# IvanBanny/para-ortho-pca-bo

Measured on AMD Instinct MI355X. Metric: BO iterations/sec (incl. GP refit + EI opt), BBOB f15 d=40, higher is better.
Workload: dtype f64; 1 GPU; configs[1]: PCA_BO on BBOB f15 d=40, budget=450, n_DoE=120, EI, var_threshold=0.95; one run per GPU (run list f15/d40/instances 0..N-1 partitioned by pcabo.sharding), timed steps spread evenly over the 330 BO iterations of the run; num_restarts=10, raw_samples=512, batch_limit=5, maxiter=200, parallelism=run-parallel x1

## Files before the change

### include/pcabo.h

```cpp
#ifndef PCABO_H
#define PCABO_H

#include <stddef.h>
#include <stdint.h>

#ifdef __cplusplus
extern "C" {
#endif

typedef struct pcabo_ctx pcabo_ctx;

typedef enum {
  PCABO_OK = 0,
  PCABO_ERR_ARG = -1,
  PCABO_ERR_NOT_PD = -2,
  PCABO_ERR_HIP = -3,
  PCABO_ERR_NAN = -4,
  PCABO_ERR_TIMEOUT = -5
} pcabo_status;

enum { PCABO_KERNEL_MATERN52 = 0, PCABO_KERNEL_RBF = 1 };
enum { PCABO_ACQ_LOG_EI = 0, PCABO_ACQ_PI = 1, PCABO_ACQ_UCB = 2 };
enum { PCABO_PTR_HOST = 0, PCABO_PTR_DEVICE = 1 };

int pcabo_abi_version(void);

int pcabo_device_count(void);

int pcabo_ctx_create(int device, int max_n, int max_d, int max_q, pcabo_ctx** out);
int pcabo_ctx_destroy(pcabo_ctx* ctx);
int pcabo_set_pointer_mode(pcabo_ctx* ctx, int mode);
int pcabo_last_error(pcabo_ctx* ctx, char* buf, int buflen);

enum { PCABO_OPT_RESIDENT = 0, PCABO_OPT_BESTF_F32 = 1, PCABO_OPT_GROUP_ACQ = 2,
       PCABO_OPT_DEVICE_LBFGSB = 3 ,
       PCABO_OPT_HIDDEN_TAIL = 5  };
int pcabo_set_option(pcabo_ctx* ctx, int option, int value);

int pcabo_wpca(pcabo_ctx* ctx, const double* X, const double* f, const int64_t* ranks, int n, int d,
               int maximize, double var_threshold, int n_components, const double* noise,
               double* data_mean, double* pca_mean, double* comps, double* evr, int* k, double* Z);

int pcabo_gp_condition(pcabo_ctx* ctx, const double* Z, const double* y, int n, int k,
                       const double* norm_bounds, double lengthscale, double noise, int kernel);

int pcabo_gp_condition_begin(pcabo_ctx* ctx, const double* Z, const double* y, int n, int k,
                             const double* norm_bounds, double lengthscale, double noise, int kernel);
int pcabo_gp_condition_end(pcabo_ctx* ctx);

int pcabo_gp_condition_end_eval(pcabo_ctx* ctx, const double* Xq, int q, double best_f, int maximize, int acq,
                                double* val);

int pcabo_gp_mll(pcabo_ctx* ctx, const double* Z , const double* y, int n, int k,
                 const double* norm_bounds, int kernel, const double* theta , double* loss, double* grad );
#define PCABO_FIT_TASK_NOT_PD (-2)
#define PCABO_FIT_TASK_DOMAIN (-3)
int pcabo_gp_fit(pcabo_ctx* ctx, const double* Z, const double* y, int n, int k, const double* norm_bounds, int kernel,
                 double* theta_inout , double* loss, int* info );
int pcabo_gp_mll_ard(pcabo_ctx* ctx, const double* Z, const double* y, int n, int k, const double* norm_bounds, int kernel,
                     const double* theta , double* loss, double* grad );
int pcabo_gp_fit_ard(pcabo_ctx* ctx, const double* Z, const double* y, int n, int k, const double* norm_bounds, int kernel,
                     double* theta_inout , double* loss, int* info );

int pcabo_wpca_gp_condition_begin(pcabo_ctx* ctx, const double* X, const double* f, const int64_t* ranks, int n,
                                  int d, int maximize, double var_threshold, int n_components, const double* noise,
                                  const double* y, double lengthscale, double gp_noise, int kernel,
                                  double* data_mean, double* pca_mean, double* comps, double* evr, int* k);

int pcabo_wpca_results(pcabo_ctx* ctx, double* data_mean, double* pca_mean, double* comps, double* evr, int* k);

int pcabo_acq_bounds(pcabo_ctx* ctx, double* bounds);

int pcabo_acq_eval(pcabo_ctx* ctx, const double* Xq, int q, double best_f, int maximize, int acq,
                   double* val, double* grad);
int pcabo_logei(pcabo_ctx* ctx, const double* Xq, int q, double best_f, int maximize,
                double* val, double* grad);

int pcabo_optimize_acqf(pcabo_ctx* ctx, const double* ics, int num_restarts, int batch_limit,
                        const double* bounds, int maxiter, double best_f, int maximize, int acq,
                        double* cand, double* vals, int* info, int* failed);

int pcabo_inverse_map(pcabo_ctx* ctx, const double* z, double* x);

int pcabo_get_gp_state(pcabo_ctx* ctx, double* K_chol , double* Rinv ,
                       double* alpha , double* y_mean_std , double* norm_bounds );
int pcabo_get_gram(pcabo_ctx* ctx, double* K );

typedef double (*pcabo_fg_callback)(const double* x, double* g, void* user);
int pcabo_lbfgsb_minimize(int nvar, double* x, const double* lower, const double* upper,
                          pcabo_fg_callback fg, void* user, int m, double factr, double pgtol,
                          int maxiter, int maxfun, int maxls, double* f_out, int* nit, int* nfev,
                          int* task_out);
int pcabo_lbfgsb_set_vector_kernels(int enabled);
int pcabo_lbfgsb_set_sum_order(int order);

int pcabo_sobol_scramble(int64_t* state, const int64_t* ltm, int k);
int pcabo_sobol_draw(const int64_t* state, const int64_t* shift, int k, int n, const double* lo, const double* rng, double* out);
int pcabo_sobol_draw_rows(const int64_t* const* states, const int64_t* const* shifts, const int* ks, int rows, int n,
                          const double* boxes, long long box_stride, double* const* outs);
int pcabo_torch_randint2(void* blob, int64_t count, int64_t* out);
int pcabo_torch_multinomial_rows(void* const* blobs, const double* weights, int rows, int n, int n_pick, int64_t* out);
int pcabo_boltzmann_pick_rows(void* const* blobs, const double* vals, int rows, int n, int n_pick, double eta, int64_t* out, int* flags);

int pcabo_set_profiling(pcabo_ctx* ctx, int enabled);
int pcabo_get_profile_calibration(pcabo_ctx* ctx, double* pair_ms, double* empty_kernel_ms);
int pcabo_get_profile(pcabo_ctx* ctx, int which, double* ms, int64_t* launches, double* bytes, double* flops);
int pcabo_reset_profile(pcabo_ctx* ctx);

typedef struct pcabo_batch pcabo_batch;
int pcabo_batch_create(int device, int B, int max_n, int max_d, int max_q, pcabo_batch** out);
int pcabo_batch_destroy(pcabo_batch* batch);
int pcabo_batch_set_workers(pcabo_batch* batch, int workers);
int pcabo_batch_set_option(pcabo_batch* batch, int option, int value);
int pcabo_device_lbfgsb_limits(int* max_n, int* max_k, int* max_group);
int pcabo_batch_last_error(pcabo_batch* batch, char* buf, int buflen);
pcabo_ctx* pcabo_batch_ctx(pcabo_batch* batch, int b);

int pcabo_batch_set_input_strides(pcabo_batch* batch, size_t x_stride, size_t noise_stride, size_t y_stride);
int pcabo_batch_wpca_gp_condition_begin(pcabo_batch* batch, const double* X, const int64_t* ranks, const double* noise,
// ... 49 lines not shown
```

### para-ortho-pca-bo_amd/csrc/kernels_acq.hip

```cpp
#include "pcabo_internal.h"
#include "acq_math.h"
#include <algorithm>
#include <cstdlib>
#include <mutex>

#define PSTRIDE (2 + 2 * PCABO_MAXD)

#ifdef PCABO_ACQ_TIMING
__device__ unsigned long long g_acq_stamps[16];
#define STAMP(i) do { if (blockIdx.x == gridDim.x / 2 && blockIdx.y == 0 && threadIdx.x == 0) g_acq_stamps[i] = wall_clock64(); } while (0)
#define STAMP_FIN(i) do { if (blockIdx.y == 0 && threadIdx.x == 0) g_acq_stamps[i] = wall_clock64(); } while (0)
extern "C" int pcabo_debug_acq_stamps(unsigned long long* out16) {
  return hipMemcpyFromSymbol(out16, HIP_SYMBOL(g_acq_stamps), sizeof(g_acq_stamps)) == hipSuccess ? 0 : -3;
}
#else
#define STAMP(i)
#define STAMP_FIN(i)
#endif

__device__ inline void st_wt(double* p, double v) {
  __hip_atomic_store(p, v, __ATOMIC_RELAXED, __HIP_MEMORY_SCOPE_AGENT);
}

template <int SLAB>
// ... 578 lines not shown
  __syncthreads();
  STAMP(5);
  {
    double gs[CU], gm[CU];
#pragma unroll
    for (int u = 0; u < CU; ++u) { gs[u] = 0.0; gm[u] = 0.0; }
#pragma unroll
    for (int b = 0; b < NB; ++b) {
      const double ts = s_ks[l + 64 * b], tm = s_tm[l + 64 * b];
#pragma unroll
      for (int u = 0; u < CU; ++u) {
        const double dlt = xc[u] - z[u][b];
        gs[u] += ts * dlt;
        gm[u] += tm * dlt;
      }
    }
    const int nu = k > w ? (k - w + 3) / 4 : 0;
    if (nu > 5) publish_grad<10>(gs, gm, w, k, l, pout, out, cur_seq);
    else if (nu > 2) publish_grad<5>(gs, gm, w, k, l, pout, out, cur_seq);
    else if (nu > 0) publish_grad<2>(gs, gm, w, k, l, pout, out, cur_seq);
  }
  }
  }
  q = (!SRV && ab.table) ? (int)(reinterpret_cast<const unsigned*>(qa.x)[blockIdx.y] & 0xffffu) : (int)blockIdx.y * qb;
  out = partial + ((size_t)q * S + s) * PSTRIDE;
  if (!server) {
    acq_tail<SLAB>(combine, s_v, partial, counters, q, S, k, bounds4, ystats, prm, val, grad, host_val, host_grad, hm, cur_seq, tid, w, l);
    break;
  }
  ++cur_seq;
  __syncthreads();
  }
}

__device__ void acq_scalar_core(double vv, double mus, int q, double ym, double ysd, const AcqParams& p, double* val,
                                double* host_val, double* coef, int l) {
  double value, c_mu, c_sg;
  acq_scalar_chain(vv, mus, ym, ysd, p.best_f, p.maximize, p.acq, &value, &c_mu, &c_sg);
  if (l == 0) {
    val[q] = value;
    if (host_val) host_val[q] = value;
    coef[0] = c_mu;
    coef[1] = c_sg;
  }
  STAMP_FIN(12);
}

__device__ void acq_finish_scalar(const double* base, int S, int q, const double* ystats, const AcqParams& p, double* val,
                                  double* host_val, double* coef, int l) {
  const double ym = ystats[0], ysd = ystats[1];
  double vv = 0.0, mus = 0.0;
  for (int s = l; s < S; s += 64) { vv += base[(size_t)s * PSTRIDE]; mus += base[(size_t)s * PSTRIDE + 1]; }
  vv = wave_sum(vv);
  mus = wave_sum(mus);
  STAMP_FIN(11);
  acq_scalar_core(vv, mus, q, ym, ysd, p, val, host_val, coef, l);
}

__device__ void acq_finish_query(const double* base, int S, int k, int q, const double* bounds4, const double* ystats,
                                 const AcqParams& p, double* val, double* grad, double* host_val, double* host_grad,
                                 int l) {
  __shared__ double s_cf2[4][2];
  double* coef = s_cf2[(threadIdx.x >> 6) & 3];
  acq_finish_scalar(base, S, q, ystats, p, val, host_val, coef, l);
  if (p.want_grad) {
    __builtin_amdgcn_wave_barrier();
    const double c_mu = coef[0], c_sg = coef[1];
    for (int c = l; c < k; c += 64) {
      double a0, b0, a1, b1, a2, b2;
      grad_partial_sum(base, S, c, 0, &a0, &b0);
      grad_partial_sum(base, S, c, 1, &a1, &b1);
      grad_partial_sum(base, S, c, 2, &a2, &b2);
      const double gs = (a0 + a1) + a2, gm = (b0 + b1) + b2;
      double g = __fma_rn(c_mu, gm, c_sg * gs) / (bounds4[PCABO_MAXD + c] - bounds4[c]);
      grad[(size_t)q * k + c] = g;
      if (host_grad) host_grad[(size_t)q * k + c] = g;
    }
  }
}

__global__ __launch_bounds__(256) void k_acq_combine(const double* __restrict__ partial, int q_total, int S, int k,
                                                     const double* __restrict__ bounds4,
                                                     const double* __restrict__ ystats, AcqParams p,
                                                     double* __restrict__ val, double* __restrict__ grad, AcqBatch ab) {
  if (ab.zs) {
    const unsigned run_ = blockIdx.z;
    partial = zrun(partial, ab.zs, run_); bounds4 = zrun(bounds4, ab.zs, run_); ystats = zrun(ystats, ab.zs, run_);
    val = zrun(val, ab.zs, run_); grad = zrun(grad, ab.zs, run_);
    if (ab.k_dev) k = *zrun(ab.k_dev, ab.zs, run_);
    if (ab.bestf) p.best_f = *zrun(ab.bestf, ab.zs, run_);
  }
  const int q = blockIdx.x * 4 + (threadIdx.x >> 6);
  if (q < q_total)
    acq_finish_query(partial + (size_t)q * S * PSTRIDE, S, k, q, bounds4, ystats, p, val, grad, nullptr, nullptr,
                     threadIdx.x & 63);
}

#ifdef PCABO_ACQ_TIMING
#define GSTAMP(i) do { if (blockIdx.x == gridDim.x - 1 && blockIdx.y == 0 && threadIdx.x == 0) g_acq_stamps[i] = wall_clock64(); } while (0)
#else
#define GSTAMP(i)
#endif
#define GQ 5
#define GT_LD 17
#define WAVE_LDS_SYNC() asm volatile("s_waitcnt lgkmcnt(0)" ::: "memory")
template <int NT>
__global__ __launch_bounds__(256) void k_acq_group(
    QueryArgs qa, const double* __restrict__ Xq, int n, int k, int NP, int ld,
    const double* __restrict__ ZnT, const double* __restrict__ R, const double* __restrict__ alpha,
    const double* __restrict__ bounds4, const double* __restrict__ ystats, AcqParams prm, double* partial,
    unsigned int* counters, double* __restrict__ val, double* __restrict__ grad, double* host_val, double* host_grad,
    HostMirror* hm, unsigned long long seq, AcqBatch ab) {
  const unsigned ent = reinterpret_cast<const unsigned*>(qa.x)[blockIdx.y];
  const unsigned run_ = ent >> 16;
  const int q0 = (int)((ent >> 8) & 0xffu), nq = (int)(ent & 0xffu);
  if (ab.zs) {
    ZnT = zrun(ZnT, ab.zs, run_); R = zrun(R, ab.zs, run_); alpha = zrun(alpha, ab.zs, run_);
    bounds4 = zrun(bounds4, ab.zs, run_); ystats = zrun(ystats, ab.zs, run_); partial = zrun(partial, ab.zs, run_);
    counters = zrun(counters, ab.zs, run_); val = zrun(val, ab.zs, run_); grad = zrun(grad, ab.zs, run_);
    Xq = zrun(Xq, ab.xq_host ? ab.hzs : ab.zs, run_);
    host_val = zrun(host_val, ab.hzs, run_); host_grad = zrun(host_grad, ab.hzs, run_); hm = zrun(hm, ab.hzs, run_);
    if (ab.k_dev) k = *zrun(ab.k_dev, ab.zs, run_);
    if (ab.bestf) prm.best_f = *zrun(ab.bestf, ab.zs, run_);
    if (ab.hyp) prm.inv_ls = zrun(ab.hyp, ab.zs, run_)[PCABO_HYP_INV_LS];
  }
  const int tid = threadIdx.x, l = tid & 63;
  const int w = __builtin_amdgcn_readfirstlane(tid >> 6);
  const int s = blockIdx.x, S = gridDim.x;
  const int r0 = 64 * s, ncol = 64 * (s + 1);
  const int KS = (k + 1) & ~1;
  extern __shared__ __attribute__((aligned(16))) double s_dyn[];
  double* s_ks = s_dyn;
  double* s_tile = s_ks + GQ * (NP > 2 * KS ? NP : 2 * KS);
  double* s_v = s_tile + 4 * 64 * GT_LD;
  double* s_tm = s_v + 64 * 8;
  double* s_coef = s_tm + GQ * 64;
  int* s_flag = reinterpret_cast<int*>(s_coef + 2 * GQ);
  double* s_vvmu = s_coef + 2 * GQ + 4;
  double* s_xn = s_vvmu + 2 * GQ;
  double* s_part = s_tile;
  double* s_gout = s_ks;
  const double inv_ls = prm.inv_ls;
  const int kernel = prm.kernel;

  GSTAMP(0);
  for (int idx = tid; idx < GQ * k; idx += 256) {
    const int q = idx / k, c = idx - q * k;
    const int qq = q < nq ? q : 0;
    const double lo = bounds4[c], hi = bounds4[PCABO_MAXD + c];
    s_xn[q * KS + c] = (Xq[(size_t)(q0 + qq) * k + c] - lo) / (hi - lo);
  }
  __syncthreads();
  GSTAMP(1);
  double cfr[NT][GQ];
  {
    const int jlim = n < ncol ? n : ncol;
    double sq[NT][GQ];
#pragma unroll
    for (int t = 0; t < NT; ++t)
#pragma unroll
      for (int q = 0; q < GQ; ++q) sq[t][q] = 0.0;
    constexpr int CB = NT == 1 ? 40 : (NT == 2 ? 20 : 8);
    for (int c0 = 0; c0 < k; c0 += CB) {
      double z[NT][CB];
#pragma unroll
      for (int t = 0; t < NT; ++t)
#pragma unroll
        for (int u = 0; u < CB; ++u) {
          const int cc = c0 + u < k ? c0 + u : k - 1, jj = tid + 256 * t < NP ? tid + 256 * t : NP - 1;
          z[t][u] = ZnT[(size_t)cc * ld + jj];
        }
#pragma unroll
      for (int u = 0; u < CB; ++u) {
        if (c0 + u < k) {
#pragma unroll
          for (int q = 0; q < GQ; ++q) {
            const double xq = s_xn[q * KS + c0 + u];
// ... 388 lines not shown
  const double* Rrow = R + (size_t)(I * 64) * ld;
  const double* Krow = KS + (size_t)(qb * 64) * ld;
  double pa[16], pb[16];
  auto fetch = [&](int J) {
#pragma unroll
    for (int u = 0; u < 16; ++u) {
      const int idx = tid + 256 * u, r = idx >> 6, c = idx & 63;
      pa[u] = Rrow[(size_t)r * ld + J * 64 + c];
      pb[u] = (qb * 64 + r < q_total) ? Krow[(size_t)r * ld + J * 64 + c] : 0.0;
    }
  };
  auto put = [&]() {
#pragma unroll
    for (int u = 0; u < 16; ++u) {
      const int idx = tid + 256 * u, r = idx >> 6, c = idx & 63;
      s_a[r * PCABO_TLD + c] = pa[u];
      s_b[r * PCABO_TLD + c] = pb[u];
    }
  };
  double4_t acc[4];
#pragma unroll
  for (int t = 0; t < 4; ++t) acc[t] = (double4_t){0.0, 0.0, 0.0, 0.0};
  fetch(0);
  for (int J = 0; J <= I; ++J) {
    __syncthreads();
    put();
    if (J < I) fetch(J + 1);
    __syncthreads();
    for (int kk = 0; kk < 64; kk += 4) {
      const double a = s_a[(16 * w + (l & 15)) * PCABO_TLD + kk + (l >> 4)];
#pragma unroll
      for (int t = 0; t < 4; ++t) {
        const double b = s_b[(16 * t + (l & 15)) * PCABO_TLD + kk + (l >> 4)];
        acc[t] = __builtin_amdgcn_mfma_f64_16x16x4f64(a, b, acc[t], 0, 0, 0);
      }
    }
  }
#pragma unroll
  for (int t = 0; t < 4; ++t) {
    double v = ((acc[t][0] * acc[t][0] + acc[t][1] * acc[t][1]) + acc[t][2] * acc[t][2]) + acc[t][3] * acc[t][3];
    v += __shfl_xor(v, 16, 64);
    v += __shfl_xor(v, 32, 64);
    if (l < 16) s_red[w][16 * t + l] = v;
  }
  __syncthreads();
  if (tid < 64 && qb * 64 + tid < q_total) {
    double* rec = partial + ((size_t)(qb * 64 + tid) * S + I) * PSTRIDE;
    rec[0] = ((s_red[0][tid] + s_red[1][tid]) + s_red[2][tid]) + s_red[3][tid];
    if (I >= njb) rec[1] = 0.0;
  }
}

bool score_gemm_possible(int q) { return q >= 64; }

__global__ __launch_bounds__(256) void k_score_ks_only(const double* __restrict__ Xq, int q_total, int n, int k, int NP, int ld,
                                                       const double* __restrict__ ZnT, const double* __restrict__ bounds4,
                                                       AcqParams prm, double* __restrict__ KS) {
  double ks[SC_QB];
  score_ks_block(Xq, q_total, n, k, NP, ld, ZnT, bounds4, prm, KS, ks);
}

__global__ __launch_bounds__(256) void k_score_mu(const double* __restrict__ KS, int q_total, int n, int ld,
                                                  const double* __restrict__ alpha, double* __restrict__ partial, int S) {
  __shared__ double s_mu[4][SC_QB];
  const int tid = threadIdx.x, l = tid & 63, w = tid >> 6;
  const int j = blockIdx.x * 256 + tid, q0 = blockIdx.y * SC_QB;
  const double aj = j < n ? alpha[j] : 0.0;
#pragma unroll
  for (int q = 0; q < SC_QB; ++q) {
    const double ks = (j < n && q0 + q < q_total) ? KS[(size_t)(q0 + q) * ld + j] : 0.0;
    const double m = wave_sum(aj * ks);
    if (l == 0) s_mu[w][q] = m;
  }
  __syncthreads();
  if (tid < SC_QB && q0 + tid < q_total)
    partial[((size_t)(q0 + tid) * S + blockIdx.x) * PSTRIDE + 1] = ((s_mu[0][tid] + s_mu[1][tid]) + s_mu[2][tid]) + s_mu[3][tid];
}

void launch_score_ks_only(hipStream_t st, const double* Xq, int q, const GpModel& m, AcqParams p, double* KS) {
  const int njb = (m.NP + 255) / 256;
  hipLaunchKernelGGL(k_score_ks_only, dim3(njb, (q + SC_QB - 1) / SC_QB, 1), dim3(256), 0, st, Xq, q, m.n, m.k, m.NP, m.ld, m.ZnT,
                     m.bounds4, p, KS);
}
void launch_score_tail(hipStream_t st, int q, const GpModel& m, AcqParams p, const double* KS, double* partial, double* val) {
  const int S = m.NP / 64, njb = (m.NP + 255) / 256;
  hipLaunchKernelGGL(k_score_mu, dim3(njb, (q + SC_QB - 1) / SC_QB, 1), dim3(256), 0, st, KS, q, m.n, m.ld, m.alpha, partial, S);
  hipLaunchKernelGGL(k_score_gemm, dim3(S, (q + 63) / 64, 1), dim3(256), 0, st, m.R, KS, q, m.NP, m.ld, njb, partial, (size_t)0);
  p.want_grad = 0;
  hipLaunchKernelGGL(k_acq_combine, dim3((q + 3) / 4, 1, 1), dim3(256), 0, st, partial, q, S, m.k, m.bounds4, m.ystats, p, val,
                     (double*)nullptr, AcqBatch());
}

void launch_score(hipStream_t st, const double* Xq, int q, const GpModel& m, AcqParams p, double* KS, double* partial, double* val,
                  AcqBatch ab, int B) {
  const int S = m.NP / 64, njb = (m.NP + 255) / 256;
  hipLaunchKernelGGL(k_score_ks, dim3(njb, (q + SC_QB - 1) / SC_QB, B), dim3(256), 0, st, Xq, q, m.n, m.k, m.NP, m.ld, m.ZnT, m.alpha,
                     m.bounds4, p, KS, partial, S, ab);
  hipLaunchKernelGGL(k_score_gemm, dim3(S, (q + 63) / 64, B), dim3(256), 0, st, m.R, KS, q, m.NP, m.ld, njb, partial, ab.zs);
  p.want_grad = 0;
  hipLaunchKernelGGL(k_acq_combine, dim3((q + 3) / 4, 1, B), dim3(256), 0, st, partial, q, S, m.k, m.bounds4, m.ystats, p, val,
                     (double*)nullptr, ab);
}

bool acq_server_possible(int q, int n, int k, int NP) {
  static int cus = -1;
  if (cus < 0) {
    int dev = 0;
    if (hipGetDevice(&dev) != hipSuccess || hipDeviceGetAttribute(&cus, hipDeviceAttributeMultiprocessorCount, dev) != hipSuccess) cus = 0;
  }
  if (k > 40 || NP > 512 || q < 1 || q > PCABO_INLAUNCH_MAXQ || (size_t)q * k > PCABO_QA_MAX) return false;
  const int S = acq_slabs(NP);
  return (S + 1) * q <= cus && S <= 32;
}

void launch_acq(hipStream_t st, const QueryArgs* qa, const double* Xq, int q, const GpModel& m, AcqParams p, double* partial,
                unsigned int* counters, double* val, double* grad, double* host_val, double* host_grad, HostMirror* hm,
                unsigned long long seq, MailPair* dev_mail, MailPair* part_pairs, AcqBatch ab, int B, int table_entries) {
  const int n = m.n, k = m.k, NP = m.NP, ld = m.ld;
  const double *ZnT = m.ZnT, *R = m.R, *alpha = m.alpha, *bounds4 = m.bounds4, *ystats = m.ystats;
  const int slab = NP >= ACQ_SLAB32_NP ? 32 : 16;
  const int S = NP / slab;
  static const QueryArgs empty = {};
  const int combine = hm != nullptr;
  const int nb = NP / 64;
  const bool fast = k <= 40 && nb <= 8;
  const int qb = (fast && !combine && q >= 64) ? 8 : 1;
  const int gy = ab.table ? table_entries : (q + qb - 1) / qb;
  const int gz = ab.table ? 1 : B;
#define ACQ_ARGS qa ? *qa : empty, Xq, q, n, k, NP, ld, ZnT, R, alpha, bounds4, ystats, p, partial, counters, val, grad, \
                 host_val, host_grad, hm, seq, combine, qb, dev_mail, part_pairs, ab
  const int FIN_LDS = 6 * PCABO_MAXD + 2;
#define ACQ_LDS(SL, NBV) (3 * NBV * 64 + PCABO_MAXD + SL + 2 + (4 * NBV * 64 > FIN_LDS ? 4 * NBV * 64 : FIN_LDS))
#define ACQ_FAST(SL, NBV)                                                                                      \
  case NBV:                                                                                                    \
    if (dev_mail)                                                                                              \
      hipLaunchKernelGGL((k_acq_fast<SL, NBV, true>), dim3(S + 1, gy), dim3(256),                              \
                         (size_t)std::max<int>(ACQ_LDS(SL, NBV), FIN_LDS_DOUBLES) * sizeof(double), st, ACQ_ARGS); \
    else                                                                                                       \
      hipLaunchKernelGGL((k_acq_fast<SL, NBV, false>), dim3(S, gy, gz), dim3(256),                             \
                         (size_t)ACQ_LDS(SL, NBV) * sizeof(double), st, ACQ_ARGS);                             \
    break;
  if (fast) {
    if (slab == 16) {
      switch (nb) { ACQ_FAST(16, 1) ACQ_FAST(16, 2) ACQ_FAST(16, 3) ACQ_FAST(16, 4) ACQ_FAST(16, 5) ACQ_FAST(16, 6)
                    ACQ_FAST(16, 7) ACQ_FAST(16, 8) }
    } else {
      switch (nb) { ACQ_FAST(32, 1) ACQ_FAST(32, 2) ACQ_FAST(32, 3) ACQ_FAST(32, 4) ACQ_FAST(32, 5) ACQ_FAST(32, 6)
                    ACQ_FAST(32, 7) ACQ_FAST(32, 8) }
    }
  } else {
    size_t lds = (size_t)(3 * NP + PCABO_MAXD + 32 + 2 + 6 * PCABO_MAXD + 2) * sizeof(double);
    if (slab == 16)
      hipLaunchKernelGGL(k_acq_fused<16>, dim3(S, ab.table ? gy : q, gz), dim3(256), lds, st, ACQ_ARGS);
    else
      hipLaunchKernelGGL(k_acq_fused<32>, dim3(S, ab.table ? gy : q, gz), dim3(256), lds, st, ACQ_ARGS);
  }
#undef ACQ_FAST
#undef ACQ_LDS
#undef ACQ_ARGS
  if (!combine)
    hipLaunchKernelGGL(k_acq_combine, dim3((q + 3) / 4, 1, gz), dim3(256), 0, st, partial, q, S, k, bounds4, ystats, p, val,
                       grad, ab);
}

template <int N>
__global__ __launch_bounds__(64) void k_debug_wave_sum_multi(const double* __restrict__ in, double* ref, double* multi,
                                                             double* uni, int* mism) {
  const int l = threadIdx.x;
  double v[N];
#pragma unroll
  for (int i = 0; i < N; ++i) v[i] = in[i * 64 + l];
#pragma unroll
  for (int i = 0; i < N; ++i) { const double r = wave_sum(v[i]); if (l == 0) ref[i] = r; }
  wave_sum_multi<N>(v, l);
  const int own = wave_multi_owner<N>(l), idx = wave_multi_index<N>(l);
  if (own >= 0) multi[own] = v[0];
  __syncthreads();
  if (__double_as_longlong(multi[idx]) != __double_as_longlong(v[0])) atomicAdd(&mism[idx], 1);
#pragma unroll
  for (int i = 0; i < N; ++i) { const double r = read_lane(v[0], __builtin_amdgcn_readfirstlane(wave_multi_lane(N, i))); if (l == 0) uni[i] = r; }
}

extern "C" int pcabo_debug_wave_sum_multi(const double* in, int N, double* ref, double* multi, double* uni, int* mism) {
  double* d = nullptr;
  if (hipMalloc(&d, (size_t)N * (64 + 3) * sizeof(double) + (size_t)N * sizeof(int)) != hipSuccess) return -3;
  double *dref = d + N * 64, *dmul = dref + N, *duni = dmul + N;
  int* dmis = reinterpret_cast<int*>(duni + N);
  int rc = hipMemcpy(d, in, (size_t)N * 64 * sizeof(double), hipMemcpyHostToDevice) == hipSuccess ? 0 : -3;
  if (rc == 0 && hipMemset(dref, 0, (size_t)N * 3 * sizeof(double) + (size_t)N * sizeof(int)) != hipSuccess) rc = -3;
#define DBG_WSM(NV) case NV: hipLaunchKernelGGL(k_debug_wave_sum_multi<NV>, dim3(1), dim3(64), 0, 0, d, dref, dmul, duni, dmis); break;
  if (rc == 0) {
    switch (N) { DBG_WSM(1) DBG_WSM(2) DBG_WSM(3) DBG_WSM(4) DBG_WSM(5) DBG_WSM(7) DBG_WSM(8) DBG_WSM(10) DBG_WSM(13)
                 DBG_WSM(20) DBG_WSM(33) DBG_WSM(64) default: rc = -1; }
  }
#undef DBG_WSM
  if (rc == 0 && hipGetLastError() != hipSuccess) rc = -3;
  if (rc == 0 && (hipMemcpy(ref, dref, N * sizeof(double), hipMemcpyDeviceToHost) != hipSuccess ||
                  hipMemcpy(multi, dmul, N * sizeof(double), hipMemcpyDeviceToHost) != hipSuccess ||
                  hipMemcpy(uni, duni, N * sizeof(double), hipMemcpyDeviceToHost) != hipSuccess ||
                  hipMemcpy(mism, dmis, N * sizeof(int), hipMemcpyDeviceToHost) != hipSuccess)) rc = -3;
  (void)hipFree(d);
  return rc;
}
```

### para-ortho-pca-bo_amd/csrc/kernels_gp.hip

```cpp
#include "pcabo_internal.h"
#include <mutex>
#include <cstdlib>

#define BS PCABO_BS
#define TLD PCABO_TLD

__global__ __launch_bounds__(256) void k_gram(const double* __restrict__ AT, const double* __restrict__ nrm, int n,
                                              int KP, int ld, double noise, int kernel, double* __restrict__ K,
                                              const int* __restrict__ k_dev, double* __restrict__ K2,
                                              int* __restrict__ info_reset, size_t zs, const double* __restrict__ hyp) {
  const XcdTile xt_ = xcd_tile();
  ZRUNX(AT); ZRUNX(nrm); ZRUNX(K); ZRUNX(k_dev); ZRUNX(K2); ZRUNX(info_reset); ZRUNX(hyp);
  if (hyp) noise = hyp[PCABO_HYP_NOISE];
  const int ti = (int)xt_.x, tj = (int)xt_.y;
  if (info_reset && ti == 0 && tj == 0 && threadIdx.x == 0) *info_reset = 0;
  if (tj > ti) return;
  if (k_dev) KP = (*k_dev + 3) & ~3;
  const int w = threadIdx.x >> 6, l = threadIdx.x & 63;
  const int i0 = ti * BS + 16 * w, j0 = tj * BS;
  double4_t acc[4];
  for (int t = 0; t < 4; ++t) acc[t] = (double4_t){0.0, 0.0, 0.0, 0.0};
  for (int kk = 0; kk < KP; kk += 4) {
    const double* row = AT + (size_t)(kk + (l >> 4)) * ld;
    double a = row[i0 + (l & 15)];
// ... 195 lines not shown
    for (int q = 0; q < 4; ++q)
#pragma unroll
      for (int r = 0; r < 4; ++r) dst[(size_t)(16 * w + (l >> 4) + 4 * r) * ld + 16 * q + (l & 15)] = cold[q][r];
  }
}
#define CHOL_LOOKN_NC 2
#define CHOL_LOOKN_LDS ((size_t)(1 + CHOL_LOOKN_NC) * BS * TLD * sizeof(double))

__global__ __launch_bounds__(256) void k_trinv_cols(const double* __restrict__ L, int nblk, int ld,
                                                    double* R, size_t zs) {
  const XcdTile xt_ = xcd_tile();
  ZRUNX(L); ZRUNX(R);
  __shared__ __attribute__((aligned(16))) double s_t[BS * TLD];
  __shared__ __attribute__((aligned(16))) double s_xk[BS * 16];
  const int tid = threadIdx.x;
  const int c0 = (int)xt_.x * 16;
  const int J = c0 / BS;
  const int w = tid >> 6, l = tid & 63;
  double pt[16], px[4];
  auto fetch_tile = [&](const double* src) {
#pragma unroll
    for (int u = 0; u < 16; ++u) { const int idx = tid + 256 * u; pt[u] = src[(size_t)(idx >> 6) * ld + (idx & 63)]; }
  };
  auto fetch_x = [&](int Kb) {
#pragma unroll
    for (int u = 0; u < 4; ++u) { const int idx = tid + 256 * u; px[u] = R[(size_t)(Kb * BS + (idx >> 4)) * ld + c0 + (idx & 15)]; }
  };
  auto put_tile = [&]() {
#pragma unroll
    for (int u = 0; u < 16; ++u) { const int idx = tid + 256 * u; s_t[(idx >> 6) * TLD + (idx & 63)] = pt[u]; }
  };
  auto put_x = [&]() {
#pragma unroll
    for (int u = 0; u < 4; ++u) s_xk[tid + 256 * u] = px[u];
  };
  if (J + 1 < nblk) { fetch_tile(L + (size_t)((J + 1) * BS) * ld + J * BS); fetch_x(J); }
  for (int I = J + 1; I < nblk; ++I) {
    double4_t acc = {0.0, 0.0, 0.0, 0.0};
    for (int Kb = J; Kb < I; ++Kb) {
      __syncthreads();
      put_tile(); put_x();
      if (Kb + 1 < I) { fetch_tile(L + (size_t)(I * BS) * ld + (Kb + 1) * BS); fetch_x(Kb + 1); }
      else fetch_tile(R + (size_t)(I * BS) * ld + I * BS);
      __syncthreads();
      for (int kk = 0; kk < BS; kk += 4) {
        double a = s_t[(16 * w + (l & 15)) * TLD + kk + (l >> 4)];
        double b = s_xk[(kk + (l >> 4)) * 16 + (l & 15)];
        acc = __builtin_amdgcn_mfma_f64_16x16x4f64(a, b, acc, 0, 0, 0);
      }
    }
    __syncthreads();
    for (int r = 0; r < 4; ++r) s_xk[(16 * w + (l >> 4) + 4 * r) * 16 + (l & 15)] = -acc[r];
    put_tile();
    if (I + 1 < nblk) { fetch_tile(L + (size_t)((I + 1) * BS) * ld + J * BS); fetch_x(J); }
    __syncthreads();
    double4_t x = {0.0, 0.0, 0.0, 0.0};
    for (int kk = 0; kk < BS; kk += 4) {
      double a = s_t[(16 * w + (l & 15)) * TLD + kk + (l >> 4)];
      double b = s_xk[(kk + (l >> 4)) * 16 + (l & 15)];
      x = __builtin_amdgcn_mfma_f64_16x16x4f64(a, b, x, 0, 0, 0);
    }
    for (int r = 0; r < 4; ++r)
      R[(size_t)(I * BS + 16 * w + (l >> 4) + 4 * r) * ld + c0 + (l & 15)] = x[r];
    __threadfence_block();
  }
}

__global__ __launch_bounds__(256) void k_rmatvec(const double* __restrict__ R, const double* __restrict__ y, int n,
                                                 int ld, double* __restrict__ t, size_t zs) {
  ZRUN(R); ZRUN(y); ZRUN(t);
  const int w = threadIdx.x >> 6, l = threadIdx.x & 63;
  for (int rr = 0; rr < 4; ++rr) {
    const int i = blockIdx.x * 16 + w * 4 + rr;
    double s = 0.0;
    if (i < n)
      for (int j = l; j <= i; j += 64) s += R[(size_t)i * ld + j] * y[j];
    s = wave_sum(s);
    if (l == 0) t[i] = (i < n) ? s : 0.0;
  }
}

#define RTM_WAVES 16
__global__ __launch_bounds__(64 * RTM_WAVES) void k_rtmatvec(const double* __restrict__ R, const double* __restrict__ t,
                                                             int n, int ld, double* __restrict__ out, size_t zs) {
  ZRUN(R); ZRUN(t); ZRUN(out);
  __shared__ double s_p[RTM_WAVES][64];
  const int w = threadIdx.x >> 6, l = threadIdx.x & 63;
  const int j0 = blockIdx.x * 64, j = j0 + l;
  double a0 = 0.0, a1 = 0.0, a2 = 0.0, a3 = 0.0;
  int i = j0 + w;
  for (; i + 3 * RTM_WAVES < n; i += 4 * RTM_WAVES) {
    a0 = fma(R[(size_t)i * ld + j], t[i], a0);
    a1 = fma(R[(size_t)(i + RTM_WAVES) * ld + j], t[i + RTM_WAVES], a1);
    a2 = fma(R[(size_t)(i + 2 * RTM_WAVES) * ld + j], t[i + 2 * RTM_WAVES], a2);
    a3 = fma(R[(size_t)(i + 3 * RTM_WAVES) * ld + j], t[i + 3 * RTM_WAVES], a3);
  }
  for (; i < n; i += RTM_WAVES) a0 = fma(R[(size_t)i * ld + j], t[i], a0);
  s_p[w][l] = (a0 + a1) + (a2 + a3);
  __syncthreads();
  if (w == 0) {
    double s = 0.0;
#pragma unroll
    for (int u = 0; u < RTM_WAVES; ++u) s += s_p[u][l];
    out[j] = (j < n) ? s : 0.0;
  }
}

void launch_gram(hipStream_t s, const double* AT, const double* nrm, int n, int NP, int KP, int ld, double noise,
                 int kernel, double* K, const int* k_dev, double* K2, int* info_reset, ZB zb) {
  int nb = NP / BS;
  hipLaunchKernelGGL(k_gram, dim3(nb, nb, zb.B), dim3(256), 0, s, AT, nrm, n, KP, ld, noise, kernel, K, k_dev, K2, info_reset,
                     zb.zs, zb.hyp);
}
void launch_add_jitter(hipStream_t s, double* K, int n, int ld, double jitter) {
  hipLaunchKernelGGL(k_add_jitter, dim3((n + 255) / 256), dim3(256), 0, s, K, n, ld, jitter);
}
bool chol_step_form(int NP, ZB zb) { return zb.B * (NP / BS) <= 256; }
int launch_cholesky(hipStream_t s, double* L, int NP, int ld, int* info, double* diag_scratch, ZB zb, double* R_folded) {
  const int nblk = NP / BS;
  if (chol_step_form(NP, zb)) return launch_chol_steps(s, L, NP, ld, info, diag_scratch, zb, R_folded);
  if (R_folded) return -1;
  if (zb.B * nblk > 1024) {
    for (int p = 0; p < nblk; ++p) {
      if (p > 0)
        hipLaunchKernelGGL(k_chol_lookback, dim3(nblk - p + 1, 1, zb.B), dim3(256), 0, s, L, p, nblk, ld, diag_scratch, zb.zs);
      launch_chol_panel(s, L, p, nblk - p, ld, info, diag_scratch, zb);
    }
    return 0;
  }
  constexpr int NC = CHOL_LOOKN_NC;
  {
    static std::mutex attr_mu;
    static bool attr_done[64] = {false};
    int dev = 0;
    if (hipGetDevice(&dev) != hipSuccess || dev < 0 || dev >= 64) return -1;
    std::lock_guard<std::mutex> lk(attr_mu);
    if (!attr_done[dev]) {
      if (hipFuncSetAttribute((const void*)k_chol_lookn<NC>, hipFuncAttributeMaxDynamicSharedMemorySize, (int)CHOL_LOOKN_LDS) != hipSuccess) return -1;
      attr_done[dev] = true;
    }
  }
  int last_panel = -1;
  for (int Jc = 0; Jc < nblk; Jc += NC) {
    const int ncols = nblk - Jc < NC ? nblk - Jc : NC;
    if (Jc > 0) {
      hipLaunchKernelGGL(k_chol_lookn<NC>, dim3(nblk - Jc + 1, 1, zb.B), dim3(256 * NC), CHOL_LOOKN_LDS, s, L, Jc, ncols, 0, Jc, ld,
                         diag_scratch, last_panel, zb.zs);
      last_panel = -1;
    }
    for (int c = 0; c < ncols; ++c) {
      const int p = Jc + c;
      launch_chol_panel(s, L, p, nblk - p, ld, info, diag_scratch, zb);
      last_panel = nblk - p > 1 ? p : -1;
      if (c + 1 < ncols) {
        hipLaunchKernelGGL(k_chol_lookn<NC>, dim3(nblk - (p + 1) + 1, 1, zb.B), dim3(256 * NC), CHOL_LOOKN_LDS, s, L, p + 1,
                           ncols - c - 1, p, p + 1, ld, diag_scratch, last_panel, zb.zs);
        last_panel = -1;
      }
    }
  }
  return 0;
}
void launch_trinv(hipStream_t s, const double* L, int NP, int ld, double* R, ZB zb) {
  const int nblk = NP / BS;
  launch_trinv_diag_w(s, L, nblk, ld, R, zb);
  hipLaunchKernelGGL(k_trinv_cols, dim3(NP / 16, 1, zb.B), dim3(256), 0, s, L, nblk, ld, R, zb.zs);
}
void launch_alpha(hipStream_t s, const double* R, const double* ys, int n, int NP, int ld, double* tmp, double* alpha,
                  ZB zb) {
  hipLaunchKernelGGL(k_rmatvec, dim3(NP / 16, 1, zb.B), dim3(256), 0, s, R, ys, n, ld, tmp, zb.zs);
  hipLaunchKernelGGL(k_rtmatvec, dim3(NP / 64, 1, zb.B), dim3(64 * RTM_WAVES), 0, s, R, tmp, n, ld, alpha, zb.zs);
}
```

### para-ortho-pca-bo_amd/csrc/kernels_wpca.hip

```cpp
#include "pcabo_internal.h"
#include <cstdlib>

#define WP_THREADS 1024

__device__ inline double block_sum_1024(double v, double* s_red) {
  const int tid = threadIdx.x, l = tid & 63;
  s_red[tid] = v;
  __syncthreads();
  if (tid < 64) {
    double a[8];
#pragma unroll
    for (int j = 0; j < 8; ++j) a[j] = s_red[64 * j + l] + s_red[64 * (j + 8) + l];
#pragma unroll
    for (int j = 0; j < 4; ++j) a[j] = a[j] + a[j + 4];
    a[0] = a[0] + a[2]; a[1] = a[1] + a[3];
    double x = a[0] + a[1];
#pragma unroll
    for (int off = 32; off > 0; off >>= 1) {
      const double y = __shfl_down(x, off, 64);
      if (l < off) x = x + y;
    }
    if (l == 0) s_red[0] = x;
  }
  __syncthreads();
  const double r = s_red[0];
  __syncthreads();
  return r;
}

__global__ void k_rank(const double* __restrict__ f, int n, int maximize, long long* __restrict__ ranks) {
  int i = blockIdx.x * blockDim.x + threadIdx.x;
  if (i >= n) return;
  double fi = maximize ? -f[i] : f[i];
  int r = 1;
  for (int j = 0; j < n; ++j) {
    double fj = maximize ? -f[j] : f[j];
    r += (fj < fi) || (fj == fi && j < i);
  }
  ranks[i] = r;
}

__global__ __launch_bounds__(WP_THREADS) void k_wpca_prep(
    const double* __restrict__ X, const long long* __restrict__ ranks, const double* __restrict__ noise,
    int n, int d, int DP, double* __restrict__ weights, double* __restrict__ data_mean,
    double* __restrict__ pca_mean, double* __restrict__ Wc, size_t zs) {
  ZRUN(X); ZRUN(ranks); ZRUN(noise); ZRUN(weights); ZRUN(data_mean); ZRUN(pca_mean); ZRUN(Wc);
  __shared__ double s_red[WP_THREADS];
  __shared__ double s_col[PCABO_MAXD];
  const int tid = threadIdx.x;
  const int CP = DP <= 64 ? 64 : 128;
  const int G = WP_THREADS / CP;
  const int c = tid % CP, g = tid / CP;
  const int n4 = (n + 3) & ~3;

  double loc = 0.0;
  const double logn = log((double)n);
  for (int i = tid; i < n; i += WP_THREADS) {
    double pw = logn - log((double)ranks[i]);
    weights[i] = pw;
    loc += pw;
  }
  const double tot = block_sum_1024(loc, s_red);
  for (int i = tid; i < n; i += WP_THREADS) weights[i] = weights[i] / tot;
  __syncthreads();

  constexpr int WP_ROWS = 32;
  const bool in_regs = (n4 + G - 1) / G <= WP_ROWS;
  double xr[WP_ROWS];
  double acc = 0.0;
  if (in_regs) {
#pragma unroll
    for (int u = 0; u < WP_ROWS; ++u) {
      const int i = g + u * G;
      xr[u] = (c < d && i < n) ? X[(size_t)i * d + c] : 0.0;
      if ((u & 7) == 7) __builtin_amdgcn_sched_barrier(0);
    }
    if (c < d) {
#pragma unroll
      for (int u = 0; u < WP_ROWS; ++u)
        if (g + u * G < n) acc += xr[u];
    }
  } else if (c < d) {
    for (int i = g; i < n; i += G) acc += X[(size_t)i * d + c];
  }
  s_red[tid] = acc;
  __syncthreads();
  if (tid < CP) {
    double s = 0.0;
    for (int gg = 0; gg < G; ++gg) s += s_red[gg * CP + tid];
    s_col[tid] = s / (double)n;
    if (tid < d) data_mean[tid] = s_col[tid];
  }
  __syncthreads();
  const double mu = (c < d) ? s_col[c] : 0.0;
  __syncthreads();

  acc = 0.0;
  if (in_regs) {
    if (c < DP) {
#pragma unroll
      for (int u = 0; u < WP_ROWS; ++u) {
        const int i = g + u * G;
        double w = 0.0;
        if (c < d && i < n) {
          w = (xr[u] - mu) * sqrt(weights[i]);
          if (noise) w += noise[(size_t)i * d + c];
        }
        xr[u] = w;
        if (i < n4) acc += w;
        if ((u & 7) == 7) __builtin_amdgcn_sched_barrier(0);
      }
    }
  } else if (c < DP) {
    for (int i = g; i < n4; i += G) {
      double w = 0.0;
      if (c < d && i < n) {
        w = (X[(size_t)i * d + c] - mu) * sqrt(weights[i]);
        if (noise) w += noise[(size_t)i * d + c];
      }
      Wc[(size_t)i * DP + c] = w;
      acc += w;
    }
  }
  s_red[tid] = acc;
  __syncthreads();
  if (tid < CP) {
    double s = 0.0;
    for (int gg = 0; gg < G; ++gg) s += s_red[gg * CP + tid];
    s_col[tid] = s / (double)n;
    if (tid < d) pca_mean[tid] = s_col[tid];
  }
  __syncthreads();
  const double mw = (c < d) ? s_col[c] : 0.0;
  if (in_regs) {
    if (c < DP) {
#pragma unroll
      for (int u = 0; u < WP_ROWS; ++u) {
        const int i = g + u * G;
        if (i < n4) Wc[(size_t)i * DP + c] = (c < d && i < n) ? xr[u] - mw : 0.0;
        if ((u & 7) == 7) __builtin_amdgcn_sched_barrier(0);
      }
    }
  } else if (c < d) {
    for (int i = g; i < n; i += G) Wc[(size_t)i * DP + c] -= mw;
  }
}

__global__ __launch_bounds__(256) void k_cov(const double* __restrict__ Wc, int n4, int DP, double inv_nm1,
                                             double* __restrict__ C, size_t zs) {
  ZRUN(Wc); ZRUN(C);
  __shared__ double s_acc[4][4][64];
  const int ti = blockIdx.x, tj = blockIdx.y;
  const int w = threadIdx.x >> 6, l = threadIdx.x & 63;
  double4_t acc = {0.0, 0.0, 0.0, 0.0};
  const int steps = n4 >> 2;
  for (int s = w; s < steps; s += 4) {
    const size_t row = (size_t)(4 * s + (l >> 4)) * DP;
    double a = Wc[row + ti * 16 + (l & 15)];
    double b = Wc[row + tj * 16 + (l & 15)];
    acc = __builtin_amdgcn_mfma_f64_16x16x4f64(a, b, acc, 0, 0, 0);
  }
  for (int r = 0; r < 4; ++r) s_acc[w][r][l] = acc[r];
  __syncthreads();
  if (w == 0) {
    for (int r = 0; r < 4; ++r) {
      double s = ((s_acc[0][r][l] + s_acc[1][r][l]) + s_acc[2][r][l]) + s_acc[3][r][l];
      C[(size_t)(ti * 16 + (l >> 4) + 4 * r) * DP + tj * 16 + (l & 15)] = s * inv_nm1;
    }
  }
}

#define JAC_THREADS 1024
#ifdef PCABO_ACQ_TIMING
__device__ unsigned long long g_jac_stamps[8];
extern "C" int pcabo_debug_jacobi_stamps(unsigned long long* out4) {
  return hipMemcpyFromSymbol(out4, HIP_SYMBOL(g_jac_stamps), sizeof(g_jac_stamps)) == hipSuccess ? 0 : -3;
}
#endif
struct PcaSelect {
  int n; double var_threshold; int n_components; double* comps; double* evr; int* k_dev; HostMirror* hm;
};
template <int NT>
__device__ inline void jac_chain(const double* x, const double* y, double& a, double& b, double& g) {
#pragma clang fp contract(off)
  a = NT > 1 ? x[NT > 1 ? 1 : 0] * x[NT > 1 ? 1 : 0] : 0.0;
  b = NT > 1 ? y[NT > 1 ? 1 : 0] * y[NT > 1 ? 1 : 0] : 0.0;
  a = __builtin_fma(x[0], x[0], a);
  b = __builtin_fma(y[0], y[0], b);
  g = __builtin_fma(x[0], y[0], 0.0);
  if (NT > 1) g = __builtin_fma(x[NT > 1 ? 1 : 0], y[NT > 1 ? 1 : 0], g);
#pragma unroll
  for (int t = 2; t < NT; ++t) {
    a = __builtin_fma(x[t], x[t], a);
    b = __builtin_fma(y[t], y[t], b);
    g = __builtin_fma(x[t], y[t], g);
  }
}
__device__ inline void jac_rotation(double a, double b, double g, double& cs, double& sn) {
#pragma clang fp contract(off)
  double r = __builtin_amdgcn_rcp(g);
  r = __builtin_fma(__builtin_fma(-g, r, 1.0), r, r);
  const double zeta = ((b - a) * 0.5) * r;
  const double hyp = __builtin_fma(zeta, zeta, 1.0);
  double y = __builtin_amdgcn_rsq(hyp);
  y = y * __builtin_fma((-0.5 * hyp) * y, y, 1.5);
  const double den = __builtin_fma(hyp, y, fabs(zeta));
  double q = __builtin_amdgcn_rcp(den);
  q = __builtin_fma(__builtin_fma(-den, q, 1.0), q, q);
  const double t = zeta >= 0.0 ? q : -q;
  const double w = __builtin_fma(t, t, 1.0), hw = -0.5 * w;
  double c = __builtin_amdgcn_rsq(w);
  c = c * __builtin_fma(hw * c, c, 1.5);
  c = c * __builtin_fma(hw * c, c, 1.5);
  cs = c;
  sn = c * t;
}
__device__ inline void jac_apply(double cs, double sn, double x, double y, double& xo, double& yo) {
#pragma clang fp contract(off)
  xo = __builtin_fma(cs, x, -(sn * y));
  yo = __builtin_fma(sn, x, cs * y);
}
template <int NT>
__global__ __launch_bounds__(JAC_THREADS) void k_jacobi(const double* __restrict__ C, int d, int DP,
                                                        const double* __restrict__ V0, double* __restrict__ Gout,
                                                        double* __restrict__ lam, int* __restrict__ sweeps_out,
                                                        PcaSelect sel, size_t zs, size_t hzs) {
  ZRUN(C); ZRUN(V0); ZRUN(Gout); ZRUN(lam); ZRUN(sweeps_out); ZRUN(sel.comps); ZRUN(sel.evr); ZRUN(sel.k_dev);
  sel.hm = zrun(sel.hm, hzs, blockIdx.z);
  constexpr int LP = 16;
  constexpr int RP = 16 * NT;
  constexpr int LD = RP | 1;
  extern __shared__ __attribute__((aligned(16))) double s_g[];
  __shared__ double s_lam[PCABO_MAXD], s_sgn[PCABO_MAXD], s_evr[PCABO_MAXD];
  __shared__ int s_order[PCABO_MAXD];
  __shared__ int s_rot;
  const int tid = threadIdx.x;
  if (tid == 0) s_rot = 0;
  __syncthreads();
  const bool staged = V0 && d <= 64;
  double* s_c = s_g + (size_t)d * LD;
  double* s_v = s_c + (size_t)d * LD;
  if (staged) {
    for (int idx = tid; idx < d * d; idx += (int)blockDim.x) {
      const int a = idx / d, b = idx % d;
      s_c[a * LD + b] = C[(size_t)a * DP + b];
      s_v[a * LD + b] = V0[(size_t)a * d + b];
    }
    __syncthreads();
  }
  if (V0) {
    if (staged) {
      for (int col = tid; col < d; col += (int)blockDim.x) {
        double a = 0.0;
        for (int r = 0; r < d; ++r) { double v = s_v[col * LD + r]; a += v * v; }
        if (!(fabs(a - 1.0) < 1e-8)) s_rot = 1;
      }
    } else {
      for (int col = tid >> 6; col < d; col += (int)blockDim.x >> 6) {
        double a = 0.0;
        for (int r = tid & 63; r < d; r += 64) { const double v = V0[(size_t)col * d + r]; a += v * v; }
        a = wave_sum(a);
        if ((tid & 63) == 0 && !(fabs(a - 1.0) < 1e-8)) s_rot = 1;
      }
// ... 72 lines not shown
        a += dpp_row<0xB1>(a); b += dpp_row<0xB1>(b); g += dpp_row<0xB1>(g);
        a += dpp_row<0x4E>(a); b += dpp_row<0x4E>(b); g += dpp_row<0x4E>(g);
        a += dpp_row<0x141>(a); b += dpp_row<0x141>(b); g += dpp_row<0x141>(g);
        a += dpp_row<0x140>(a); b += dpp_row<0x140>(b); g += dpp_row<0x140>(g);
        const double ab = a * b, gg = g * g;
        JSTAMP(ph_dot);
        if (gg > tol * tol * ab && fabs(g) > 1e-300) {
          double cs, sn;
          jac_rotation(a, b, g, cs, sn);
#ifdef PCABO_ACQ_TIMING
          if (cs == 123.456) s_rot = 2;
#endif
          JSTAMP(ph_rot);
#pragma unroll
          for (int t = 0; t < NT; ++t) {
            double xo, yo;
            jac_apply(cs, sn, xr[t], yr[t], xo, yo);
            gp[16 * t] = xo; gq[16 * t] = yo;
          }
          if (lane == 0 && gg > 1e-16 * ab) s_rot = 1;
          JSTAMP(ph_wr);
        }
      }
      __syncthreads();
      JSTAMP(ph_bar);
    }
    int rot = s_rot;
    __syncthreads();
    if (tid == 0) s_rot = 0;
    __syncthreads();
    if (!rot) { ++sweep; break; }
  }
#ifdef PCABO_ACQ_TIMING
  if (tid == 0) { g_jac_stamps[0] = clock64() - jc0; g_jac_stamps[1] = wall_clock64() - jw0; g_jac_stamps[2] = (unsigned long long)sweep; g_jac_stamps[3] = (unsigned long long)(de - 1);
    g_jac_stamps[4] = ph_dot; g_jac_stamps[5] = ph_rot; g_jac_stamps[6] = ph_wr; g_jac_stamps[7] = ph_bar; }
#endif
  {
    const int nw = (int)blockDim.x >> 6, w = tid >> 6, l = tid & 63;
    for (int c0 = w; c0 < d; c0 += 8 * nw) {
      double x0[8], x1[8], v[8];
#pragma unroll
      for (int i = 0; i < 8; ++i) {
        const int col = c0 + nw * i;
        x0[i] = col < d && l < d ? s_g[col * LD + l] : 0.0;
        x1[i] = col < d && l + 64 < d ? s_g[col * LD + l + 64] : 0.0;
        v[i] = __builtin_fma(x1[i], x1[i], __builtin_fma(x0[i], x0[i], 0.0));
      }
      wave_sum_multi<8>(v, l);
      const double nrm = sqrt(v[0]);
      const double inv = nrm > 0.0 ? 1.0 / nrm : 0.0;
#pragma unroll
      for (int i = 0; i < 8; ++i) {
        const int col = c0 + nw * i;
        const double inv_i = read_lane(inv, i);
        if (col < d && l < d) {
          const double u = x0[i] * inv_i;
          Gout[(size_t)col * d + l] = u;
          s_g[col * LD + l] = u;
        }
        if (col < d && l + 64 < d) {
          const double u = x1[i] * inv_i;
          Gout[(size_t)col * d + l + 64] = u;
          s_g[col * LD + l + 64] = u;
        }
      }
      if (l < 8 && c0 + nw * l < d) { lam[c0 + nw * l] = nrm / cscale; s_lam[c0 + nw * l] = nrm; }
    }
  }
  if (tid == 0) *sweeps_out = sweep;
  __syncthreads();
  if (tid < d) {
    const double me = s_lam[tid];
    int r = 0;
    for (int j = 0; j < d; ++j) r += (s_lam[j] > me) || (s_lam[j] == me && j < tid);
    s_order[r] = tid;
  }
  __syncthreads();
  const int rcount = sel.n < d ? sel.n : d;
  if (tid < rcount) {
    double tot = 0.0;
    for (int r = 0; r < rcount; ++r) tot += s_lam[s_order[r]];
    const double e = s_lam[s_order[tid]] / tot;
    sel.evr[tid] = e;
    s_evr[tid] = e;
    const double* v = s_g + s_order[tid] * LD;
    double best = -1.0, sgn = 1.0;
    for (int j = 0; j < d; ++j) {
      double a = fabs(v[j]);
      if (a > best) { best = a; sgn = v[j] < 0.0 ? -1.0 : 1.0; }
    }
    s_sgn[tid] = sgn;
  }
  __syncthreads();
  if (tid == 0) {
    int k;
    double cum = 0.0;
    int cnt = 0;
    for (int r = 0; r < rcount; ++r) {
      cum += s_evr[r];
      cnt += (cum <= sel.var_threshold);
    }
    if (sel.n_components > 0) k = sel.n_components < rcount ? sel.n_components : rcount;
    else {
      k = cnt + 1;
      if (k > rcount) k = rcount;
      if (k < 1) k = 1;
    }
    *sel.k_dev = k;
    sel.hm->k = k;
  }
  for (int idx = tid; idx < rcount * d; idx += (int)blockDim.x) {
    const int r = idx / d, j = idx % d;
    sel.comps[idx] = s_sgn[r] * s_g[s_order[r] * LD + j];
  }
}

__global__ __launch_bounds__(256) void k_project(const double* __restrict__ X, const double* __restrict__ data_mean,
                                                 const double* __restrict__ pca_mean, const double* __restrict__ comps,
                                                 const int* __restrict__ k_dev, int n, int d, double* __restrict__ Z,
                                                 size_t zs) {
  ZRUN(X); ZRUN(data_mean); ZRUN(pca_mean); ZRUN(comps); ZRUN(k_dev); ZRUN(Z);
  __shared__ double s_x[8][PCABO_MAXD];
  __shared__ double s_m[PCABO_MAXD];
  const int k = *k_dev;
  const int i0 = blockIdx.x * 8;
  for (int idx = threadIdx.x; idx < 8 * d; idx += 256) {
    int r = idx / d, j = idx % d;
    s_x[r][j] = (i0 + r < n) ? X[(size_t)(i0 + r) * d + j] - data_mean[j] : 0.0;
  }
  if (threadIdx.x < d) s_m[threadIdx.x] = pca_mean[threadIdx.x];
  __syncthreads();
  for (int idx = threadIdx.x; idx < 8 * k; idx += 256) {
    int r = idx / k, c = idx % k;
    if (i0 + r >= n) continue;
    const double* ck = comps + (size_t)c * d;
    double s = 0.0, sm = 0.0;
    for (int j = 0; j < d; ++j) { s += s_x[r][j] * ck[j]; sm += s_m[j] * ck[j]; }
    Z[(size_t)(i0 + r) * k + c] = s - sm;
  }
}

__global__ __launch_bounds__(WP_THREADS) void k_zstats(const double* __restrict__ Z, const double* __restrict__ y,
                                                       int n, int k, const double* __restrict__ user_nb,
                                                       double* __restrict__ bounds4, double* __restrict__ zn_mean,
                                                       double* __restrict__ ystats, double* __restrict__ ys,
                                                       HostMirror* hm, const int* __restrict__ k_dev, size_t zs,
                                                       size_t hzs, double mean_c, const double* __restrict__ hyp,
                                                       const double* __restrict__ ard_ls) {
  ZRUN(Z); ZRUN(y); ZRUN(user_nb); ZRUN(bounds4); ZRUN(zn_mean); ZRUN(ystats); ZRUN(ys); ZRUN(k_dev); ZRUN(hyp);
  if (hyp) mean_c = hyp[PCABO_HYP_MEAN_C];
  hm = zrun(hm, hzs, blockIdx.z);
  if (k_dev) k = *k_dev;
  __shared__ double s_red[WP_THREADS];
  __shared__ double s_min[WP_THREADS];
  __shared__ double s_max[WP_THREADS];
  const int tid = threadIdx.x;
  const int CP = k <= 64 ? 64 : 128;
  const int G = WP_THREADS / CP;
  const int c = tid % CP, g = tid / CP;
  double mn = INFINITY, mx = -INFINITY, sm = 0.0;
  if (c < k) {
    int i = g;
    for (; i + 7 * G < n; i += 8 * G) {
      double z[8];
#pragma unroll
      for (int u = 0; u < 8; ++u) z[u] = Z[(size_t)(i + u * G) * k + c];
#pragma unroll
      for (int u = 0; u < 8; ++u) { mn = fmin(mn, z[u]); mx = fmax(mx, z[u]); sm += z[u]; }
    }
    for (; i < n; i += G) {
      double z = Z[(size_t)i * k + c];
      mn = fmin(mn, z); mx = fmax(mx, z); sm += z;
    }
  }
  s_min[tid] = mn; s_max[tid] = mx; s_red[tid] = sm;
  __syncthreads();
  if (tid < k) {
    double a = INFINITY, b = -INFINITY, s = 0.0;
    for (int gg = 0; gg < G; ++gg) {
      a = fmin(a, s_min[gg * CP + tid]); b = fmax(b, s_max[gg * CP + tid]); s += s_red[gg * CP + tid];
    }
    double rng = b - a;
    double nlo = a - 0.1 * rng, nhi = b + 0.1 * rng;
    if (user_nb) { nlo = user_nb[tid]; nhi = user_nb[k + tid]; }
    if (ard_ls) nhi = nlo + fmax((nhi - nlo) * ard_ls[tid], fmax(fabs(nlo), nhi - nlo) * 0x1p-40);
    double alo = a - 0.5 * rng, ahi = b + 0.5 * rng;
    if (ahi - alo < 0.1) { double mid = (ahi + alo) / 2; alo = mid - 0.1 / 2; ahi = mid + 0.1 / 2; }
    bounds4[tid] = nlo; bounds4[PCABO_MAXD + tid] = nhi;
    bounds4[2 * PCABO_MAXD + tid] = alo; bounds4[3 * PCABO_MAXD + tid] = ahi;
    hm->norm_lo[tid] = nlo; hm->norm_hi[tid] = nhi; hm->acq_lo[tid] = alo; hm->acq_hi[tid] = ahi;
    zn_mean[tid] = (s / (double)n - nlo) / (nhi - nlo);
  }
  __syncthreads();
  double loc = 0.0;
  for (int i = tid; i < n; i += WP_THREADS) loc += y[i];
  const double ym = block_sum_1024(loc, s_red) / (double)n;
  loc = 0.0;
  for (int i = tid; i < n; i += WP_THREADS) { double t = y[i] - ym; loc += t * t; }
  double var = block_sum_1024(loc, s_red) / (double)(n > 1 ? n - 1 : 1);
  double sd = sqrt(var);
  if (!(sd >= 1e-8)) sd = 1.0;
  const double ym2 = (mean_c == 0.0) ? ym : ym + sd * mean_c;
  for (int i = tid; i < n; i += WP_THREADS) ys[i] = (y[i] - ym2) / sd;
  if (tid == 0) { ystats[0] = ym2; ystats[1] = sd; hm->y_mean = ym2; hm->y_std = sd; }
}

__global__ __launch_bounds__(256) void k_znorm(const double* __restrict__ Z, int n, int k, int NP, int KP, int ld,
                                               const double* __restrict__ bounds4, const double* __restrict__ zn_mean,
                                               double inv_ls, double* __restrict__ ZnT, double* __restrict__ AT,
                                               double* __restrict__ nrm, const int* __restrict__ k_dev, size_t zs,
                                               const double* __restrict__ hyp) {
  ZRUN(Z); ZRUN(bounds4); ZRUN(zn_mean); ZRUN(ZnT); ZRUN(AT); ZRUN(nrm); ZRUN(k_dev); ZRUN(hyp);
  if (hyp) inv_ls = hyp[PCABO_HYP_INV_LS];
  if (k_dev) { k = *k_dev; KP = (k + 3) & ~3; }
  const int i = blockIdx.x * 256 + threadIdx.x;
  if (i >= NP) return;
  double s = 0.0;
  const size_t row = (size_t)(i < n ? i : n - 1) * k;
  for (int c0 = 0; c0 < KP; c0 += 4) {
    double zr[4];
#pragma unroll
    for (int u = 0; u < 4; ++u) zr[u] = Z[row + (c0 + u < k ? c0 + u : k - 1)];
#pragma unroll
    for (int u = 0; u < 4; ++u) {
      const int c = c0 + u;
      double zn = 0.0, a = 0.0;
      if (i < n && c < k) {
        double lo = bounds4[c], hi = bounds4[PCABO_MAXD + c];
        zn = (zr[u] - lo) / (hi - lo);
        a = (zn - zn_mean[c]) * inv_ls;
      }
      ZnT[(size_t)c * ld + i] = zn;
      AT[(size_t)c * ld + i] = a;
      s += a * a;
    }
  }
  nrm[i] = s;
}

__global__ __launch_bounds__(128) void k_inverse_map(const double* __restrict__ z, const double* __restrict__ comps,
                                                     const double* __restrict__ data_mean,
                                                     const double* __restrict__ pca_mean, int k, int d,
                                                     double* __restrict__ x, const int* __restrict__ k_dev, size_t zs,
                                                     double* __restrict__ host_x, HostMirror* hm, unsigned long long seq) {
  ZRUN(z); ZRUN(comps); ZRUN(data_mean); ZRUN(pca_mean); ZRUN(x); ZRUN(k_dev);
  if (k_dev) k = *k_dev;
  const int j = threadIdx.x;
  if (j < d) {
    double s = 0.0;
    int c = 0;
    for (; c + 8 <= k; c += 8) {
      double cv[8];
#pragma unroll
      for (int u = 0; u < 8; ++u) cv[u] = comps[(size_t)(c + u) * d + j];
#pragma unroll
      for (int u = 0; u < 8; ++u) s += z[c + u] * cv[u];
    }
    for (; c < k; ++c) s += z[c] * comps[(size_t)c * d + j];
    const double xj = (s + pca_mean[j]) + data_mean[j];
    x[j] = xj;
    if (host_x) host_x[j] = xj;
  }
  if (hm) {
    __threadfence_system();
    __syncthreads();
    if (threadIdx.x == 0)
      __hip_atomic_store(const_cast<unsigned long long*>(&hm->qflag[0]), seq, __ATOMIC_RELEASE, __HIP_MEMORY_SCOPE_SYSTEM);
  }
}

void launch_rank(hipStream_t s, const double* f, int n, int maximize, long long* ranks) {
  hipLaunchKernelGGL(k_rank, dim3((n + 255) / 256), dim3(256), 0, s, f, n, maximize, ranks);
}
void launch_wpca_prep(hipStream_t s, const double* X, const long long* ranks, const double* noise, int n, int d,
                      int DP, double* weights, double* data_mean, double* pca_mean, double* Wc, ZB zb) {
  hipLaunchKernelGGL(k_wpca_prep, dim3(1, 1, zb.B), dim3(WP_THREADS), 0, s, X, ranks, noise, n, d, DP, weights, data_mean,
                     pca_mean, Wc, zb.zs);
}
void launch_cov(hipStream_t s, const double* Wc, int n, int DP, double* C, ZB zb) {
  int n4 = (n + 3) & ~3;
  hipLaunchKernelGGL(k_cov, dim3(DP / 16, DP / 16, zb.B), dim3(256), 0, s, Wc, n4, DP, 1.0 / (double)(n - 1), C, zb.zs);
}
template <int NT>
static void launch_jacobi_as(hipStream_t s, int threads, size_t lds, const double* C, int d, int DP, const double* V0, double* G,
                             double* lam, int* sweeps, const PcaSelect& sel, const ZB& zb) {
  static bool attr_set = false;
  if (!attr_set) {
    (void)hipFuncSetAttribute((const void*)k_jacobi<NT>, hipFuncAttributeMaxDynamicSharedMemorySize, 156 * 1024);
    attr_set = true;
  }
  hipLaunchKernelGGL(k_jacobi<NT>, dim3(1, 1, zb.B), dim3(threads), lds, s, C, d, DP, V0, G, lam, sweeps, sel, zb.zs, zb.hzs);
}
void launch_jacobi(hipStream_t s, const double* C, int d, int DP, const double* V0, double* G, double* lam, int* sweeps,
                   int n, double var_threshold, int n_components, double* comps, double* evr, int* k_dev, HostMirror* hm,
                   ZB zb) {
  const int nt = d <= 16 ? 1 : d <= 32 ? 2 : d <= 48 ? 3 : d <= 64 ? 4 : d <= 96 ? 6 : 8;
  const size_t col = (size_t)(16 * nt | 1);
  size_t lds = (size_t)d * col * sizeof(double);
  if (V0 && d <= 64) lds += (size_t)2 * d * col * sizeof(double);
  const int npairs = ((d + 1) & ~1) / 2;
  int threads = (npairs * 16 + 63) & ~63;
  if (threads < d) threads = (d + 63) & ~63;
  PcaSelect sel{n, var_threshold, n_components, comps, evr, k_dev, hm};
  switch (nt) {
    case 1: launch_jacobi_as<1>(s, threads, lds, C, d, DP, V0, G, lam, sweeps, sel, zb); break;
    case 2: launch_jacobi_as<2>(s, threads, lds, C, d, DP, V0, G, lam, sweeps, sel, zb); break;
    case 3: launch_jacobi_as<3>(s, threads, lds, C, d, DP, V0, G, lam, sweeps, sel, zb); break;
    case 4: launch_jacobi_as<4>(s, threads, lds, C, d, DP, V0, G, lam, sweeps, sel, zb); break;
    case 6: launch_jacobi_as<6>(s, threads, lds, C, d, DP, V0, G, lam, sweeps, sel, zb); break;
    default: launch_jacobi_as<8>(s, threads, lds, C, d, DP, V0, G, lam, sweeps, sel, zb); break;
  }
}
void launch_project(hipStream_t s, const double* X, const double* data_mean, const double* pca_mean,
                    const double* comps, const int* k_dev, int n, int d, double* Z, ZB zb) {
  hipLaunchKernelGGL(k_project, dim3((n + 7) / 8, 1, zb.B), dim3(256), 0, s, X, data_mean, pca_mean, comps, k_dev, n, d, Z,
                     zb.zs);
}
void launch_zstats(hipStream_t s, const double* Z, const double* y, int n, int k, const double* user_norm_bounds,
                   double* bounds4, double* zn_mean, double* ystats, double* ys, HostMirror* hm, const int* k_dev, ZB zb,
                   double mean_c, const double* ard_ls) {
  hipLaunchKernelGGL(k_zstats, dim3(1, 1, zb.B), dim3(WP_THREADS), 0, s, Z, y, n, k, user_norm_bounds, bounds4, zn_mean,
                     ystats, ys, hm, k_dev, zb.zs, zb.hzs, mean_c, zb.hyp, ard_ls);
}
void launch_znorm(hipStream_t s, const double* Z, int n, int k, int NP, int KP, int ld, const double* bounds4,
                  const double* zn_mean, double inv_ls, double* ZnT, double* AT, double* nrm, const int* k_dev, ZB zb) {
  hipLaunchKernelGGL(k_znorm, dim3((NP + 255) / 256, 1, zb.B), dim3(256), 0, s, Z, n, k, NP, KP, ld, bounds4, zn_mean, inv_ls,
                     ZnT, AT, nrm, k_dev, zb.zs, zb.hyp);
}
void launch_inverse_map(hipStream_t s, const double* z, const double* comps, const double* data_mean,
                        const double* pca_mean, int k, int d, double* x, const int* k_dev, ZB zb, double* host_x,
                        HostMirror* hm, unsigned long long seq) {
  hipLaunchKernelGGL(k_inverse_map, dim3(1, 1, zb.B), dim3(128), 0, s, z, comps, data_mean, pca_mean, k, d, x, k_dev, zb.zs,
                     host_x, hm, seq);
}
```

### para-ortho-pca-bo_amd/csrc/pcabo_api.hip

```cpp
#include "../../include/pcabo.h"
#include "pcabo_internal.h"
#include "lbfgsb.h"
#include "host_side.h"

#include <algorithm>
#include <atomic>
#include <chrono>
#include <thread>
#include <condition_variable>
#include <functional>
#include <mutex>
#include <cstdlib>
#include <cmath>
#include <cstdio>
#include <cstring>
#include <new>
#include <optional>
#include <vector>
#include <dirent.h>
#include <fcntl.h>
#include <signal.h>
#include <stdint.h>
#include <cerrno>
#include <unistd.h>
#include <emmintrin.h>

#define PCABO_ABI_VERSION 2
#define PROF_GROUPS 6
#define PROF_POOL 4096

struct ProfPair { hipEvent_t a, b; int group; double bytes, flops; };

struct OptHelper {
  std::thread th;
  std::mutex mu;
  std::condition_variable cv;
  std::atomic<unsigned> go{0}, done{0};
  std::atomic<bool> quit{false}, active{false};
  std::function<void()> fn;
  void run() {
    unsigned seen = 0;
    while (true) {
      {
        std::unique_lock<std::mutex> lk(mu);
        cv.wait(lk, [&] { return active.load(std::memory_order_acquire) || quit.load(std::memory_order_acquire); });
      }
      if (quit.load(std::memory_order_acquire)) return;
      while (active.load(std::memory_order_acquire)) {
        const unsigned cur = go.load(std::memory_order_acquire);
        if (cur == seen) { __builtin_ia32_pause(); continue; }
        seen = cur;
        fn();
        done.store(cur, std::memory_order_release);
      }
    }
  }
  void start() { if (!th.joinable()) th = std::thread([this] { run(); }); }
  void begin(std::function<void()> f) {
    start();
    fn = std::move(f);
    { std::lock_guard<std::mutex> lk(mu); active.store(true, std::memory_order_release); }
    cv.notify_one();
  }
  void end() { active.store(false, std::memory_order_release); }
  void shutdown() {
    if (!th.joinable()) return;
    { std::lock_guard<std::mutex> lk(mu); quit.store(true, std::memory_order_release); active.store(false, std::memory_order_release); }
    cv.notify_one();
    th.join();
  }
};

struct pcabo_ctx {
  int device = 0;
  hipStream_t stream = nullptr;
  hipEvent_t evBounds = nullptr;
  hipEvent_t evPca = nullptr;
  hipStream_t stream2 = nullptr;
  hipEvent_t evZn = nullptr, evKS = nullptr;
  bool zn_recorded = false;
  bool opt_hidden_tail = true;
  int max_n = 0, max_d = 0, max_q = 0;
  int NPcap = 0, ld = 0, DPcap = 0, KPcap = 0, Scap = 0;
  int ptr_mode = PCABO_PTR_HOST;
  int n = 0, d = 0, k = 0, NP = 0, KP = 0;
  bool have_wpca = false, have_gp = false, gp_pending = false;
  int wpca_n = 0, wpca_d = 0; bool wpca_uncollected = false;
  double lengthscale = 0.0, noise = 0.0;
  int kernel = 0;
  double *dX = nullptr, *dNoise = nullptr, *dF = nullptr, *dWeights = nullptr, *dWc = nullptr;
  long long* dRanks = nullptr;
  double *dDataMean = nullptr, *dPcaMean = nullptr, *dC = nullptr, *dG = nullptr, *dLam = nullptr;
  double* dGbuf[2] = {nullptr, nullptr};
  int gcur = 0, vprev_d = 0;
  double *dComps = nullptr, *dEvr = nullptr, *dZ = nullptr;
  double* dPcaOut = nullptr;
  double *dIn = nullptr, *hIn = nullptr;
  int *dK = nullptr, *dSweeps = nullptr, *dInfo = nullptr;
  double *dY = nullptr, *dYs = nullptr, *dYstats = nullptr, *dBounds4 = nullptr, *dZnMean = nullptr, *dUserNB = nullptr;
  double *dZnT = nullptr, *dAT = nullptr, *dNrm = nullptr, *dGram = nullptr, *dL = nullptr, *dR = nullptr;
  double *dTmp = nullptr, *dAlpha = nullptr, *dDiag = nullptr;
  double *dXq = nullptr, *dPartial = nullptr, *dVal = nullptr, *dGrad = nullptr, *dZq = nullptr, *dXout = nullptr;
  unsigned int* dCounters = nullptr;
  int cnt_S = 0; bool cnt_dirty = true;
  double* dKS = nullptr;
  double* dBestF = nullptr;
  double* dMll = nullptr;
  double* dArdLs = nullptr;
  double* dHyp = nullptr;
  char *dRegion = nullptr, *hRegion = nullptr;
  size_t region_bytes = 0, hregion_bytes = 0;
  bool in_batch = false; int batch_index = 0;
  bool rt_stale = false;
  HostMirror* hm = nullptr;
  double *hXq = nullptr, *hVal = nullptr, *hGrad = nullptr, *hSmall = nullptr, *hBestF = nullptr;
  double* hMll = nullptr;
  double* hArdLs = nullptr;
  double* hHyp = nullptr;
  MailPair* dMail = nullptr;
  bool mail_bar = false;
  MailPair* dPairs = nullptr;
  bool opt_resident = true;
  bool opt_group_acq = false;
  bool bestf_f32 = true;
  int srv_penalty = 0;
  unsigned long long seq = 0;
  OptHelper helper;
  std::vector<std::unique_ptr<OptHelper>> more_helpers;
  bool registered = false;
  bool alone = true; int alone_age = 0;
  char err[512] = {0};
  bool prof = false;
  std::vector<ProfPair> pairs;
  size_t pairs_used = 0;
  double prof_ms[PROF_GROUPS] = {0};
  double prof_pair_ms = 0.0;
  double prof_empty_ms = 0.0;
  int64_t prof_launches[PROF_GROUPS] = {0};
  double prof_bytes[PROF_GROUPS] = {0}, prof_flops[PROF_GROUPS] = {0};
};

static std::mutex g_presence_mu;
static int g_presence_refs[64] = {0};
static void presence_path(char* buf, size_t n, int device, long pid) { snprintf(buf, n, "/dev/shm/pcabo.%d.%ld", device, pid); }
static void presence_register(int device) {
  if (device < 0 || device >= 64) return;
  std::lock_guard<std::mutex> lk(g_presence_mu);
  if (g_presence_refs[device]++ == 0) {
    char path[128]; presence_path(path, sizeof(path), device, (long)getpid());
    int fd = open(path, O_CREAT | O_WRONLY, 0644);
    if (fd >= 0) close(fd);
  }
}
static void presence_unregister(int device) {
  if (device < 0 || device >= 64) return;
  std::lock_guard<std::mutex> lk(g_presence_mu);
  if (g_presence_refs[device] > 0 && --g_presence_refs[device] == 0) {
    char path[128]; presence_path(path, sizeof(path), device, (long)getpid());
    unlink(path);
  }
}
static int presence_local_contexts(int device) {
  if (device < 0 || device >= 64) return 1;
  std::lock_guard<std::mutex> lk(g_presence_mu);
// ... 234 lines not shown
  HIPCHK(hipEventCreateWithFlags(&ctx->evPca, hipEventDisableTiming));
  if (!stream) {
    HIPCHK(hipStreamCreateWithFlags(&ctx->stream2, hipStreamNonBlocking));
    HIPCHK(hipEventCreateWithFlags(&ctx->evZn, hipEventDisableTiming));
    HIPCHK(hipEventCreateWithFlags(&ctx->evKS, hipEventDisableTiming));
  }
  ctx->region_bytes = carve_device(ctx, nullptr);
  ctx->hregion_bytes = carve_host(ctx, nullptr);
  if (dreg) {
    ctx->dRegion = dreg; ctx->hRegion = hreg;
  } else {
    HIPCHK(hipMalloc((void**)&ctx->dRegion, ctx->region_bytes));
    HIPCHK(hipHostMalloc((void**)&ctx->hRegion, ctx->hregion_bytes, hipHostMallocDefault));
    memset(ctx->hRegion, 0, ctx->hregion_bytes);
  }
  carve_device(ctx, ctx->dRegion);
  carve_host(ctx, ctx->hRegion);
  if (!dreg) {
    HIPCHK(hipMemsetAsync(ctx->dRegion, 0, ctx->region_bytes, ctx->stream));
    if (hipExtMallocWithFlags((void**)&ctx->dMail, PCABO_MAIL_PAIRS * sizeof(MailPair), hipDeviceMallocFinegrained) != hipSuccess) {
      (void)hipGetLastError();
      HIPCHK(dalloc(&ctx->dMail, PCABO_MAIL_PAIRS));
    }
    HIPCHK(hipMemsetAsync(ctx->dMail, 0, PCABO_MAIL_PAIRS * sizeof(MailPair), ctx->stream));
    const size_t np = (size_t)PCABO_INLAUNCH_MAXQ * 32 * (2 + 2 * PCABO_MAXD);
    HIPCHK(dalloc(&ctx->dPairs, np));
    HIPCHK(hipMemsetAsync(ctx->dPairs, 0, np * sizeof(MailPair), ctx->stream));
    HIPCHK(hipStreamSynchronize(ctx->stream));
    ctx->mail_bar = mail_bar_usable(ctx);
  } else {
    ctx->opt_resident = false;
  }
  {
    static std::atomic<unsigned long long> ctx_counter{0};
    ctx->seq = ((unsigned long long)(getpid() & 0xffff) << 44) + ((ctx_counter.fetch_add(1) + 1) << 30);
  }
  return PCABO_OK;
}

static void ctx_teardown(pcabo_ctx* ctx) {
  (void)hipSetDevice(ctx->device);
  if (ctx->stream2) (void)hipStreamSynchronize(ctx->stream2);
  if (ctx->stream) (void)hipStreamSynchronize(ctx->stream);
  for (auto& p : ctx->pairs) { (void)hipEventDestroy(p.a); (void)hipEventDestroy(p.b); }
  if (!ctx->in_batch) {
    if (ctx->dRegion) (void)hipFree(ctx->dRegion);
    if (ctx->hRegion) (void)hipHostFree(ctx->hRegion);
    if (ctx->dMail) (void)hipFree(ctx->dMail);
    if (ctx->dPairs) (void)hipFree(ctx->dPairs);
  }
  if (ctx->evBounds) (void)hipEventDestroy(ctx->evBounds);
  if (ctx->evPca) (void)hipEventDestroy(ctx->evPca);
  if (ctx->evZn) (void)hipEventDestroy(ctx->evZn);
  if (ctx->evKS) (void)hipEventDestroy(ctx->evKS);
  if (ctx->stream2) (void)hipStreamDestroy(ctx->stream2);
  if (ctx->stream && !ctx->in_batch) (void)hipStreamDestroy(ctx->stream);
  ctx->helper.shutdown();
  for (auto& h : ctx->more_helpers) h->shutdown();
  ctx->more_helpers.clear();
  if (ctx->registered) presence_unregister(ctx->device);
}

static bool ctx_sizes_ok(int max_n, int max_d, int max_q) {
  return max_n >= 2 && max_d >= 1 && max_d <= PCABO_MAXD && max_q >= 1 && max_q < PCABO_CNT_DONE;
}

struct RowsDH {
  const double *Z, *y, *unb;
  int n, k, KP; const int* k_dev;
  double inv_ls, noise, mean_c; int kernel;
  ZB zb;
  hipEvent_t ev[2];
  int* cnt_S; bool* cnt_dirty;
  const double* ard_ls = nullptr;
  hipEvent_t ev_zn = nullptr;
};
template <class Phase>
static int enqueue_factor(pcabo_ctx* ctx, hipStream_t s, int n, int NP, ZB zb, Phase&& phase) {
  if (const int rc = phase(2)) return rc;
  const bool fold = !ctx->in_batch && ctx->opt_hidden_tail && zb.zs == 0 && zb.B == 1 && chol_step_form(NP, zb);
  if (launch_cholesky(s, ctx->dL, NP, ctx->ld, ctx->dInfo, ctx->dDiag, zb, fold ? ctx->dR : nullptr) != 0)
    return set_err(ctx, PCABO_ERR_HIP, "the Cholesky launches could not be set up (device or kernel attribute)%s", "");
  if (const int rc = phase(3)) return rc;
  if (fold) launch_trinv_drain(s, ctx->dL, NP, ctx->ld, ctx->dR);
  else launch_trinv(s, ctx->dL, NP, ctx->ld, ctx->dR, zb);
  launch_alpha(s, ctx->dR, ctx->dYs, n, NP, ctx->ld, ctx->dTmp, ctx->dAlpha, zb);
  if (const int rc = phase(4)) return rc;
  if (zb.zs) HIPCHK(hipMemcpy2DAsync((void*)&ctx->hm->chol_info, zb.hzs, ctx->dInfo, zb.zs, sizeof(int), zb.B, hipMemcpyDeviceToHost, s));
  else HIPCHK(hipMemcpyAsync((void*)&ctx->hm->chol_info, ctx->dInfo, sizeof(int), hipMemcpyDeviceToHost, s));
  return PCABO_OK;
}
template <class Phase>
static int enqueue_rows_dh(pcabo_ctx* ctx, hipStream_t s, const RowsDH& a, Phase&& phase) {
  const int NP = round_up(a.n, PCABO_BS);
  if (a.cnt_S && (acq_slabs(NP) != *a.cnt_S || *a.cnt_dirty)) {
    if (a.zb.zs) HIPCHK(hipMemset2DAsync(ctx->dCounters, a.zb.zs, 0, (PCABO_CNT_DONE + 1) * sizeof(unsigned int), a.zb.B, s));
    else HIPCHK(hipMemsetAsync(ctx->dCounters, 0, (PCABO_CNT_DONE + 1) * sizeof(unsigned int), s));
    *a.cnt_S = acq_slabs(NP); *a.cnt_dirty = false;
  }
  if (const int rc = phase(1)) return rc;
  launch_zstats(s, a.Z, a.y, a.n, a.k, a.unb, ctx->dBounds4, ctx->dZnMean, ctx->dYstats, ctx->dYs, ctx->hm, a.k_dev, a.zb, a.mean_c, a.ard_ls);
  for (hipEvent_t e : a.ev) if (e) HIPCHK(hipEventRecord(e, s));
  launch_znorm(s, a.Z, a.n, a.k, NP, a.KP, ctx->ld, ctx->dBounds4, ctx->dZnMean, a.inv_ls, ctx->dZnT, ctx->dAT, ctx->dNrm, a.k_dev, a.zb);
  if (a.ev_zn) HIPCHK(hipEventRecord(a.ev_zn, s));
  launch_gram(s, ctx->dAT, ctx->dNrm, a.n, NP, a.KP, ctx->ld, a.noise, a.kernel, nullptr, a.k_dev, ctx->dL, ctx->dInfo, a.zb);
  return enqueue_factor(ctx, s, a.n, NP, a.zb, phase);
}

struct CondProf {
  pcabo_ctx* c; int kk;
  std::optional<ProfScope> ps;
  int operator()(int phase) {
    const double n = c->n;
    ps.reset();
    if (phase == 1) ps.emplace(c, 1, 8.0 * n * kk + 4.0 * n * (n + 1.0), 2.0 * n * n * kk + 12.0 * n * n);
    if (phase == 2) ps.emplace(c, 2, 16.0 * n * n, n * n * n / 3.0);
    if (phase == 3) ps.emplace(c, 3, 16.0 * n * n, n * n * n / 3.0 + 2.0 * n * n);
    return PCABO_OK;
  }
};

static int launch_factorisation(pcabo_ctx* ctx, double jitter) {
  hipStream_t s = ctx->stream;
  if (jitter > 0.0) {
    launch_gram(s, ctx->dAT, ctx->dNrm, ctx->n, ctx->NP, round_up(ctx->k, 4), ctx->ld, ctx->noise, ctx->kernel, nullptr, nullptr,
                ctx->dL, ctx->dInfo);
    launch_add_jitter(s, ctx->dL, ctx->n, ctx->ld, jitter);
  }
  return enqueue_factor(ctx, s, ctx->n, ctx->NP, ZB(), CondProf{ctx, 0});
}

template <class Extra>
static int factor_attempts(pcabo_ctx* ctx, int attempt, Extra&& extra) {
  double jitter = 1e-8;
  for (int a = 2; a <= attempt; ++a) jitter *= 10.0;
  for (;; ++attempt) {
    if (attempt > 0) {
      const int rc = launch_factorisation(ctx, jitter);
      if (rc != PCABO_OK) return rc;
      jitter *= 10.0;
    }
    const int rc = extra();
    if (rc != PCABO_OK) return rc;
    HIPCHK(wait_stream(ctx->stream));
    HIPCHK(hipGetLastError());
    if (ctx->hm->chol_info == 0) return PCABO_OK;
    if (attempt == 3)
      return set_err(ctx, PCABO_ERR_NOT_PD, "K + s2 I not positive definite after jitter retries (pivot %s%d)", "", ctx->hm->chol_info);
  }
}
static int factor_attempts(pcabo_ctx* ctx, int attempt) { return factor_attempts(ctx, attempt, [] { return (int)PCABO_OK; }); }

extern "C" {

int pcabo_ctx_create(int device, int max_n, int max_d, int max_q, pcabo_ctx** out) {
  if (!out) return PCABO_ERR_ARG;
  *out = nullptr;
  if (!ctx_sizes_ok(max_n, max_d, max_q)) return PCABO_ERR_ARG;
  int ndev = 0;
  if (hipGetDeviceCount(&ndev) != hipSuccess || ndev <= 0 || device < 0 || device >= ndev) return PCABO_ERR_HIP;
  pcabo_ctx* ctx = new (std::nothrow) pcabo_ctx();
  if (!ctx) return PCABO_ERR_HIP;
  *out = ctx;
  return ctx_setup(ctx, device, max_n, max_d, max_q, nullptr, nullptr, nullptr);
}

int pcabo_ctx_destroy(pcabo_ctx* ctx) {
  if (!ctx) return PCABO_ERR_ARG;
  if (ctx->in_batch) return set_err(ctx, PCABO_ERR_ARG, "pcabo_ctx_destroy: the context belongs to a batch (pcabo_batch_destroy frees it)%s", "");
  ctx_teardown(ctx);
  delete ctx;
  return PCABO_OK;
}

int pcabo_set_pointer_mode(pcabo_ctx* ctx, int mode) {
  if (!ctx || (mode != PCABO_PTR_HOST && mode != PCABO_PTR_DEVICE)) return PCABO_ERR_ARG;
  ctx->ptr_mode = mode;
  return PCABO_OK;
}

int pcabo_set_option(pcabo_ctx* ctx, int option, int value) {
  if (!ctx) return PCABO_ERR_ARG;
  switch (option) {
    case PCABO_OPT_RESIDENT: ctx->opt_resident = value != 0 && !ctx->in_batch; return PCABO_OK;
    case PCABO_OPT_BESTF_F32: ctx->bestf_f32 = value != 0; return PCABO_OK;
    case PCABO_OPT_GROUP_ACQ: ctx->opt_group_acq = value != 0; return PCABO_OK;
    case PCABO_OPT_HIDDEN_TAIL: ctx->opt_hidden_tail = value != 0; return PCABO_OK;
    default: return set_err(ctx, PCABO_ERR_ARG, "pcabo_set_option: unknown option %s%d", "", option);
  }
}

int pcabo_last_error(pcabo_ctx* ctx, char* buf, int buflen) {
  if (!ctx || !buf || buflen <= 0) return PCABO_ERR_ARG;
  snprintf(buf, buflen, "%s", ctx->err);
  return PCABO_OK;
}

#define STAGE_IN(dst, src, count, T)                                                                        \
  do {                                                                                                      \
    if (ctx->ptr_mode == PCABO_PTR_HOST) {                                                                  \
      HIPCHK(hipMemcpyAsync((void*)(dst), (const void*)(src), (size_t)(count) * sizeof(T), hipMemcpyHostToDevice, ctx->stream)); \
    } else {                                                                                                \
      HIPCHK(hipMemcpyAsync((void*)(dst), (const void*)(src), (size_t)(count) * sizeof(T), hipMemcpyDeviceToDevice, ctx->stream)); \
    }                                                                                                       \
  } while (0)
#define STAGE_OUT(dst, src, count, T)                                                                       \
  do {                                                                                                      \
    HIPCHK(hipMemcpyAsync((void*)(dst), (const void*)(src), (size_t)(count) * sizeof(T),                    \
                          ctx->ptr_mode == PCABO_PTR_HOST ? hipMemcpyDeviceToHost : hipMemcpyDeviceToDevice, ctx->stream)); \
  } while (0)
#define HOST_OUT(dst, src, count, T) \
  HIPCHK(hipMemcpyAsync((void*)(dst), (const void*)(src), (size_t)(count) * sizeof(T), hipMemcpyDeviceToHost, ctx->stream))

struct WpcaInputs { const double *X, *noise, *y; const long long* ranks; };
static int stage_inputs(pcabo_ctx* ctx, const double* X, const double* f, const int64_t* ranks, const double* noise,
                        const double* y, int n, int d, int maximize, WpcaInputs* in) {
  hipStream_t s = ctx->stream;
  const size_t nd = (size_t)n * d;
  if (ctx->ptr_mode == PCABO_PTR_HOST) {
    double* h = ctx->hIn;
    size_t off = 0;
    memcpy(h, X, nd * sizeof(double));                               in->X = ctx->dIn; off += nd;
    if (noise) { memcpy(h + off, noise, nd * sizeof(double));        in->noise = ctx->dIn + off; off += nd; }
    const size_t off_r = off;
    memcpy(h + off, ranks ? (const void*)ranks : (const void*)f, (size_t)n * 8); off += n;
    if (y) { memcpy(h + off, y, (size_t)n * sizeof(double));         in->y = ctx->dIn + off; off += n; }
    HIPCHK(hipMemcpyAsync(ctx->dIn, h, off * sizeof(double), hipMemcpyHostToDevice, s));
    if (ranks) in->ranks = (const long long*)(ctx->dIn + off_r);
    else { launch_rank(s, ctx->dIn + off_r, n, maximize, ctx->dRanks); in->ranks = ctx->dRanks; }
    return PCABO_OK;
  }
  STAGE_IN(ctx->dX, X, nd, double);                                  in->X = ctx->dX;
  if (ranks) { STAGE_IN(ctx->dRanks, ranks, n, long long); }
  else { STAGE_IN(ctx->dF, f, n, double); launch_rank(s, ctx->dF, n, maximize, ctx->dRanks); }
  in->ranks = ctx->dRanks;
  if (noise) { STAGE_IN(ctx->dNoise, noise, nd, double);             in->noise = ctx->dNoise; }
  if (y) { STAGE_IN(ctx->dY, y, n, double);                          in->y = ctx->dY; }
  return PCABO_OK;
}

static int enqueue_wpca(pcabo_ctx* ctx, const WpcaInputs& in, int n, int d, double var_threshold, int n_components) {
  hipStream_t s = ctx->stream;
  const int DP = round_up(d, 16);
  {
    ProfScope ps(ctx, 0, 8.0 * n * d * 2 + 8.0 * n * d, 2.0 * n * d * d + 9.0 * d * d * d + 2.0 * n * d * d);
    launch_wpca_prep(s, in.X, in.ranks, in.noise, n, d, DP, ctx->dWeights, ctx->dDataMean, ctx->dPcaMean, ctx->dWc);
    launch_cov(s, ctx->dWc, n, DP, ctx->dC);
    const double* v0 = (ctx->vprev_d == d) ? ctx->dGbuf[ctx->gcur] : nullptr;
    ctx->gcur ^= 1;
    ctx->dG = ctx->dGbuf[ctx->gcur];
    launch_jacobi(s, ctx->dC, d, DP, v0, ctx->dG, ctx->dLam, ctx->dSweeps, n, var_threshold, n_components, ctx->dComps,
                  ctx->dEvr, ctx->dK, ctx->hm);
    ctx->vprev_d = d;
    launch_project(s, in.X, ctx->dDataMean, ctx->dPcaMean, ctx->dComps, ctx->dK, n, d, ctx->dZ);
  }
  const int rcount = n < d ? n : d;
  HIPCHK(hipMemcpyAsync(ctx->hSmall, ctx->dPcaOut, ((size_t)3 * ctx->max_d + (size_t)rcount * d) * sizeof(double),
                        hipMemcpyDeviceToHost, s));
  HIPCHK(hipEventRecord(ctx->evPca, s));
  return PCABO_OK;
}

static int collect_wpca(pcabo_ctx* ctx, int n, int d, double* data_mean, double* pca_mean, double* comps, double* evr,
                        int* k) {
  HIPCHK(wait_event(ctx->evPca));
  HIPCHK(hipGetLastError());
  const int rcount = n < d ? n : d;
  const double* h = ctx->hSmall;
  const size_t D = ctx->max_d;
  if (data_mean) memcpy(data_mean, h, (size_t)d * sizeof(double));
  if (pca_mean) memcpy(pca_mean, h + D, (size_t)d * sizeof(double));
  if (evr) memcpy(evr, h + 2 * D, (size_t)rcount * sizeof(double));
  if (comps) memcpy(comps, h + 3 * D, (size_t)rcount * d * sizeof(double));
  ctx->d = d; ctx->k = ctx->hm->k;
  ctx->have_wpca = true;
  if (k) *k = ctx->k;
  return PCABO_OK;
}

int pcabo_wpca(pcabo_ctx* ctx, const double* X, const double* f, const int64_t* ranks, int n, int d, int maximize,
               double var_threshold, int n_components, const double* noise, double* data_mean, double* pca_mean,
               double* comps, double* evr, int* k, double* Z) {
  if (!ctx) return PCABO_ERR_ARG;
  if (!X || (!f && !ranks) || n < 2 || n > ctx->max_n || d < 1 || d > ctx->max_d)
    return set_err(ctx, PCABO_ERR_ARG, "pcabo_wpca: bad argument or size beyond context capacity%s", "");
  if (ctx->gp_pending) return set_err(ctx, PCABO_ERR_ARG, "pcabo_wpca: a conditioning is in flight, call pcabo_gp_condition_end first%s", "");
  HIPCHK(hipSetDevice(ctx->device));
  hipStream_t s = ctx->stream;
  WpcaInputs in{nullptr, nullptr, nullptr, nullptr};
  int rc = stage_inputs(ctx, X, f, ranks, noise, nullptr, n, d, maximize, &in);
  if (rc != PCABO_OK) return rc;
  rc = enqueue_wpca(ctx, in, n, d, var_threshold, n_components);
  if (rc != PCABO_OK) return rc;
  ctx->have_gp = false;
  rc = collect_wpca(ctx, n, d, data_mean, pca_mean, comps, evr, k);
  if (rc != PCABO_OK) return rc;
  ctx->n = n;
  if (Z) {
    STAGE_OUT(Z, ctx->dZ, (size_t)n * ctx->k, double);
    HIPCHK(hipStreamSynchronize(s));
  }
  return PCABO_OK;
}

static int enqueue_condition(pcabo_ctx* ctx, const double* y_dev, int n, int k, const double* unb, double lengthscale,
                             double noise, int kernel, double mean_c = 0.0, const double* ard_ls = nullptr) {
  ctx->n = n;
  ctx->NP = round_up(n, PCABO_BS);
  if (k >= 0) { ctx->k = k; ctx->KP = round_up(k, 4); }
  ctx->lengthscale = lengthscale; ctx->noise = noise; ctx->kernel = kernel;
  ctx->have_gp = false;
  ctx->gp_pending = true;
  ctx->zn_recorded = ctx->stream2 && ctx->opt_hidden_tail && !ctx->prof;
  const RowsDH a{ctx->dZ, y_dev, unb, n, k, ctx->KP, k < 0 ? ctx->dK : nullptr, 1.0 / lengthscale, noise, mean_c, kernel, ZB(),
                 {ctx->evBounds, nullptr}, &ctx->cnt_S, &ctx->cnt_dirty, ard_ls, ctx->zn_recorded ? ctx->evZn : nullptr};
  return enqueue_rows_dh(ctx, ctx->stream, a, CondProf{ctx, k < 0 ? ctx->max_d : k});
}

static int stage_gp_inputs(pcabo_ctx* ctx, const double* Z, const double* y, int n, int k, const double* norm_bounds, const double** unb) {
  HIPCHK(hipSetDevice(ctx->device));
  if (Z) STAGE_IN(ctx->dZ, Z, (size_t)n * k, double);
  STAGE_IN(ctx->dY, y, n, double);
  *unb = nullptr;
  if (norm_bounds) {
    HIPCHK(hipMemcpyAsync(ctx->dUserNB, norm_bounds, (size_t)2 * k * sizeof(double), hipMemcpyHostToDevice, ctx->stream));
    *unb = ctx->dUserNB;
  }
  return PCABO_OK;
}

static bool gp_args_ok(const pcabo_ctx* ctx, int n, double lengthscale, double noise, int kernel) {
  return n >= 2 && n <= ctx->max_n && lengthscale > 0.0 && noise >= 0.0 &&
         (kernel == PCABO_KERNEL_MATERN52 || kernel == PCABO_KERNEL_RBF);
}

int pcabo_gp_condition_begin(pcabo_ctx* ctx, const double* Z, const double* y, int n, int k, const double* norm_bounds,
                             double lengthscale, double noise, int kernel) {
  if (!ctx) return PCABO_ERR_ARG;
// ... 196 lines not shown
  return PCABO_OK;
}

int pcabo_acq_bounds(pcabo_ctx* ctx, double* bounds) {
  if (!ctx || !bounds) return PCABO_ERR_ARG;
  if (ctx->wpca_uncollected) { int rc0 = pcabo_wpca_results(ctx, nullptr, nullptr, nullptr, nullptr, nullptr); if (rc0 != PCABO_OK) return rc0; }
  if (ctx->gp_pending) {
    HIPCHK(hipSetDevice(ctx->device));
    HIPCHK(wait_event(ctx->evBounds));
  } else if (!ctx->have_gp) {
    return set_err(ctx, PCABO_ERR_ARG, "pcabo_acq_bounds: call pcabo_gp_condition first%s", "");
  }
  for (int c = 0; c < ctx->k; ++c) { bounds[c] = ctx->hm->acq_lo[c]; bounds[ctx->k + c] = ctx->hm->acq_hi[c]; }
  return PCABO_OK;
}

static const char* acq_arg_error(int acq, double scalar) {
  if (acq != PCABO_ACQ_LOG_EI && acq != PCABO_ACQ_PI && acq != PCABO_ACQ_UCB) return "unknown acquisition code";
  if (acq == PCABO_ACQ_UCB && !(std::isfinite(scalar) && scalar >= 0.0))
    return "PCABO_ACQ_UCB takes kappa = sqrt(beta) in the best_f slot: it must be finite and >= 0";
  return nullptr;
}

static AcqParams make_params(pcabo_ctx* ctx, double best_f, int maximize, int acq, int want_grad) {
  AcqParams p;
  p.best_f = ctx->bestf_f32 ? (double)(float)best_f : best_f;
  p.y_mean = 0.0; p.y_std = 1.0;
  p.inv_ls = 1.0 / ctx->lengthscale;
  p.maximize = maximize ? 1 : 0;
  p.acq = acq;
  p.kernel = ctx->kernel;
  p.want_grad = want_grad;
  return p;
}

static GpModel gp_model(const pcabo_ctx* c) { return {c->n, c->k, c->NP, c->ld, c->dZnT, c->dR, c->dAlpha, c->dBounds4, c->dYstats}; }

static int acq_published(pcabo_ctx* ctx, FlagWait w) {
  if (w == FLAGS_UNPUBLISHED) {
    HIPCHK(hipGetLastError());
    return set_err(ctx, PCABO_ERR_TIMEOUT, "acquisition kernel finished without publishing its results%s", "");
  }
  if (w == FLAGS_LATE) return set_err(ctx, PCABO_ERR_TIMEOUT, "device did not publish acquisition results%s", "");
  return PCABO_OK;
}

static int eval_staged(pcabo_ctx* ctx, int nq, AcqParams& p, bool allow_gemm = true) {
  hipStream_t s = ctx->stream;
  const int k = ctx->k;
  const unsigned long long seq = ++ctx->seq;
  const QueryArgs* qa = nullptr;
  const double* xdev = nullptr;
  if ((size_t)nq * k <= PCABO_QA_MAX) {
    qa = reinterpret_cast<const QueryArgs*>(ctx->hXq);
  } else {
    HIPCHK(hipMemcpyAsync(ctx->dXq, ctx->hXq, (size_t)nq * k * sizeof(double), hipMemcpyHostToDevice, s));
    xdev = ctx->dXq;
  }
  const bool small = nq <= PCABO_INLAUNCH_MAXQ;
  if (!small && !p.want_grad && allow_gemm && score_gemm_possible(nq)) {
    if (!xdev) {
      HIPCHK(hipMemcpyAsync(ctx->dXq, ctx->hXq, (size_t)nq * k * sizeof(double), hipMemcpyHostToDevice, s));
      xdev = ctx->dXq;
    }
    ProfScope ps(ctx, 5, acq_bytes(ctx->n, k, nq, 0), acq_flops(ctx->n, k, nq, 0));
    launch_score(s, xdev, nq, gp_model(ctx), p, ctx->dKS, ctx->dPartial, ctx->dVal);
  } else {
    ProfScope ps(ctx, small ? 4 : 5, acq_bytes(ctx->n, k, nq, p.want_grad), acq_flops(ctx->n, k, nq, p.want_grad));
    launch_acq(s, qa, xdev, nq, gp_model(ctx), p, ctx->dPartial, ctx->dCounters, ctx->dVal, ctx->dGrad, small ? ctx->hVal : nullptr,
               small ? ctx->hGrad : nullptr, small ? ctx->hm : nullptr, seq);
  }
  if (!small) {
    HIPCHK(hipMemcpyAsync(ctx->hVal, ctx->dVal, (size_t)nq * sizeof(double), hipMemcpyDeviceToHost, s));
    if (p.want_grad) HIPCHK(hipMemcpyAsync(ctx->hGrad, ctx->dGrad, (size_t)nq * k * sizeof(double), hipMemcpyDeviceToHost, s));
    HIPCHK(wait_stream(s));
    HIPCHK(hipGetLastError());
    return PCABO_OK;
  }
  return acq_published(ctx, wait_flags(ctx->hm, 0, nq, seq, deadline_in(20), &s));
}

static int score_tail(pcabo_ctx* ctx, int nq, AcqParams& p) {
  hipStream_t s = ctx->stream;
  launch_score_tail(s, nq, gp_model(ctx), p, ctx->dKS, ctx->dPartial, ctx->dVal);
  HIPCHK(hipMemcpyAsync(ctx->hVal, ctx->dVal, (size_t)nq * sizeof(double), hipMemcpyDeviceToHost, s));
  HIPCHK(wait_stream(s));
  HIPCHK(hipGetLastError());
  return PCABO_OK;
}

static int eval_staged_groups(pcabo_ctx* ctx, const int* g0, const int* gn, int ng, AcqParams& p) {
  hipStream_t s = ctx->stream;
  const unsigned long long seq = ++ctx->seq;
  QueryArgs tab;
  unsigned* ent = reinterpret_cast<unsigned*>(tab.x);
  for (int g = 0; g < ng; ++g) ent[g] = ((unsigned)g0[g] << 8) | (unsigned)gn[g];
  {
    int nq = 0;
    for (int g = 0; g < ng; ++g) nq += gn[g];
    ProfScope ps(ctx, 4, acq_bytes(ctx->n, ctx->k, nq, p.want_grad), acq_flops(ctx->n, ctx->k, nq, p.want_grad));
    if (launch_acq_group(s, &tab, ng, ctx->hXq, gp_model(ctx), p, ctx->dPartial, ctx->dCounters + PCABO_GROUP_CNT_OFFSET, ctx->dVal,
                         ctx->dGrad, ctx->hVal, ctx->hGrad, ctx->hm, seq, AcqBatch()) != 0)
      return set_err(ctx, PCABO_ERR_HIP, "the restart-group acquisition kernel could not be launched%s", "");
  }
  HIPCHK(hipGetLastError());
  const auto deadline = deadline_in(20);
  FlagWait w = FLAGS_SET;
  for (int g = 0; g < ng && w == FLAGS_SET; ++g) w = wait_flags(ctx->hm, g0[g], gn[g], seq, deadline, &s);
  return acq_published(ctx, w);
}
static bool group_mode(const pcabo_ctx* ctx, int q, int want_grad) {
  return ctx->opt_group_acq && want_grad && q <= PCABO_INLAUNCH_MAXQ && acq_group_possible(ctx->NP, ctx->k);
}

int pcabo_acq_eval(pcabo_ctx* ctx, const double* Xq, int q, double best_f, int maximize, int acq, double* val,
                   double* grad) {
  if (!ctx) return PCABO_ERR_ARG;
  if (!Xq || !val || q < 1 || q > ctx->max_q)
    return set_err(ctx, PCABO_ERR_ARG, "pcabo_acq_eval: bad argument or q beyond context capacity%s", "");
  if (const char* why = acq_arg_error(acq, best_f)) return set_err(ctx, PCABO_ERR_ARG, "pcabo_acq_eval: %s", why);
  if (!ctx->have_gp) return set_err(ctx, PCABO_ERR_ARG, "pcabo_acq_eval: call pcabo_gp_condition first%s", "");
  HIPCHK(hipSetDevice(ctx->device));
  hipStream_t s = ctx->stream;
  const int k = ctx->k;
  const size_t nx = (size_t)q * k;
  if (ctx->ptr_mode == PCABO_PTR_HOST) memcpy(ctx->hXq, Xq, nx * sizeof(double));
  else {
    HIPCHK(hipMemcpyAsync(ctx->hXq, Xq, nx * sizeof(double), hipMemcpyDeviceToHost, s));
    HIPCHK(hipStreamSynchronize(s));
  }
  AcqParams p = make_params(ctx, best_f, maximize, acq, grad ? 1 : 0);
  int rc;
  if (group_mode(ctx, q, grad != nullptr) && ctx->ptr_mode == PCABO_PTR_HOST) {
    int g0[(PCABO_INLAUNCH_MAXQ + PCABO_GROUP_Q - 1) / PCABO_GROUP_Q], gn[(PCABO_INLAUNCH_MAXQ + PCABO_GROUP_Q - 1) / PCABO_GROUP_Q], ng = 0;
    for (int a = 0; a < q; a += PCABO_GROUP_Q) { g0[ng] = a; gn[ng] = std::min(PCABO_GROUP_Q, q - a); ++ng; }
    rc = eval_staged_groups(ctx, g0, gn, ng, p);
  } else {
    rc = eval_staged(ctx, q, p);
  }
  if (rc != PCABO_OK) return rc;
  if (ctx->ptr_mode == PCABO_PTR_HOST) {
    memcpy(val, ctx->hVal, (size_t)q * sizeof(double));
    if (grad) memcpy(grad, ctx->hGrad, nx * sizeof(double));
  } else {
    HIPCHK(hipMemcpyAsync(val, ctx->dVal, (size_t)q * sizeof(double), hipMemcpyDeviceToDevice, s));
    if (grad) HIPCHK(hipMemcpyAsync(grad, ctx->dGrad, nx * sizeof(double), hipMemcpyDeviceToDevice, s));
    HIPCHK(hipStreamSynchronize(s));
  }
  return PCABO_OK;
}

int pcabo_gp_condition_end_eval(pcabo_ctx* ctx, const double* Xq, int q, double best_f, int maximize, int acq,
                                double* val) {
  if (!ctx) return PCABO_ERR_ARG;
  if (!Xq || !val || q < 1 || q > ctx->max_q)
    return set_err(ctx, PCABO_ERR_ARG, "pcabo_gp_condition_end_eval: bad argument or q beyond context capacity%s", "");
  if (const char* why = acq_arg_error(acq, best_f)) return set_err(ctx, PCABO_ERR_ARG, "pcabo_gp_condition_end_eval: %s", why);
  if (!ctx->gp_pending) return set_err(ctx, PCABO_ERR_ARG, "pcabo_gp_condition_end_eval: no conditioning in flight%s", "");
  if (ctx->wpca_uncollected) { int rc0 = pcabo_wpca_results(ctx, nullptr, nullptr, nullptr, nullptr, nullptr); if (rc0 != PCABO_OK) return rc0; }
  if (q <= PCABO_INLAUNCH_MAXQ || ctx->ptr_mode != PCABO_PTR_HOST) {
    int rc = pcabo_gp_condition_end(ctx);
    if (rc != PCABO_OK) return rc;
    return pcabo_acq_eval(ctx, Xq, q, best_f, maximize, acq, val, nullptr);
  }
  HIPCHK(hipSetDevice(ctx->device));
  memcpy(ctx->hXq, Xq, (size_t)q * ctx->k * sizeof(double));
  AcqParams p = make_params(ctx, best_f, maximize, acq, 0);
  const bool hidden = ctx->zn_recorded && ctx->opt_hidden_tail && !ctx->prof && score_gemm_possible(q);
  ctx->zn_recorded = false;
  int rc;
  if (hidden) {
    HIPCHK(hipStreamWaitEvent(ctx->stream2, ctx->evZn, 0));
    HIPCHK(hipMemcpyAsync(ctx->dXq, ctx->hXq, (size_t)q * ctx->k * sizeof(double), hipMemcpyHostToDevice, ctx->stream2));
    launch_score_ks_only(ctx->stream2, ctx->dXq, q, gp_model(ctx), p, ctx->dKS);
    HIPCHK(hipEventRecord(ctx->evKS, ctx->stream2));
    HIPCHK(hipStreamWaitEvent(ctx->stream, ctx->evKS, 0));
    rc = score_tail(ctx, q, p);
  } else {
    rc = eval_staged(ctx, q, p);
  }
  if (rc != PCABO_OK) { ctx->gp_pending = false; return rc; }
  if (ctx->hm->chol_info != 0) {
    rc = pcabo_gp_condition_end(ctx);
    if (rc != PCABO_OK) return rc;
    rc = hidden ? score_tail(ctx, q, p) : eval_staged(ctx, q, p);
    if (rc != PCABO_OK) return rc;
  } else {
    ctx->gp_pending = false;
    ctx->have_gp = true;
  }
  memcpy(val, ctx->hVal, (size_t)q * sizeof(double));
  return PCABO_OK;
}

int pcabo_logei(pcabo_ctx* ctx, const double* Xq, int q, double best_f, int maximize, double* val, double* grad) {
  return pcabo_acq_eval(ctx, Xq, q, best_f, maximize, PCABO_ACQ_LOG_EI, val, grad);
}

static void server_post(pcabo_ctx* ctx, int cap, int nq, int k, unsigned long long tag) {
  MailPair* m = ctx->dMail;
  const int np = cap * k;
  for (int i = 0; i < np; ++i) put_mail_pair(m + 1 + i, ctx->hXq[i], tag);
  for (int q = 0; q < cap; ++q) put_mail_pair(m + 1 + np + q, q < nq ? 1.0 : 0.0, tag);
  _mm_sfence();
}
static int server_wait(pcabo_ctx* ctx, int nq, unsigned long long tag) {
  if (wait_flags(ctx->hm, 0, nq, tag, deadline_in(3)) != FLAGS_SET)
    return set_err(ctx, PCABO_ERR_TIMEOUT, "resident acquisition kernel did not answer%s", "");
  return PCABO_OK;
}

int pcabo_optimize_acqf(pcabo_ctx* ctx, const double* ics, int num_restarts, int batch_limit, const double* bounds,
                        int maxiter, double best_f, int maximize, int acq, double* cand, double* vals, int* info,
                        int* failed) {
  if (!ctx) return PCABO_ERR_ARG;
  if (!ics || !bounds || !cand || !vals || num_restarts < 1 || batch_limit < 1 || num_restarts > ctx->max_q)
    return set_err(ctx, PCABO_ERR_ARG, "pcabo_optimize_acqf: bad argument%s", "");
  if (const char* why = acq_arg_error(acq, best_f)) return set_err(ctx, PCABO_ERR_ARG, "pcabo_optimize_acqf: %s", why);
  if (!ctx->have_gp) return set_err(ctx, PCABO_ERR_ARG, "pcabo_optimize_acqf: call pcabo_gp_condition first%s", "");
  HIPCHK(hipSetDevice(ctx->device));
  const int k = ctx->k;
  RunRestarts run;
  run.init(ics, bounds, num_restarts, batch_limit, k, maxiter);
  std::vector<RestartGroup>& grp = run.grp;
  const int ngroups = (int)grp.size();
  AcqParams p = make_params(ctx, best_f, maximize, acq, 1);
  auto now = [] { return std::chrono::duration<double>(std::chrono::steady_clock::now().time_since_epoch()).count(); };
  std::vector<char> pending(ngroups, 0);
  auto advance = [&](int gi) {
    if (pending[gi]) pending[gi] = 0;
    else grp[gi].advance();
  };
  OptHelper& hp = ctx->helper;
  const int T = ngroups >= 12 ? std::min(7, 1 + ngroups / 8) : 2;
  if (T > 2) while ((int)ctx->more_helpers.size() < T - 2) ctx->more_helpers.emplace_back(new OptHelper());
  std::vector<OptHelper*> hs;
  if (ngroups > 1) hs.push_back(&hp);
  for (int i = 0; i < T - 2; ++i) hs.push_back(ctx->more_helpers[i].get());
  for (size_t i = 0; i < hs.size(); ++i) {
    const int first = (int)i + 1;
    hs[i]->begin([&, first] { for (int gi = first; gi < ngroups; gi += T) advance(gi); });
  }
  struct Ender { std::vector<OptHelper*>& h; ~Ender() { for (OptHelper* x : h) x->end(); } } ender{hs};
  unsigned round_no = 0;
  std::vector<int> qoff(ngroups, -1);
  int srv_cap = 0;
  struct ServerStop {
    pcabo_ctx* c; int& cap; int k;
    void stop() {
      if (cap <= 0) return;
      server_post(c, cap, 0, k, ++c->seq);
      (void)hipStreamSynchronize(c->stream);
      cap = 0;
    }
    ~ServerStop() { stop(); }
  } server_stop{ctx, srv_cap, k};
  while (true) {
    ++round_no;
    unsigned tickets[8] = {0};
    for (size_t i = 0; i < hs.size(); ++i) {
      tickets[i] = hs[i]->go.load(std::memory_order_relaxed) + 1;
      hs[i]->go.store(tickets[i], std::memory_order_release);
    }
    for (int gi = 0; gi < ngroups; gi += T) advance(gi);
    for (size_t i = 0; i < hs.size(); ++i)
      while (hs[i]->done.load(std::memory_order_acquire) != tickets[i]) __builtin_ia32_pause();
    int nq = 0;
    for (int gi = 0; gi < ngroups; ++gi) {
      qoff[gi] = -1;
      if (!grp[gi].active) continue;
      qoff[gi] = nq;
      memcpy(ctx->hXq + (size_t)nq * k, grp[gi].x.data(), grp[gi].x.size() * sizeof(double));
      nq += grp[gi].nq;
    }
    if (nq == 0) break;
    int rc;
// ... 161 lines not shown


int pcabo_set_profiling(pcabo_ctx* ctx, int enabled) {
  if (!ctx) return PCABO_ERR_ARG;
  HIPCHK(hipSetDevice(ctx->device));
  if (enabled && ctx->pairs.empty()) {
    ctx->pairs.resize(PROF_POOL);
    for (auto& p : ctx->pairs) { HIPCHK(hipEventCreate(&p.a)); HIPCHK(hipEventCreate(&p.b)); p.group = 0; }
  }
  if (!enabled) prof_resolve(ctx);
  if (enabled && !ctx->prof) {
    prof_resolve(ctx);
    double med[2] = {0.0, 0.0};
    for (int mode = 0; mode < 2; ++mode) {
      std::vector<float> r;
      for (int i = 0; i < 64; ++i) {
        HIPCHK(hipEventRecord(ctx->pairs[i].a, ctx->stream));
        if (mode == 1) hipLaunchKernelGGL(k_nop, dim3(1), dim3(64), 0, ctx->stream);
        HIPCHK(hipEventRecord(ctx->pairs[i].b, ctx->stream));
      }
      HIPCHK(hipStreamSynchronize(ctx->stream));
      for (int i = 0; i < 64; ++i) { float ms = 0.f; if (hipEventElapsedTime(&ms, ctx->pairs[i].a, ctx->pairs[i].b) == hipSuccess) r.push_back(ms); }
      if (!r.empty()) { std::sort(r.begin(), r.end()); med[mode] = r[r.size() / 2]; }
    }
    ctx->prof_pair_ms = med[0];
    ctx->prof_empty_ms = med[1];
  }
  ctx->prof = enabled != 0;
  return PCABO_OK;
}

int pcabo_get_profile_calibration(pcabo_ctx* ctx, double* pair_ms, double* empty_kernel_ms) {
  if (!ctx) return PCABO_ERR_ARG;
  if (pair_ms) *pair_ms = ctx->prof_pair_ms;
  if (empty_kernel_ms) *empty_kernel_ms = ctx->prof_empty_ms;
  return PCABO_OK;
}

int pcabo_get_profile(pcabo_ctx* ctx, int which, double* ms, int64_t* launches, double* bytes, double* flops) {
  if (!ctx || which < 0 || which >= PROF_GROUPS) return PCABO_ERR_ARG;
  HIPCHK(hipSetDevice(ctx->device));
  prof_resolve(ctx);
  if (ms) *ms = ctx->prof_ms[which];
  if (launches) *launches = ctx->prof_launches[which];
  if (bytes) *bytes = ctx->prof_bytes[which];
  if (flops) *flops = ctx->prof_flops[which];
  return PCABO_OK;
}

int pcabo_reset_profile(pcabo_ctx* ctx) {
  if (!ctx) return PCABO_ERR_ARG;
  prof_resolve(ctx);
  for (int i = 0; i < PROF_GROUPS; ++i) { ctx->prof_ms[i] = 0.0; ctx->prof_launches[i] = 0; ctx->prof_bytes[i] = 0.0; ctx->prof_flops[i] = 0.0; }
  return PCABO_OK;
}


}


struct pcabo_batch {
  int device = 0, B = 0, max_n = 0, max_d = 0, max_q = 0;
  hipStream_t stream = nullptr;
  hipEvent_t evPca = nullptr, evBounds = nullptr;
  char *dSlab = nullptr, *hSlab = nullptr;
  size_t zs = 0, hzs = 0;
  std::vector<pcabo_ctx*> ctx;
  std::vector<char> active;
  int n = 0, d = 0, NP = 0;
  bool wpca_uncollected = false, gp_pending = false, have_gp = false;
  double lengthscale = 0.0, noise = 0.0;
  int kernel = 0;
  const double *fitZ = nullptr, *fitY = nullptr, *fitUnb = nullptr;
  bool fitted = false;
  int fit_rounds = 0;
  int gcur = 0, vprev_d = 0;
  int cnt_S = 0; bool cnt_dirty = true;
  bool prof = false; hipEvent_t pev[6] = {nullptr, nullptr, nullptr, nullptr, nullptr, nullptr};
  bool group_acq = true;
  size_t in_stride_x = 0, in_stride_noise = 0, in_stride_y = 0;
  bool score_enqueued = false;
  bool imap_enqueued = false;
  bool opt_enqueued = false; int opt_restarts = 0, opt_limit = 0; std::vector<int> opt_act;
  int dev_lbfgsb = 0;
  std::vector<unsigned> dbg_branches; std::vector<double> dbg_group_out; int dbg_groups = 0;
  unsigned *dOptTab = nullptr, *hOptTab = nullptr;
  int G = 0;
  std::vector<hipStream_t> gstream;
  GangPool pool;
  std::atomic<unsigned long long> seq{0};
  char err[512] = {0};
};

static int bset_err(pcabo_batch* b, int code, const char* fmt, const char* a = "", int v = 0) {
  if (b) snprintf(b->err, sizeof(b->err), fmt, a, v);
  return code;
}
#define BHIPCHK(call)                                                                        \
  do {                                                                                       \
    hipError_t e_ = (call);                                                                  \
    if (e_ != hipSuccess) return bset_err(batch, PCABO_ERR_HIP, "HIP error: %s (line %d)", hipGetErrorString(e_), __LINE__); \
  } while (0)

static ZB batch_zb(const pcabo_batch* b) { ZB z; z.B = b->B; z.zs = b->zs; z.hzs = b->hzs; return z; }
static const double* batch_hyp(const pcabo_batch* b) { return b->fitted ? b->ctx[0]->dHyp : nullptr; }

static void batch_free(pcabo_batch* batch) {
  (void)hipSetDevice(batch->device);
  batch->pool.shutdown();
  if (batch->stream) (void)hipStreamSynchronize(batch->stream);
  for (pcabo_ctx* c : batch->ctx) if (c) { ctx_teardown(c); delete c; }
  for (hipStream_t s : batch->gstream) if (s) (void)hipStreamDestroy(s);
  if (batch->evPca) (void)hipEventDestroy(batch->evPca);
  if (batch->evBounds) (void)hipEventDestroy(batch->evBounds);
  for (hipEvent_t e : batch->pev) if (e) (void)hipEventDestroy(e);
  if (batch->dSlab) (void)hipFree(batch->dSlab);
  if (batch->hSlab) (void)hipHostFree(batch->hSlab);
  if (batch->dOptTab) (void)hipFree(batch->dOptTab);
  if (batch->hOptTab) (void)hipHostFree(batch->hOptTab);
  if (batch->stream) (void)hipStreamDestroy(batch->stream);
  delete batch;
}

static int batch_enqueue_condition(pcabo_batch* batch, const double* Z, const double* y, const double* unb, int n, int d, int k,
                                   double lengthscale, double gp_noise, int kernel) {
  pcabo_ctx* c0 = batch->ctx[0];
  hipStream_t s = batch->stream;
  const ZB zb = batch_zb(batch);
  const int NP = round_up(n, PCABO_BS);
  const RowsDH a{Z, y, unb, n, -1, 0, c0->dK, 1.0 / lengthscale, gp_noise, 0.0, kernel, zb,
                 {batch->evBounds, k < 0 ? nullptr : batch->evPca}, &batch->cnt_S, &batch->cnt_dirty};
  const int rc = enqueue_rows_dh(c0, s, a, [&](int phase) {
    if (batch->prof) (void)hipEventRecord(batch->pev[phase], s);
    if (phase == 4 && batch->dev_lbfgsb) launch_rt_build(s, c0->dR, n, NP, c0->ld, c0->dGram, zb);
    return (int)PCABO_OK;
  });
  if (rc != PCABO_OK) return bset_err(batch, rc, "%s", c0->err);
  BHIPCHK(hipGetLastError());
  batch->n = n; batch->d = d; batch->NP = NP;
  batch->lengthscale = lengthscale; batch->noise = gp_noise; batch->kernel = kernel;
  batch->wpca_uncollected = k < 0; batch->gp_pending = true; batch->have_gp = false;
  batch->fitZ = Z; batch->fitY = y; batch->fitUnb = unb; batch->fitted = false;
  for (pcabo_ctx* c : batch->ctx) {
    c->n = n; c->d = d; c->NP = NP; c->lengthscale = lengthscale; c->noise = gp_noise; c->kernel = kernel;
    c->have_gp = false; c->have_wpca = false; c->gp_pending = false; c->wpca_uncollected = false;
    if (k >= 0) { c->k = k; c->KP = round_up(k, 4); }
    else { c->gcur = batch->gcur; c->dG = c->dGbuf[c->gcur]; c->vprev_d = d; }
    c->cnt_S = batch->cnt_S; c->cnt_dirty = false;
  }
  return PCABO_OK;
}

extern "C" {

int pcabo_batch_create(int device, int B, int max_n, int max_d, int max_q, pcabo_batch** out) {
  if (!out) return PCABO_ERR_ARG;
  *out = nullptr;
  if (B < 1 || B > 4096 || !ctx_sizes_ok(max_n, max_d, max_q)) return PCABO_ERR_ARG;
  int ndev = 0;
  if (hipGetDeviceCount(&ndev) != hipSuccess || ndev <= 0 || device < 0 || device >= ndev) return PCABO_ERR_HIP;
  pcabo_batch* batch = new (std::nothrow) pcabo_batch();
  if (!batch) return PCABO_ERR_HIP;
  *out = batch;
  batch->device = device; batch->B = B; batch->max_n = max_n; batch->max_d = max_d; batch->max_q = max_q;
  BHIPCHK(hipSetDevice(device));
  BHIPCHK(hipStreamCreateWithFlags(&batch->stream, hipStreamNonBlocking));
  BHIPCHK(hipEventCreateWithFlags(&batch->evPca, hipEventDisableTiming));
  BHIPCHK(hipEventCreateWithFlags(&batch->evBounds, hipEventDisableTiming));
  {
    pcabo_ctx probe;
    probe.max_n = max_n; probe.max_d = max_d; probe.max_q = max_q;
    probe.NPcap = round_up(max_n, PCABO_BS); probe.DPcap = round_up(max_d, 16); probe.KPcap = round_up(max_d, 4);
    probe.Scap = probe.NPcap / PCABO_SLAB;
    batch->zs = carve_device(&probe, nullptr);
    batch->hzs = carve_host(&probe, nullptr);
  }
  BHIPCHK(hipMalloc((void**)&batch->dSlab, batch->zs * (size_t)B));
  BHIPCHK(hipHostMalloc((void**)&batch->hSlab, batch->hzs * (size_t)B, hipHostMallocDefault));
  memset(batch->hSlab, 0, batch->hzs * (size_t)B);
  BHIPCHK(hipMalloc((void**)&batch->dOptTab, (size_t)B * PCABO_INLAUNCH_MAXQ * sizeof(unsigned)));
  BHIPCHK(hipHostMalloc((void**)&batch->hOptTab, (size_t)B * PCABO_INLAUNCH_MAXQ * sizeof(unsigned), hipHostMallocDefault));
  BHIPCHK(hipMemsetAsync(batch->dSlab, 0, batch->zs * (size_t)B, batch->stream));
  BHIPCHK(hipStreamSynchronize(batch->stream));
  batch->ctx.assign(B, nullptr);
  batch->active.assign(B, 1);
  for (int b = 0; b < B; ++b) {
    pcabo_ctx* c = new (std::nothrow) pcabo_ctx();
    if (!c) return bset_err(batch, PCABO_ERR_HIP, "out of memory%s", "");
    batch->ctx[b] = c;
    int rc = ctx_setup(c, device, max_n, max_d, max_q, batch->dSlab + batch->zs * (size_t)b,
                       batch->hSlab + batch->hzs * (size_t)b, batch->stream);
    c->batch_index = b;
    if (rc != PCABO_OK) return bset_err(batch, rc, "context %s%d of the batch could not be set up", "", b);
    if (c->region_bytes != batch->zs || c->hregion_bytes != batch->hzs)
      return bset_err(batch, PCABO_ERR_ARG, "internal: layout mismatch%s", "");
  }
  int T = std::min(8, (int)std::thread::hardware_concurrency() - 2);
  T = std::max(1, std::min(T, std::min(B, 32)));
  batch->G = T;
  batch->gstream.assign((size_t)T, nullptr);
  for (size_t g = 0; g < batch->gstream.size(); ++g) BHIPCHK(hipStreamCreateWithFlags(&batch->gstream[g], hipStreamNonBlocking));
  batch->pool.start(T);
  for (pcabo_ctx* c : batch->ctx) c->opt_group_acq = batch->group_acq;
  batch->seq.store(((unsigned long long)(getpid() & 0xffff) << 44) + (1ull << 43));
  return PCABO_OK;
}

int pcabo_batch_destroy(pcabo_batch* batch) {
  if (!batch) return PCABO_ERR_ARG;
  batch_free(batch);
  return PCABO_OK;
}

int pcabo_batch_set_workers(pcabo_batch* batch, int workers) {
  if (!batch || workers < 1) return PCABO_ERR_ARG;
  BHIPCHK(hipSetDevice(batch->device));
  const int T = std::max(1, std::min(workers, std::min(batch->B, 32)));
  if (T == batch->G) return PCABO_OK;
  batch->pool.shutdown();
  BHIPCHK(hipStreamSynchronize(batch->stream));
  for (hipStream_t& s : batch->gstream) if (s) { (void)hipStreamSynchronize(s); (void)hipStreamDestroy(s); s = nullptr; }
  batch->gstream.assign((size_t)T, nullptr);
  for (size_t g = 0; g < batch->gstream.size(); ++g) BHIPCHK(hipStreamCreateWithFlags(&batch->gstream[g], hipStreamNonBlocking));
  batch->G = T;
  batch->pool.start(T);
  return PCABO_OK;
}

int pcabo_batch_set_option(pcabo_batch* batch, int option, int value) {
  if (!batch) return PCABO_ERR_ARG;
  if (option == PCABO_OPT_DEVICE_LBFGSB) {
    if (value < 0 || value > 2) return bset_err(batch, PCABO_ERR_ARG, "pcabo_batch_set_option: PCABO_OPT_DEVICE_LBFGSB takes 0, 1 or 2 (%s%d)", "", value);
    if (value != 0 && batch->dev_lbfgsb == 0) for (pcabo_ctx* c : batch->ctx) if (c->have_gp) c->rt_stale = true;
    batch->dev_lbfgsb = value;
    return PCABO_OK;
  }
  if (option != PCABO_OPT_GROUP_ACQ) return bset_err(batch, PCABO_ERR_ARG, "pcabo_batch_set_option: unknown option %s%d", "", option);
  batch->group_acq = value != 0;
  for (pcabo_ctx* c : batch->ctx) c->opt_group_acq = batch->group_acq;
  return PCABO_OK;
}

int pcabo_batch_set_profiling(pcabo_batch* batch, int enabled) {
  if (!batch) return PCABO_ERR_ARG;
  BHIPCHK(hipSetDevice(batch->device));
  if (enabled && !batch->pev[0]) for (auto& e : batch->pev) BHIPCHK(hipEventCreate(&e));
  batch->prof = enabled != 0;
  return PCABO_OK;
}
int pcabo_batch_get_profile(pcabo_batch* batch, double* ms) {
  if (!batch || !ms || !batch->prof) return PCABO_ERR_ARG;
  BHIPCHK(hipSetDevice(batch->device));
  BHIPCHK(hipEventSynchronize(batch->pev[4]));
  for (int i = 0; i < 4; ++i) { float t = 0.f; BHIPCHK(hipEventElapsedTime(&t, batch->pev[i], batch->pev[i + 1])); ms[i] = t; }
  return PCABO_OK;
}

int pcabo_batch_set_active(pcabo_batch* batch, const int* active) {
  if (!batch || !active) return PCABO_ERR_ARG;
  for (int b = 0; b < batch->B; ++b) batch->active[b] = active[b] != 0;
  return PCABO_OK;
}

int pcabo_batch_last_error(pcabo_batch* batch, char* buf, int buflen) {
  if (!batch || !buf || buflen <= 0) return PCABO_ERR_ARG;
  snprintf(buf, buflen, "%s", batch->err);
  return PCABO_OK;
}

pcabo_ctx* pcabo_batch_ctx(pcabo_batch* batch, int b) {
  if (!batch || b < 0 || b >= batch->B) return nullptr;
  return batch->ctx[b];
}

int pcabo_batch_set_input_strides(pcabo_batch* batch, size_t x_stride, size_t noise_stride, size_t y_stride) {
  if (!batch) return PCABO_ERR_ARG;
  batch->in_stride_x = x_stride; batch->in_stride_noise = noise_stride; batch->in_stride_y = y_stride;
  return PCABO_OK;
}

int pcabo_batch_wpca_gp_condition_begin(pcabo_batch* batch, const double* X, const int64_t* ranks, const double* noise,
                                        const double* y, int n, int d, int maximize, double var_threshold,
                                        int n_components, double lengthscale, double gp_noise, int kernel) {
  (void)maximize;
  if (!batch) return PCABO_ERR_ARG;
  pcabo_ctx* c0 = batch->ctx[0];
  if (!X || !ranks || !y || n < 2 || n > batch->max_n || d < 1 || d > batch->max_d || !gp_args_ok(c0, n, lengthscale, gp_noise, kernel))
    return bset_err(batch, PCABO_ERR_ARG, "pcabo_batch_wpca_gp_condition_begin: bad argument or size beyond the batch's capacity%s", "");
  if (batch->gp_pending) return bset_err(batch, PCABO_ERR_ARG, "pcabo_batch_wpca_gp_condition_begin: a conditioning is in flight%s", "");
  BHIPCHK(hipSetDevice(batch->device));
  hipStream_t s = batch->stream;
  const int B = batch->B;
  const size_t nd = (size_t)n * d;
  const size_t off_noise = nd, off_r = noise ? 2 * nd : nd, off_y = off_r + n, total = off_y + n;
  const size_t sx = batch->in_stride_x ? batch->in_stride_x : nd, sn = batch->in_stride_noise ? batch->in_stride_noise : nd;
  const size_t sy = batch->in_stride_y ? batch->in_stride_y : (size_t)n;
  if (sx < nd || sn < nd || sy < (size_t)n)
    return bset_err(batch, PCABO_ERR_ARG, "pcabo_batch_wpca_gp_condition_begin: an input stride is smaller than a run's block%s", "");
  for (int b = 0; b < B; ++b) {
    double* h = batch->ctx[b]->hIn;
    memcpy(h, X + (size_t)b * sx, nd * sizeof(double));
    if (noise) memcpy(h + off_noise, noise + (size_t)b * sn, nd * sizeof(double));
    memcpy(h + off_r, ranks + (size_t)b * n, (size_t)n * 8);
    memcpy(h + off_y, y + (size_t)b * sy, (size_t)n * sizeof(double));
  }
  BHIPCHK(hipMemcpy2DAsync(c0->dIn, batch->zs, c0->hIn, batch->hzs, total * sizeof(double), B, hipMemcpyHostToDevice, s));
  const double* inX = c0->dIn;
  const double* inNoise = noise ? c0->dIn + off_noise : nullptr;
  const long long* inRanks = reinterpret_cast<const long long*>(c0->dIn + off_r);
  const double* inY = c0->dIn + off_y;
  const ZB zb = batch_zb(batch);
  const int DP = round_up(d, 16);
  if (batch->prof) (void)hipEventRecord(batch->pev[0], s);
  launch_wpca_prep(s, inX, inRanks, inNoise, n, d, DP, c0->dWeights, c0->dDataMean, c0->dPcaMean, c0->dWc, zb);
  launch_cov(s, c0->dWc, n, DP, c0->dC, zb);
  const double* v0 = (batch->vprev_d == d) ? c0->dGbuf[batch->gcur] : nullptr;
  batch->gcur ^= 1;
  launch_jacobi(s, c0->dC, d, DP, v0, c0->dGbuf[batch->gcur], c0->dLam, c0->dSweeps, n, var_threshold, n_components,
                c0->dComps, c0->dEvr, c0->dK, c0->hm, zb);
  batch->vprev_d = d;
  launch_project(s, inX, c0->dDataMean, c0->dPcaMean, c0->dComps, c0->dK, n, d, c0->dZ, zb);
  const int rcount = n < d ? n : d;
  BHIPCHK(hipMemcpy2DAsync(c0->hSmall, batch->hzs, c0->dPcaOut, batch->zs,
                           ((size_t)3 * batch->max_d + (size_t)rcount * d) * sizeof(double), B, hipMemcpyDeviceToHost, s));
  BHIPCHK(hipEventRecord(batch->evPca, s));
  return batch_enqueue_condition(batch, c0->dZ, inY, nullptr, n, d, -1, lengthscale, gp_noise, kernel);
}

int pcabo_batch_gp_condition_begin(pcabo_batch* batch, const double* Z, const double* y, int n, int k, const double* norm_bounds,
                                   double lengthscale, double gp_noise, int kernel) {
  if (!batch) return PCABO_ERR_ARG;
  pcabo_ctx* c0 = batch->ctx[0];
  if (!Z || !y || n < 2 || n > batch->max_n || k < 1 || k > batch->max_d || !gp_args_ok(c0, n, lengthscale, gp_noise, kernel))
    return bset_err(batch, PCABO_ERR_ARG, "pcabo_batch_gp_condition_begin: bad argument or size beyond the batch's capacity%s", "");
  if (batch->gp_pending) return bset_err(batch, PCABO_ERR_ARG, "pcabo_batch_gp_condition_begin: a conditioning is in flight%s", "");
  BHIPCHK(hipSetDevice(batch->device));
  hipStream_t s = batch->stream;
  const int B = batch->B;
  const size_t nk = (size_t)n * k, off_y = nk, total = nk + n;
  const size_t sx = batch->in_stride_x ? batch->in_stride_x : nk, sy = batch->in_stride_y ? batch->in_stride_y : (size_t)n;
  if (sx < nk || sy < (size_t)n)
    return bset_err(batch, PCABO_ERR_ARG, "pcabo_batch_gp_condition_begin: an input stride is smaller than a run's block%s", "");
  for (int b = 0; b < B; ++b) {
    pcabo_ctx* c = batch->ctx[b];
    memcpy(c->hIn, Z + (size_t)b * sx, nk * sizeof(double));
    memcpy(c->hIn + off_y, y + (size_t)b * sy, (size_t)n * sizeof(double));
    c->hm->k = k;
    if (norm_bounds) memcpy(c->hSmall, norm_bounds, (size_t)2 * k * sizeof(double));
  }
  BHIPCHK(hipMemcpy2DAsync(c0->dIn, batch->zs, c0->hIn, batch->hzs, total * sizeof(double), B, hipMemcpyHostToDevice, s));
  BHIPCHK(hipMemcpy2DAsync(c0->dK, batch->zs, &c0->hm->k, batch->hzs, sizeof(int), B, hipMemcpyHostToDevice, s));
  if (norm_bounds)
    BHIPCHK(hipMemcpy2DAsync(c0->dUserNB, batch->zs, c0->hSmall, batch->hzs, (size_t)2 * k * sizeof(double), B, hipMemcpyHostToDevice, s));
  if (batch->prof) (void)hipEventRecord(batch->pev[0], s);
  return batch_enqueue_condition(batch, c0->dIn, c0->dIn + off_y, norm_bounds ? c0->dUserNB : nullptr, n, k, k, lengthscale, gp_noise, kernel);
}

int pcabo_batch_wpca_results(pcabo_batch* batch, double* data_mean, double* pca_mean, double* comps, double* evr, int* k) {
  if (!batch) return PCABO_ERR_ARG;
  if (!batch->wpca_uncollected && batch->n == 0) return bset_err(batch, PCABO_ERR_ARG, "pcabo_batch_wpca_results: nothing enqueued%s", "");
  BHIPCHK(hipSetDevice(batch->device));
  BHIPCHK(wait_event(batch->evPca));
  BHIPCHK(hipGetLastError());
  const int n = batch->n, d = batch->d, rcount = n < d ? n : d;
  const size_t D = batch->max_d;
  for (int b = 0; b < batch->B; ++b) {
    pcabo_ctx* c = batch->ctx[b];
    const double* h = c->hSmall;
    if (data_mean) memcpy(data_mean + (size_t)b * d, h, (size_t)d * sizeof(double));
    if (pca_mean) memcpy(pca_mean + (size_t)b * d, h + D, (size_t)d * sizeof(double));
    if (evr) memcpy(evr + (size_t)b * d, h + 2 * D, (size_t)rcount * sizeof(double));
    if (comps) memcpy(comps + (size_t)b * d * d, h + 3 * D, (size_t)rcount * d * sizeof(double));
    c->k = c->hm->k; c->KP = round_up(c->k, 4); c->have_wpca = true;
    if (k) k[b] = c->k;
  }
  batch->wpca_uncollected = false;
  return PCABO_OK;
}

int pcabo_batch_acq_bounds(pcabo_batch* batch, double* bounds) {
  if (!batch || !bounds) return PCABO_ERR_ARG;
  if (batch->wpca_uncollected) { int rc = pcabo_batch_wpca_results(batch, nullptr, nullptr, nullptr, nullptr, nullptr); if (rc != PCABO_OK) return rc; }
  if (batch->gp_pending) {
    BHIPCHK(hipSetDevice(batch->device));
    BHIPCHK(wait_event(batch->evBounds));
  } else if (!batch->have_gp) {
    return bset_err(batch, PCABO_ERR_ARG, "pcabo_batch_acq_bounds: no conditioning enqueued%s", "");
  }
  for (int b = 0; b < batch->B; ++b) {
    const pcabo_ctx* c = batch->ctx[b];
    double* o = bounds + (size_t)b * 2 * batch->max_d;
    for (int j = 0; j < c->k; ++j) { o[j] = c->hm->acq_lo[j]; o[c->k + j] = c->hm->acq_hi[j]; }
  }
  return PCABO_OK;
}

static int batch_max_k(const pcabo_batch* batch) {
  int km = 1;
// ... 754 lines not shown
```

### para-ortho-pca-bo_amd/csrc/pcabo_internal.h

```cpp
#pragma once
#include <hip/hip_runtime.h>
#include <stdint.h>
#include <type_traits>

#define PCABO_BS 64
#define PCABO_SLAB 16
#define PCABO_MAXD 128
#define PCABO_TLD 66

#define PCABO_QA_MAX 416
#define PCABO_CNT_DONE 0x3fff
#define PCABO_INLAUNCH_MAXQ 32

typedef double double4_t __attribute__((ext_vector_type(4)));
struct QueryArgs { double x[PCABO_QA_MAX]; };
struct alignas(16) MailPair { double v; unsigned long long tag; };
static inline __host__ __device__ unsigned long long mail_mix(unsigned long long vbits) {
  const unsigned int lo = (unsigned int)vbits, hi = (unsigned int)(vbits >> 32);
  return (unsigned long long)((lo ^ hi ^ (hi >> 11)) & 0xFFFFFFu);
}
#define PCABO_MAIL_PAIRS (1 + PCABO_QA_MAX + PCABO_INLAUNCH_MAXQ + 1)
#define PCABO_SERVER_TIMEOUT_TICKS 200000000ull

#ifdef __HIPCC__
// ... 132 lines not shown
  if (T == 1) return dpp_get<0x4E, 0xf>(v);
  if (T == 2) return dpp_get<0x141, 0xf>(dpp_get<0x1B, 0xf>(v));
  return dpp_get<0x128, 0xf>(v);
}
template <int T>
__device__ inline double swap_add(double a, double b) {
  unsigned alo = (unsigned)__double2loint(a), ahi = (unsigned)__double2hiint(a);
  unsigned blo = (unsigned)__double2loint(b), bhi = (unsigned)__double2hiint(b);
  if (T == 4) {
    const auto lo = __builtin_amdgcn_permlane16_swap(alo, blo, false, false);
    const auto hi = __builtin_amdgcn_permlane16_swap(ahi, bhi, false, false);
    alo = lo[0]; blo = lo[1]; ahi = hi[0]; bhi = hi[1];
  } else {
    const auto lo = __builtin_amdgcn_permlane32_swap(alo, blo, false, false);
    const auto hi = __builtin_amdgcn_permlane32_swap(ahi, bhi, false, false);
    alo = lo[0]; blo = lo[1]; ahi = hi[0]; bhi = hi[1];
  }
  return __hiloint2double((int)ahi, (int)alo) + __hiloint2double((int)bhi, (int)blo);
}
template <int T>
__device__ inline double pair_level(double a, double b, int lane) {
  if (T >= 4) return swap_add<T>(a, b);
  const bool hi = (lane >> T) & 1;
  return (hi ? b : a) + lane_xor<T>(hi ? a : b);
}
template <int T>
__device__ inline double single_level(double v) {
  if (T >= 4) return swap_add<T>(v, v);
  return v + lane_xor<T>(v);
}
__host__ __device__ constexpr int wave_multi_live(int n, int t) { return (n + (1 << t) - 1) >> t; }
template <int T, int N>
__device__ inline void wave_multi_level(double* v, int lane) {
  constexpr int M = wave_multi_live(N, T);
#pragma unroll
  for (int i = 0; i < M / 2; ++i) v[i] = pair_level<T>(v[2 * i], v[2 * i + 1], lane);
  if (M & 1) v[M / 2] = single_level<T>(v[M - 1]);
}
template <int N>
__device__ inline void wave_sum_multi(double* v, int lane) {
  static_assert(N >= 1 && N <= 64, "one value per lane at the end");
  wave_multi_level<0, N>(v, lane); wave_multi_level<1, N>(v, lane); wave_multi_level<2, N>(v, lane);
  wave_multi_level<3, N>(v, lane); wave_multi_level<4, N>(v, lane); wave_multi_level<5, N>(v, lane);
}
template <int N>
__device__ inline int wave_multi_index(int lane) {
  int slot = 0;
#pragma unroll
  for (int t = 5; t >= 0; --t) {
    const int m = wave_multi_live(N, t);
    slot = slot < m / 2 ? 2 * slot + ((lane >> t) & 1) : m - 1;
  }
  return slot;
}
template <int N>
__device__ inline int wave_multi_owner(int lane) {
  int slot = 0;
  bool first = true;
#pragma unroll
  for (int t = 5; t >= 0; --t) {
    const int m = wave_multi_live(N, t);
    if (slot < m / 2) slot = 2 * slot + ((lane >> t) & 1);
    else { slot = m - 1; first = first && !((lane >> t) & 1); }
  }
  return first ? slot : -1;
}
__host__ __device__ constexpr int wave_multi_lane(int n, int i, int t = 0) {
  return t == 6 ? 0
       : (i < wave_multi_live(n, t) / 2 * 2 ? ((i & 1) << t) + wave_multi_lane(n, i / 2, t + 1)
                                            : wave_multi_lane(n, wave_multi_live(n, t) / 2, t + 1));
}
__device__ inline double read_lane(double v, int lane) {
  return __hiloint2double(__builtin_amdgcn_readlane(__double2hiint(v), lane),
                          __builtin_amdgcn_readlane(__double2loint(v), lane));
}
#endif

void launch_rank(hipStream_t s, const double* f, int n, int maximize, long long* ranks);
#define PCABO_HYP_INV_LS 0
#define PCABO_HYP_NOISE 1
#define PCABO_HYP_MEAN_C 2
#define PCABO_HYP_WORDS 4
struct ZB { int B = 1; size_t zs = 0, hzs = 0; const double* hyp = nullptr; };
void launch_wpca_prep(hipStream_t s, const double* X, const long long* ranks, const double* noise, int n, int d,
                      int DP, double* weights, double* data_mean, double* pca_mean, double* Wc, ZB zb = ZB());
void launch_cov(hipStream_t s, const double* Wc, int n, int DP, double* C, ZB zb = ZB());
void launch_jacobi(hipStream_t s, const double* C, int d, int DP, const double* V0, double* G, double* lam, int* sweeps,
                   int n, double var_threshold, int n_components, double* comps, double* evr, int* k_dev, HostMirror* hm,
                   ZB zb = ZB());
void launch_project(hipStream_t s, const double* X, const double* data_mean, const double* pca_mean,
                    const double* comps, const int* k_dev, int n, int d, double* Z, ZB zb = ZB());
void launch_zstats(hipStream_t s, const double* Z, const double* y, int n, int k, const double* user_norm_bounds,
                   double* bounds4 , double* zn_mean, double* ystats,
                   double* ys, HostMirror* hm, const int* k_dev = nullptr, ZB zb = ZB(),
                   double mean_c = 0.0,
                   const double* ard_ls = nullptr);
void launch_znorm(hipStream_t s, const double* Z, int n, int k, int NP, int KP, int ld, const double* bounds4,
                  const double* zn_mean, double inv_ls, double* ZnT, double* AT, double* nrm,
                  const int* k_dev = nullptr, ZB zb = ZB());
void launch_gram(hipStream_t s, const double* AT, const double* nrm, int n, int NP, int KP, int ld, double noise,
                 int kernel, double* K, const int* k_dev = nullptr, double* K2 = nullptr, int* info_reset = nullptr,
                 ZB zb = ZB());
void launch_add_jitter(hipStream_t s, double* K, int n, int ld, double jitter);
int launch_cholesky(hipStream_t s, double* L, int NP, int ld, int* info, double* diag_scratch, ZB zb = ZB(), double* R_folded = nullptr);
bool chol_step_form(int NP, ZB zb);
void launch_trinv_drain(hipStream_t s, const double* L, int NP, int ld, double* R);
void launch_trinv(hipStream_t s, const double* L, int NP, int ld, double* R, ZB zb = ZB());
void launch_chol_panel(hipStream_t s, double* L, int p, int nblocks, int ld, int* info, double* diag_scratch, ZB zb = ZB());
int launch_chol_steps(hipStream_t s, double* L, int NP, int ld, int* info, double* diag_scratch , ZB zb = ZB(),
                      double* R = nullptr);
void launch_trinv_diag_w(hipStream_t s, const double* L, int nblk, int ld, double* R, ZB zb = ZB());
void launch_alpha(hipStream_t s, const double* R, const double* ys, int n, int NP, int ld, double* tmp, double* alpha,
                  ZB zb = ZB());
void launch_mll_grad(hipStream_t s, const double* R, const double* AT, const double* nrm, const double* alpha, const double* L,
                     const double* ys, int n, int NP, int KP, int ld, double* partial, double* out,
                     const int* k_dev = nullptr, ZB zb = ZB());
void launch_mll_grad_ard(hipStream_t s, const double* R, const double* AT, const double* nrm, const double* alpha, const double* L,
                         const double* ys, int n, int NP, int KP, int ld, double* partial, double* out);
void launch_acq(hipStream_t s, const QueryArgs* qa, const double* Xq, int q, const GpModel& m, AcqParams p, double* partial,
                unsigned int* counters, double* val, double* grad, double* host_val, double* host_grad, HostMirror* hm,
                unsigned long long seq,
                MailPair* dev_mail = nullptr, MailPair* part_pairs = nullptr,
                AcqBatch ab = AcqBatch(), int B = 1, int table_entries = 0);
#define PCABO_GROUP_Q 5
#define PCABO_GROUP_CNT_OFFSET 8192
bool acq_group_possible(int NP, int k);
int launch_acq_group(hipStream_t st, const QueryArgs* tab, int entries, const double* Xq, const GpModel& m, AcqParams p,
                     double* partial, unsigned int* counters, double* val, double* grad, double* host_val, double* host_grad,
                     HostMirror* hm, unsigned long long seq, AcqBatch ab);
bool score_gemm_possible(int q);
void launch_score(hipStream_t st, const double* Xq, int q, const GpModel& m, AcqParams p, double* KS, double* partial, double* val,
                  AcqBatch ab = AcqBatch(), int B = 1);
void launch_score_ks_only(hipStream_t st, const double* Xq, int q, const GpModel& m, AcqParams p, double* KS);
void launch_score_tail(hipStream_t st, int q, const GpModel& m, AcqParams p, const double* KS, double* partial, double* val);
bool acq_server_possible(int q, int n, int k, int NP);
int acq_slabs(int NP);
void launch_inverse_map(hipStream_t s, const double* z, const double* comps, const double* data_mean,
                        const double* pca_mean, int k, int d, double* x, const int* k_dev = nullptr, ZB zb = ZB(),
                        double* host_x = nullptr, HostMirror* hm = nullptr, unsigned long long seq = 0);
void launch_rt_build(hipStream_t s, const double* R, int n, int NP, int ld, double* RT, ZB zb = ZB());
bool lbfgsb_device_possible(int NP, int kmax, int batch_limit);
int launch_lbfgsb_group(hipStream_t st, const unsigned* table, int entries, int mode, int num_restarts, int maxiter, const GpModel& m,
                        const double* Xq, const double* RT, const double* bestf, const int* k_dev, double inv_ls,
                        int maximize, int acq, int kernel, double* out_x, double* out_v, size_t zs,
                        const double* hyp = nullptr,
                        int batch_limit = PCABO_GROUP_Q);
```

### para-ortho-pca-bo_amd/pcabo/_native.py

```python
from __future__ import annotations

import ctypes as C
import math
import os
from typing import Optional

import numpy as np

ABI_VERSION = 2
KERNEL_MATERN52, KERNEL_RBF = 0, 1
ACQ_LOG_EI, ACQ_PI, ACQ_UCB = 0, 1, 2
PTR_HOST, PTR_DEVICE = 0, 1
OPT_RESIDENT, OPT_BESTF_F32, OPT_GROUP_ACQ, OPT_DEVICE_LBFGSB = 0, 1, 2, 3
OPT_HIDDEN_TAIL = 5
FIT_THETA0 = (0.006737946999085467, 0.0, 0.0)
FIT_TASK_NOT_PD = -2
PROFILE_GROUPS = ("wpca", "gram", "cholesky", "root_inverse_alpha", "acq_partial", "acq_large_batches")

HW_QUEUES_ENV, HW_QUEUES_WANTED = "GPU_MAX_HW_QUEUES", 16


def hw_queues_advice(streams: int) -> Optional[str]:
    try:
        have = int(os.environ.get(HW_QUEUES_ENV, "4"))
    except ValueError:
        have = 4
    if have >= streams:
        return None
    return (f"{HW_QUEUES_ENV}={os.environ.get(HW_QUEUES_ENV, 'unset (default 4)')}: {streams} streams of this batch will share "
            f"hardware queues and their kernels serialise; set {HW_QUEUES_ENV}={max(HW_QUEUES_WANTED, streams)} in the environment "
            "before the process makes its first GPU call")


_LIB_PATH = os.path.join(os.path.dirname(os.path.abspath(__file__)), "..", "lib", "libpcabo.so")

EXPORTS = [
    "pcabo_abi_version", "pcabo_device_count", "pcabo_ctx_create", "pcabo_ctx_destroy",
    "pcabo_set_pointer_mode", "pcabo_set_option", "pcabo_last_error", "pcabo_wpca", "pcabo_gp_condition", "pcabo_gp_condition_begin",
    "pcabo_gp_condition_end", "pcabo_gp_condition_end_eval", "pcabo_wpca_gp_condition_begin", "pcabo_wpca_results",
    "pcabo_gp_mll", "pcabo_gp_fit", "pcabo_gp_mll_ard", "pcabo_gp_fit_ard",
    "pcabo_acq_bounds",
    "pcabo_acq_eval", "pcabo_logei", "pcabo_optimize_acqf", "pcabo_inverse_map", "pcabo_get_gp_state",
    "pcabo_get_gram", "pcabo_lbfgsb_minimize", "pcabo_lbfgsb_set_vector_kernels", "pcabo_lbfgsb_set_sum_order", "pcabo_sobol_scramble", "pcabo_sobol_draw", "pcabo_sobol_draw_rows", "pcabo_torch_randint2", "pcabo_torch_multinomial_rows", "pcabo_boltzmann_pick_rows", "pcabo_set_profiling",
    "pcabo_get_profile", "pcabo_get_profile_calibration", "pcabo_reset_profile",
    "pcabo_batch_create", "pcabo_batch_destroy", "pcabo_batch_last_error", "pcabo_batch_ctx",
    "pcabo_batch_wpca_gp_condition_begin", "pcabo_batch_wpca_results", "pcabo_batch_acq_bounds",
    "pcabo_batch_gp_condition_end_eval", "pcabo_batch_optimize_acqf", "pcabo_batch_inverse_map", "pcabo_batch_device_acq_eval",
    "pcabo_batch_busy", "pcabo_batch_gp_condition_end_eval_begin", "pcabo_batch_gp_condition_end_eval_end",
    "pcabo_batch_optimize_acqf_begin", "pcabo_batch_optimize_acqf_end", "pcabo_batch_inverse_map_begin", "pcabo_batch_inverse_map_end",
    "pcabo_batch_set_input_strides", "pcabo_batch_gp_condition_begin",
    "pcabo_batch_gp_mll", "pcabo_batch_gp_fit", "pcabo_batch_gp_fit_rounds",
    "pcabo_batch_set_profiling", "pcabo_batch_get_profile", "pcabo_batch_set_active", "pcabo_batch_set_workers", "pcabo_batch_set_option",
    "pcabo_device_lbfgsb_limits",
    "pcabo_bbob_table_doubles", "pcabo_bbob_create", "pcabo_bbob_destroy", "pcabo_bbob_eval",
    "pcabo_comm_unique_id", "pcabo_comm_create", "pcabo_gather_best", "pcabo_comm_last_error", "pcabo_comm_destroy",
]


class PcaboError(RuntimeError):
    def __init__(self, code: int, msg: str):
        super().__init__(f"libpcabo error {code}: {msg}")
        self.code = code


def lib_path() -> str:
    return os.path.normpath(os.environ.get("PCABO_LIB") or _LIB_PATH)


def _load() -> C.CDLL:
    path = lib_path()
    if not os.path.exists(path):
        raise ImportError(
            f"{path} not found: build it with `python -c 'import __graft_entry__ as g; g.build()'` "
            "(or `make -C para-ortho-pca-bo_amd/csrc`).  There is no CPU fallback for the HIP path.")
    lib = C.CDLL(path)
    lib.pcabo_abi_version.restype = C.c_int
    if lib.pcabo_abi_version() != ABI_VERSION:
        raise ImportError(f"{path}: ABI version mismatch")
    dp, ip, vp = C.POINTER(C.c_double), C.POINTER(C.c_int), C.c_void_p
    lib.pcabo_device_count.restype = C.c_int
    lib.pcabo_ctx_create.argtypes = [C.c_int, C.c_int, C.c_int, C.c_int, C.POINTER(vp)]
    lib.pcabo_ctx_destroy.argtypes = [vp]
    lib.pcabo_set_pointer_mode.argtypes = [vp, C.c_int]
    lib.pcabo_set_option.argtypes = [vp, C.c_int, C.c_int]
    lib.pcabo_last_error.argtypes = [vp, C.c_char_p, C.c_int]
    lib.pcabo_wpca.argtypes = [vp, vp, vp, vp, C.c_int, C.c_int, C.c_int, C.c_double, C.c_int, vp,
                               vp, vp, vp, vp, ip, vp]
    lib.pcabo_gp_condition.argtypes = [vp, vp, vp, C.c_int, C.c_int, vp, C.c_double, C.c_double, C.c_int]
    lib.pcabo_gp_condition_begin.argtypes = lib.pcabo_gp_condition.argtypes
    lib.pcabo_gp_condition_end.argtypes = [vp]
    lib.pcabo_gp_mll.argtypes = [vp, vp, vp, C.c_int, C.c_int, vp, C.c_int, vp, dp, vp]
    lib.pcabo_gp_fit.argtypes = [vp, vp, vp, C.c_int, C.c_int, vp, C.c_int, vp, dp, vp]
    lib.pcabo_gp_mll_ard.argtypes = lib.pcabo_gp_mll.argtypes
    lib.pcabo_gp_fit_ard.argtypes = lib.pcabo_gp_fit.argtypes
    lib.pcabo_wpca_results.argtypes = [vp, vp, vp, vp, vp, ip]
    lib.pcabo_gp_condition_end_eval.argtypes = [vp, vp, C.c_int, C.c_double, C.c_int, C.c_int, vp]
    lib.pcabo_wpca_gp_condition_begin.argtypes = [vp, vp, vp, vp, C.c_int, C.c_int, C.c_int, C.c_double, C.c_int, vp,
                                                  vp, C.c_double, C.c_double, C.c_int, vp, vp, vp, vp, ip]
    lib.pcabo_acq_bounds.argtypes = [vp, vp]
    lib.pcabo_acq_eval.argtypes = [vp, vp, C.c_int, C.c_double, C.c_int, C.c_int, vp, vp]
    lib.pcabo_logei.argtypes = [vp, vp, C.c_int, C.c_double, C.c_int, vp, vp]
    lib.pcabo_optimize_acqf.argtypes = [vp, vp, C.c_int, C.c_int, vp, C.c_int, C.c_double, C.c_int, C.c_int,
                                        vp, vp, vp, ip]
    lib.pcabo_inverse_map.argtypes = [vp, vp, vp]
    lib.pcabo_get_gp_state.argtypes = [vp, vp, vp, vp, vp, vp]
    lib.pcabo_get_gram.argtypes = [vp, vp]
    lib.pcabo_sobol_scramble.argtypes = [vp, vp, C.c_int]
    lib.pcabo_sobol_draw.argtypes = [vp, vp, C.c_int, C.c_int, vp, vp, vp]
    lib.pcabo_sobol_draw_rows.argtypes = [vp, vp, vp, C.c_int, C.c_int, vp, C.c_longlong, vp]
    lib.pcabo_set_profiling.argtypes = [vp, C.c_int]
    lib.pcabo_get_profile.argtypes = [vp, C.c_int, dp, C.POINTER(C.c_int64), dp, dp]
    lib.pcabo_reset_profile.argtypes = [vp]
    lib.pcabo_get_profile_calibration.argtypes = [vp, dp, dp]
    lib.pcabo_lbfgsb_set_vector_kernels.argtypes = [C.c_int]
    lib.pcabo_batch_create.argtypes = [C.c_int, C.c_int, C.c_int, C.c_int, C.c_int, C.POINTER(vp)]
    lib.pcabo_comm_unique_id.argtypes = [C.c_char_p]
    lib.pcabo_comm_create.argtypes = [C.c_char_p, C.c_int, C.c_int, C.c_int, C.POINTER(vp)]
    lib.pcabo_gather_best.argtypes = [vp, vp, C.c_int, vp]
    lib.pcabo_comm_last_error.argtypes = [vp, C.c_char_p, C.c_int]
    lib.pcabo_comm_destroy.argtypes = [vp]
    lib.pcabo_batch_destroy.argtypes = [vp]
    lib.pcabo_batch_set_workers.argtypes = [vp, C.c_int]
    lib.pcabo_batch_set_option.argtypes = [vp, C.c_int, C.c_int]
    lib.pcabo_batch_last_error.argtypes = [vp, C.c_char_p, C.c_int]
    lib.pcabo_batch_ctx.argtypes = [vp, C.c_int]
    lib.pcabo_batch_wpca_gp_condition_begin.argtypes = [vp, vp, vp, vp, vp, C.c_int, C.c_int, C.c_int, C.c_double, C.c_int,
                                                        C.c_double, C.c_double, C.c_int]
    lib.pcabo_batch_wpca_results.argtypes = [vp, vp, vp, vp, vp, vp]
    lib.pcabo_batch_acq_bounds.argtypes = [vp, vp]
    lib.pcabo_batch_gp_condition_end_eval.argtypes = [vp, vp, C.c_int, vp, C.c_int, C.c_int, vp, vp]
    lib.pcabo_batch_optimize_acqf.argtypes = [vp, vp, C.c_int, C.c_int, vp, C.c_int, vp, C.c_int, C.c_int, vp, vp, vp, vp, vp]
    lib.pcabo_batch_inverse_map.argtypes = [vp, vp, vp]
    lib.pcabo_batch_device_acq_eval.argtypes = [vp, vp, C.c_int, vp, C.c_int, C.c_int, vp, vp]
    lib.pcabo_batch_busy.argtypes = [vp]
    lib.pcabo_batch_gp_condition_end_eval_begin.argtypes = [vp, vp, C.c_int, vp, C.c_int, C.c_int]
    lib.pcabo_batch_gp_condition_end_eval_end.argtypes = [vp, vp, C.c_int, vp, C.c_int, C.c_int, vp, vp]
    lib.pcabo_batch_optimize_acqf_begin.argtypes = [vp, vp, C.c_int, C.c_int, vp, C.c_int, vp, C.c_int, C.c_int]
    lib.pcabo_batch_optimize_acqf_end.argtypes = [vp, C.c_int, C.c_int, vp, vp, vp, vp, vp]
    lib.pcabo_batch_inverse_map_begin.argtypes = [vp, vp]
    lib.pcabo_batch_set_input_strides.argtypes = [vp, C.c_size_t, C.c_size_t, C.c_size_t]
    lib.pcabo_batch_gp_condition_begin.argtypes = [vp, vp, vp, C.c_int, C.c_int, vp, C.c_double, C.c_double, C.c_int]
    lib.pcabo_batch_inverse_map_end.argtypes = [vp, vp]
    lib.pcabo_batch_set_profiling.argtypes = [vp, C.c_int]
    lib.pcabo_batch_set_active.argtypes = [vp, vp]
    lib.pcabo_batch_get_profile.argtypes = [vp, vp]
    lib.pcabo_batch_gp_mll.argtypes = [vp, vp, vp, vp, vp]
    lib.pcabo_batch_gp_fit.argtypes = [vp, vp, vp, vp, vp]
    lib.pcabo_batch_gp_fit_rounds.argtypes = [vp]
    for name in EXPORTS:
        getattr(lib, name).restype = C.c_int
    lib.pcabo_batch_ctx.restype = vp
    return lib


LIB = _load()
FG_CALLBACK = C.CFUNCTYPE(C.c_double, C.POINTER(C.c_double), C.POINTER(C.c_double), C.c_void_p)
LIB.pcabo_lbfgsb_minimize.argtypes = [
    C.c_int, C.c_void_p, C.c_void_p, C.c_void_p, FG_CALLBACK, C.c_void_p, C.c_int, C.c_double, C.c_double,
    C.c_int, C.c_int, C.c_int, C.POINTER(C.c_double), C.POINTER(C.c_int), C.POINTER(C.c_int), C.POINTER(C.c_int)]


LIB.pcabo_debug_lbfgsb_branch_names.argtypes = [C.c_char_p, C.c_int]
LIB.pcabo_debug_lbfgsb_branches.argtypes = [C.c_void_p, C.c_int]


def _branch_names():
    buf = C.create_string_buffer(2048)
    count = LIB.pcabo_debug_lbfgsb_branch_names(buf, 2048)
    names = tuple(buf.value.decode().split(","))
    assert len(names) == count
    return names


LBFGSB_BRANCHES = _branch_names()
DEVICE_GROUP_FIELDS = ("niter", "nfev", "warnflag", "task", "status", "evaluations", "ties", "evaluation_cap")
if hasattr(LIB, "pcabo_debug_batch_lbfgsb_branches"):
    LIB.pcabo_debug_batch_lbfgsb_branches.argtypes = [C.c_void_p, C.c_void_p, C.c_int]
    LIB.pcabo_debug_batch_lbfgsb_device_out.argtypes = [C.c_void_p, C.c_void_p, C.c_int]


def device_count() -> int:
    return int(LIB.pcabo_device_count())


def device_lbfgsb_limits():
    a, b, c = C.c_int(0), C.c_int(0), C.c_int(0)
    LIB.pcabo_device_lbfgsb_limits(C.byref(a), C.byref(b), C.byref(c))
    return a.value, b.value, c.value


def _ptr(a: Optional[np.ndarray]):
    return None if a is None else a.ctypes.data


def _f64(a, shape=None) -> np.ndarray:
    a = np.ascontiguousarray(a, dtype=np.float64)
    if shape is not None:
        a = a.reshape(shape)
    return a


class Context:

    def __init__(self, max_n: int, max_d: int, max_q: int = 512, device: int = 0):
        self._h = C.c_void_p()
        rc = LIB.pcabo_ctx_create(int(device), int(max_n), int(max_d), int(max_q), C.byref(self._h))
        if rc != 0:
            msg = self._err() if self._h else "no usable HIP device (the HIP path has no CPU fallback)"
            if self._h:
                LIB.pcabo_ctx_destroy(self._h)
                self._h = C.c_void_p()
            raise PcaboError(rc, msg)
        self.max_n, self.max_d, self.max_q, self.device = max_n, max_d, max_q, device
        self.n = self.d = self.k = 0

    def _err(self) -> str:
        buf = C.create_string_buffer(512)
        LIB.pcabo_last_error(self._h, buf, 512)
        return buf.value.decode(errors="replace")

    def _chk(self, rc: int) -> None:
        if rc != 0:
            raise PcaboError(rc, self._err())

    def set_option(self, option: int, value: int) -> None:
        self._chk(LIB.pcabo_set_option(self._h, int(option), int(value)))

    def match_best_f_dtype(self, best_f) -> None:
        f32 = 0 if isinstance(best_f, np.floating) and best_f.dtype == np.float64 else 1
        if getattr(self, "_bestf_f32", 1) != f32:
            self.set_option(OPT_BESTF_F32, f32)
            self._bestf_f32 = f32

    def close(self) -> None:
        if getattr(self, "_h", None):
            LIB.pcabo_ctx_destroy(self._h)
            self._h = C.c_void_p()

    def __del__(self):
        try:
            self.close()
        except Exception:
            pass

    def wpca(self, X, f=None, ranks=None, maximize=False, var_threshold=0.95, n_components=0, noise=None,
             want_Z=True, want_full=True):
        X = _f64(X)
        n, d = X.shape
        f_a = None if f is None else _f64(f, (n,))
        r_a = None if ranks is None else np.ascontiguousarray(ranks, dtype=np.int64).reshape(n)
        nz = None if noise is None else _f64(noise, (n, d))
        rc_ = min(n, d)
        data_mean, pca_mean = np.empty(d), np.empty(d)
        comps = np.empty((rc_, d)) if want_full else None
        evr = np.empty(rc_) if want_full else None
        k = C.c_int(0)
        Z = np.empty((n, d)) if want_Z else None
        self._chk(LIB.pcabo_wpca(self._h, _ptr(X), _ptr(f_a), _ptr(r_a), n, d, int(bool(maximize)),
                                 float(var_threshold), int(n_components), _ptr(nz), _ptr(data_mean), _ptr(pca_mean),
                                 _ptr(comps), _ptr(evr), C.byref(k), _ptr(Z)))
        self.n, self.d, self.k = n, d, k.value
        if want_Z:
            Z = Z.reshape(-1)[: n * k.value].reshape(n, k.value).copy()
# ... 80 lines not shown

    @staticmethod
    def _theta_ard(theta, k):
        if theta is None:
            return np.array(FIT_THETA0[:2] + (0.0,) * k, dtype=np.float64)
        return _f64(theta, (2 + k,)).copy()

    def gp_mll_ard(self, y, theta, Z=None, norm_bounds=None, kernel=KERNEL_MATERN52):
        y, Z, k, nb = self._fit_args(y, Z, norm_bounds)
        th = self._theta_ard(theta, k)
        loss, g = C.c_double(0.0), np.empty(2 + k)
        self._chk(LIB.pcabo_gp_mll_ard(self._h, _ptr(Z), _ptr(y), y.shape[0], k, _ptr(nb), int(kernel), _ptr(th),
                                       C.byref(loss), _ptr(g)))
        self.n, self.k = y.shape[0], k
        return {**self._fit_result_ard(th, loss.value), "grad": g}

    def gp_fit_ard(self, y, theta0=None, Z=None, norm_bounds=None, kernel=KERNEL_MATERN52):
        y, Z, k, nb = self._fit_args(y, Z, norm_bounds)
        th = self._theta_ard(theta0, k)
        loss, info = C.c_double(0.0), np.zeros(4, dtype=np.int32)
        self._chk(LIB.pcabo_gp_fit_ard(self._h, _ptr(Z), _ptr(y), y.shape[0], k, _ptr(nb), int(kernel), _ptr(th),
                                       C.byref(loss), _ptr(info)))
        self.n, self.k = y.shape[0], k
        return {**self._fit_result_ard(th, loss.value), "iterations": int(info[0]), "evaluations": int(info[1]),
                "warnflag": int(info[2]), "task": int(info[3])}

    def gp_wait(self) -> None:
        self._chk(LIB.pcabo_gp_condition_end(self._h))
        self._keep = None

    def gp_wait_eval(self, Xq, best_f, maximize=False, acq=ACQ_LOG_EI) -> np.ndarray:
        Xq = _f64(Xq).reshape(-1, self.k)
        q = Xq.shape[0]
        val = np.empty(q)
        self._chk(LIB.pcabo_gp_condition_end_eval(self._h, _ptr(Xq), q, float(best_f), int(bool(maximize)), int(acq),
                                                  _ptr(val)))
        self._keep = None
        return val

    def acq_bounds(self) -> np.ndarray:
        b = np.empty((2, self.k))
        self._chk(LIB.pcabo_acq_bounds(self._h, _ptr(b)))
        return b

    def acq_eval(self, Xq, best_f, maximize=False, acq=ACQ_LOG_EI, grad=True):
        Xq = _f64(Xq).reshape(-1, self.k)
        q = Xq.shape[0]
        val = np.empty(q)
        g = np.empty((q, self.k)) if grad else None
        self._chk(LIB.pcabo_acq_eval(self._h, _ptr(Xq), q, float(best_f), int(bool(maximize)), int(acq), _ptr(val),
                                     _ptr(g)))
        return (val, g) if grad else val

    def optimize_acqf(self, ics, bounds, best_f, maximize=False, acq=ACQ_LOG_EI, batch_limit=5, maxiter=200):
        ics = _f64(ics).reshape(-1, self.k)
        nr = ics.shape[0]
        bounds = _f64(bounds, (2, self.k))
        cand = np.empty((nr, self.k))
        vals = np.empty(nr)
        ng = (nr + batch_limit - 1) // batch_limit
        info = np.zeros((ng, 4), dtype=np.int32)
        failed = C.c_int(0)
        self._chk(LIB.pcabo_optimize_acqf(self._h, _ptr(ics), nr, int(batch_limit), _ptr(bounds), int(maxiter),
                                          float(best_f), int(bool(maximize)), int(acq), _ptr(cand), _ptr(vals),
                                          _ptr(info), C.byref(failed)))
        return cand, vals, info, bool(failed.value)

    def inverse_map(self, z) -> np.ndarray:
        z = _f64(z).reshape(-1)
        x = np.empty(self.d)
        self._chk(LIB.pcabo_inverse_map(self._h, _ptr(z), _ptr(x)))
        return x

    def gp_state(self):
        n, k = self.n, self.k
        L, R, alpha, ys, nb = np.empty((n, n)), np.empty((n, n)), np.empty(n), np.empty(2), np.empty((2, k))
        self._chk(LIB.pcabo_get_gp_state(self._h, _ptr(L), _ptr(R), _ptr(alpha), _ptr(ys), _ptr(nb)))
        return {"L": np.tril(L), "R": np.tril(R), "alpha": alpha, "y_mean": ys[0], "y_std": ys[1], "norm_bounds": nb}

    def gram(self) -> np.ndarray:
        K = np.empty((self.n, self.n))
        self._chk(LIB.pcabo_get_gram(self._h, _ptr(K)))
        return K

    def set_profiling(self, on: bool) -> None:
        self._chk(LIB.pcabo_set_profiling(self._h, int(bool(on))))

    def reset_profile(self) -> None:
        self._chk(LIB.pcabo_reset_profile(self._h))

    def profile(self) -> dict:
        out = {}
        for i, name in enumerate(PROFILE_GROUPS):
            ms, cnt, by, fl = C.c_double(0), C.c_int64(0), C.c_double(0), C.c_double(0)
            self._chk(LIB.pcabo_get_profile(self._h, i, C.byref(ms), C.byref(cnt), C.byref(by), C.byref(fl)))
            out[name] = {"ms": ms.value, "launches": cnt.value, "bytes": by.value, "flops": fl.value}
        return out

    def profile_calibration(self) -> dict:
        a, b = C.c_double(0), C.c_double(0)
        self._chk(LIB.pcabo_get_profile_calibration(self._h, C.byref(a), C.byref(b)))
        return {"pair_ms": a.value, "empty_kernel_ms": b.value}


class _BorrowedContext(Context):

    def __init__(self, handle, max_n, max_d, max_q, device):
        self._h = C.c_void_p(handle)
        self.max_n, self.max_d, self.max_q, self.device = max_n, max_d, max_q, device
        self.n = self.d = self.k = 0

    def close(self) -> None:
        self._h = C.c_void_p()


class Batch:

    def __init__(self, B: int, max_n: int, max_d: int, max_q: int = 512, device: int = 0, workers: int = 0,
                 group_acq: bool = True, device_lbfgsb: int = 0):
        self._h = C.c_void_p()
        rc = LIB.pcabo_batch_create(int(device), int(B), int(max_n), int(max_d), int(max_q), C.byref(self._h))
        if rc != 0:
            msg = self._err() if self._h else "no usable HIP device (the HIP path has no CPU fallback)"
            if self._h:
                LIB.pcabo_batch_destroy(self._h)
                self._h = C.c_void_p()
            raise PcaboError(rc, msg)
        self.B, self.max_n, self.max_d, self.max_q, self.device = B, max_n, max_d, max_q, device
        self.n = self.d = 0
        self.k = np.zeros(B, dtype=np.int32)
        self.ctx = [_BorrowedContext(LIB.pcabo_batch_ctx(self._h, b), max_n, max_d, max_q, device) for b in range(B)]
        if workers:
            self.set_workers(workers)
        if not group_acq:
            self._chk(LIB.pcabo_batch_set_option(self._h, OPT_GROUP_ACQ, 0))
        if device_lbfgsb:
            self._chk(LIB.pcabo_batch_set_option(self._h, OPT_DEVICE_LBFGSB, int(device_lbfgsb)))
        self.device_lbfgsb = int(device_lbfgsb)
        advice = hw_queues_advice(min(B, int(workers) if workers else 8) + 2)
        if advice:
            import warnings
            warnings.warn(advice, RuntimeWarning, stacklevel=2)

    def set_workers(self, workers: int) -> None:
        self._chk(LIB.pcabo_batch_set_workers(self._h, int(workers)))

    def _err(self) -> str:
        buf = C.create_string_buffer(512)
        LIB.pcabo_batch_last_error(self._h, buf, 512)
        return buf.value.decode(errors="replace")

    def _chk(self, rc: int) -> None:
        if rc != 0:
            raise PcaboError(rc, self._err())

    def close(self) -> None:
        if getattr(self, "_h", None):
            for c in self.ctx:
                c.close()
            LIB.pcabo_batch_destroy(self._h)
            self._h = C.c_void_p()

    def __del__(self):
        try:
            self.close()
        except Exception:
            pass

    @staticmethod
    def _block(a, row):
        if a is None:
            return None, 0
        a = np.asarray(a, dtype=np.float64)
        item = a.itemsize
        inner_ok = all(a.strides[i] == item * int(np.prod(a.shape[i + 1:])) for i in range(1, a.ndim))
        if a.dtype == np.float64 and inner_ok and a.strides[0] % item == 0 and a.strides[0] // item >= row:
            return a, a.strides[0] // item
        return np.ascontiguousarray(a, dtype=np.float64), row

    def wpca_gp_condition_begin(self, X, ranks, noise, y, maximize=False, var_threshold=0.95, n_components=0,
                                lengthscale=0.6931471805599453, gp_noise=0.006737946999085467, kernel=KERNEL_MATERN52):
        X = np.asarray(X, dtype=np.float64)
        B, n, d = X.shape
        assert B == self.B
        ranks = np.ascontiguousarray(ranks, dtype=np.int64).reshape(B, n)
        y = np.asarray(y, dtype=np.float64).reshape(B, n)
        X, sx = self._block(X, n * d)
        nz, sn = self._block(noise, n * d)
        y, sy = self._block(y, n)
        strides = (0 if sx == n * d else sx, 0 if sn == n * d else sn, 0 if sy == n else sy)
        if strides != getattr(self, "_in_strides", (0, 0, 0)):
            self._chk(LIB.pcabo_batch_set_input_strides(self._h, *strides))
            self._in_strides = strides
        self._chk(LIB.pcabo_batch_wpca_gp_condition_begin(self._h, _ptr(X), _ptr(ranks), _ptr(nz), _ptr(y), n, d,
                                                          int(bool(maximize)), float(var_threshold), int(n_components),
                                                          float(lengthscale), float(gp_noise), int(kernel)))
        self.n, self.d = n, d

    def gp_condition_begin(self, Z, y, norm_bounds=None, lengthscale=0.6931471805599453, gp_noise=0.006737946999085467,
                           kernel=KERNEL_MATERN52):
        Z = np.asarray(Z, dtype=np.float64)
        B, n, k = Z.shape
        assert B == self.B
        y = np.asarray(y, dtype=np.float64).reshape(B, n)
        Z, sx = self._block(Z, n * k)
        y, sy = self._block(y, n)
        strides = (0 if sx == n * k else sx, 0, 0 if sy == n else sy)
        if strides != getattr(self, "_in_strides", (0, 0, 0)):
            self._chk(LIB.pcabo_batch_set_input_strides(self._h, *strides))
            self._in_strides = strides
        nb = None if norm_bounds is None else _f64(norm_bounds, (2, k))
        self._chk(LIB.pcabo_batch_gp_condition_begin(self._h, _ptr(Z), _ptr(y), n, k, _ptr(nb), float(lengthscale), float(gp_noise),
                                                     int(kernel)))
        self.n, self.d = n, k
        self.k = np.full(B, k, dtype=np.int32)
        for c in self.ctx:
            c.n, c.d, c.k = n, k, k

    def wpca_results(self):
        B, n, d = self.B, self.n, self.d
        rc_ = min(n, d)
        dm, pm, comps, evr = np.empty((B, d)), np.empty((B, d)), np.empty((B, d, d)), np.empty((B, d))
        k = np.zeros(B, dtype=np.int32)
        self._chk(LIB.pcabo_batch_wpca_results(self._h, _ptr(dm), _ptr(pm), _ptr(comps), _ptr(evr), _ptr(k)))
        self.k = k
        for b, c in enumerate(self.ctx):
# ... 298 lines not shown
```

Baseline: 404.6 BO iterations/s.

## Fuse weighted-PCA prep into covariance kernel and write results directly to host

Adds a fused k_wpca_cov kernel that computes rank weights, data and weighted means, and the covariance tile via f64 MFMA in one launch per tile. This replaces the single-block prep kernel plus the separate cov kernel. Kernels also now write small outputs (means, comps, evr, scores, info) straight into host-mapped buffers, which removes some device-to-host memcpys and stream stalls. The cost is redundant per-tile recomputation of weights and means, plus reliance on contraction-off helpers to keep results bit-identical.

```diff
diff --git a/include/pcabo.h b/include/pcabo.h
--- a/include/pcabo.h
+++ b/include/pcabo.h
@@ -34,7 +34,8 @@
 
 enum { PCABO_OPT_RESIDENT = 0, PCABO_OPT_BESTF_F32 = 1, PCABO_OPT_GROUP_ACQ = 2,
        PCABO_OPT_DEVICE_LBFGSB = 3 ,
-       PCABO_OPT_HIDDEN_TAIL = 5  };
+       PCABO_OPT_HIDDEN_TAIL = 5 ,
+       PCABO_OPT_FUSED_WPCA = 6 };
 int pcabo_set_option(pcabo_ctx* ctx, int option, int value);
 
 int pcabo_wpca(pcabo_ctx* ctx, const double* X, const double* f, const int64_t* ranks, int n, int d,
diff --git a/para-ortho-pca-bo_amd/csrc/kernels_acq.hip b/para-ortho-pca-bo_amd/csrc/kernels_acq.hip
--- a/para-ortho-pca-bo_amd/csrc/kernels_acq.hip
+++ b/para-ortho-pca-bo_amd/csrc/kernels_acq.hip
@@ -684,7 +684,8 @@
 __global__ __launch_bounds__(256) void k_acq_combine(const double* __restrict__ partial, int q_total, int S, int k,
                                                      const double* __restrict__ bounds4,
                                                      const double* __restrict__ ystats, AcqParams p,
-                                                     double* __restrict__ val, double* __restrict__ grad, AcqBatch ab) {
+                                                     double* __restrict__ val, double* __restrict__ grad, AcqBatch ab,
+                                                     double* __restrict__ host_val) {
   if (ab.zs) {
     const unsigned run_ = blockIdx.z;
     partial = zrun(partial, ab.zs, run_); bounds4 = zrun(bounds4, ab.zs, run_); ystats = zrun(ystats, ab.zs, run_);
@@ -694,7 +695,7 @@
   }
   const int q = blockIdx.x * 4 + (threadIdx.x >> 6);
   if (q < q_total)
-    acq_finish_query(partial + (size_t)q * S * PSTRIDE, S, k, q, bounds4, ystats, p, val, grad, nullptr, nullptr,
+    acq_finish_query(partial + (size_t)q * S * PSTRIDE, S, k, q, bounds4, ystats, p, val, grad, host_val, nullptr,
                      threadIdx.x & 63);
 }
 
@@ -1249,13 +1250,14 @@
   hipLaunchKernelGGL(k_score_ks_only, dim3(njb, (q + SC_QB - 1) / SC_QB, 1), dim3(256), 0, st, Xq, q, m.n, m.k, m.NP, m.ld, m.ZnT,
                      m.bounds4, p, KS);
 }
-void launch_score_tail(hipStream_t st, int q, const GpModel& m, AcqParams p, const double* KS, double* partial, double* val) {
+void launch_score_tail(hipStream_t st, int q, const GpModel& m, AcqParams p, const double* KS, double* partial, double* val,
+                       double* host_val) {
   const int S = m.NP / 64, njb = (m.NP + 255) / 256;
   hipLaunchKernelGGL(k_score_mu, dim3(njb, (q + SC_QB - 1) / SC_QB, 1), dim3(256), 0, st, KS, q, m.n, m.ld, m.alpha, partial, S);
   hipLaunchKernelGGL(k_score_gemm, dim3(S, (q + 63) / 64, 1), dim3(256), 0, st, m.R, KS, q, m.NP, m.ld, njb, partial, (size_t)0);
   p.want_grad = 0;
   hipLaunchKernelGGL(k_acq_combine, dim3((q + 3) / 4, 1, 1), dim3(256), 0, st, partial, q, S, m.k, m.bounds4, m.ystats, p, val,
-                     (double*)nullptr, AcqBatch());
+                     (double*)nullptr, AcqBatch(), host_val);
 }
 
 void launch_score(hipStream_t st, const double* Xq, int q, const GpModel& m, AcqParams p, double* KS, double* partial, double* val,
@@ -1266,7 +1268,7 @@
   hipLaunchKernelGGL(k_score_gemm, dim3(S, (q + 63) / 64, B), dim3(256), 0, st, m.R, KS, q, m.NP, m.ld, njb, partial, ab.zs);
   p.want_grad = 0;
   hipLaunchKernelGGL(k_acq_combine, dim3((q + 3) / 4, 1, B), dim3(256), 0, st, partial, q, S, m.k, m.bounds4, m.ystats, p, val,
-                     (double*)nullptr, ab);
+                     (double*)nullptr, ab, (double*)nullptr);
 }
 
 bool acq_server_possible(int q, int n, int k, int NP) {
@@ -1327,7 +1329,7 @@
 #undef ACQ_ARGS
   if (!combine)
     hipLaunchKernelGGL(k_acq_combine, dim3((q + 3) / 4, 1, gz), dim3(256), 0, st, partial, q, S, k, bounds4, ystats, p, val,
-                       grad, ab);
+                       grad, ab, (double*)nullptr);
 }
 
 template <int N>
diff --git a/para-ortho-pca-bo_amd/csrc/kernels_gp.hip b/para-ortho-pca-bo_amd/csrc/kernels_gp.hip
--- a/para-ortho-pca-bo_amd/csrc/kernels_gp.hip
+++ b/para-ortho-pca-bo_amd/csrc/kernels_gp.hip
@@ -301,8 +301,10 @@
 
 #define RTM_WAVES 16
 __global__ __launch_bounds__(64 * RTM_WAVES) void k_rtmatvec(const double* __restrict__ R, const double* __restrict__ t,
-                                                             int n, int ld, double* __restrict__ out, size_t zs) {
+                                                             int n, int ld, double* __restrict__ out, size_t zs,
+                                                             const int* __restrict__ info, int* __restrict__ host_info) {
   ZRUN(R); ZRUN(t); ZRUN(out);
+  if (host_info && blockIdx.x == 0 && threadIdx.x == 0) *host_info = *info;
   __shared__ double s_p[RTM_WAVES][64];
   const int w = threadIdx.x >> 6, l = threadIdx.x & 63;
   const int j0 = blockIdx.x * 64, j = j0 + l;
@@ -386,7 +388,7 @@
   hipLaunchKernelGGL(k_trinv_cols, dim3(NP / 16, 1, zb.B), dim3(256), 0, s, L, nblk, ld, R, zb.zs);
 }
 void launch_alpha(hipStream_t s, const double* R, const double* ys, int n, int NP, int ld, double* tmp, double* alpha,
-                  ZB zb) {
+                  ZB zb, const int* info, int* host_info) {
   hipLaunchKernelGGL(k_rmatvec, dim3(NP / 16, 1, zb.B), dim3(256), 0, s, R, ys, n, ld, tmp, zb.zs);
-  hipLaunchKernelGGL(k_rtmatvec, dim3(NP / 64, 1, zb.B), dim3(64 * RTM_WAVES), 0, s, R, tmp, n, ld, alpha, zb.zs);
-}
+  hipLaunchKernelGGL(k_rtmatvec, dim3(NP / 64, 1, zb.B), dim3(64 * RTM_WAVES), 0, s, R, tmp, n, ld, alpha, zb.zs, info, host_info);
+}
diff --git a/para-ortho-pca-bo_amd/csrc/kernels_wpca.hip b/para-ortho-pca-bo_amd/csrc/kernels_wpca.hip
--- a/para-ortho-pca-bo_amd/csrc/kernels_wpca.hip
+++ b/para-ortho-pca-bo_amd/csrc/kernels_wpca.hip
@@ -40,10 +40,21 @@
   ranks[i] = r;
 }
 
+__device__ inline double wpca_preweight(double logn, long long rank) { return logn - log((double)rank); }
+__device__ inline double wpca_weighted(double x, double mu, double sw) {
+#pragma clang fp contract(off)
+  return (x - mu) * sw;
+}
+__device__ inline double wpca_noised(double w, double nz) {
+#pragma clang fp contract(off)
+  return w + nz;
+}
+
 __global__ __launch_bounds__(WP_THREADS) void k_wpca_prep(
     const double* __restrict__ X, const long long* __restrict__ ranks, const double* __restrict__ noise,
     int n, int d, int DP, double* __restrict__ weights, double* __restrict__ data_mean,
-    double* __restrict__ pca_mean, double* __restrict__ Wc, size_t zs) {
+    double* __restrict__ pca_mean, double* __restrict__ Wc, size_t zs, double* __restrict__ host_data_mean,
+    double* __restrict__ host_pca_mean) {
   ZRUN(X); ZRUN(ranks); ZRUN(noise); ZRUN(weights); ZRUN(data_mean); ZRUN(pca_mean); ZRUN(Wc);
   __shared__ double s_red[WP_THREADS];
   __shared__ double s_col[PCABO_MAXD];
@@ -56,7 +67,7 @@
   double loc = 0.0;
   const double logn = log((double)n);
   for (int i = tid; i < n; i += WP_THREADS) {
-    double pw = logn - log((double)ranks[i]);
+    double pw = wpca_preweight(logn, ranks[i]);
     weights[i] = pw;
     loc += pw;
   }
@@ -89,7 +100,7 @@
     double s = 0.0;
     for (int gg = 0; gg < G; ++gg) s += s_red[gg * CP + tid];
     s_col[tid] = s / (double)n;
-    if (tid < d) data_mean[tid] = s_col[tid];
+    if (tid < d) { data_mean[tid] = s_col[tid]; if (host_data_mean) host_data_mean[tid] = s_col[tid]; }
   }
   __syncthreads();
   const double mu = (c < d) ? s_col[c] : 0.0;
@@ -103,8 +114,8 @@
         const int i = g + u * G;
         double w = 0.0;
         if (c < d && i < n) {
-          w = (xr[u] - mu) * sqrt(weights[i]);
-          if (noise) w += noise[(size_t)i * d + c];
+          w = wpca_weighted(xr[u], mu, sqrt(weights[i]));
+          if (noise) w = wpca_noised(w, noise[(size_t)i * d + c]);
         }
         xr[u] = w;
         if (i < n4) acc += w;
@@ -115,8 +126,8 @@
     for (int i = g; i < n4; i += G) {
       double w = 0.0;
       if (c < d && i < n) {
-        w = (X[(size_t)i * d + c] - mu) * sqrt(weights[i]);
-        if (noise) w += noise[(size_t)i * d + c];
+        w = wpca_weighted(X[(size_t)i * d + c], mu, sqrt(weights[i]));
+        if (noise) w = wpca_noised(w, noise[(size_t)i * d + c]);
       }
       Wc[(size_t)i * DP + c] = w;
       acc += w;
@@ -128,7 +139,7 @@
     double s = 0.0;
     for (int gg = 0; gg < G; ++gg) s += s_red[gg * CP + tid];
     s_col[tid] = s / (double)n;
-    if (tid < d) pca_mean[tid] = s_col[tid];
+    if (tid < d) { pca_mean[tid] = s_col[tid]; if (host_pca_mean) host_pca_mean[tid] = s_col[tid]; }
   }
   __syncthreads();
   const double mw = (c < d) ? s_col[c] : 0.0;
@@ -170,6 +181,149 @@
   }
 }
 
+#define WC_ROWS 32
+__global__ __launch_bounds__(256) void k_wpca_cov(
+    const double* __restrict__ X, const long long* __restrict__ ranks, const double* __restrict__ noise, int n, int d, int DP,
+    double inv_nm1, double* __restrict__ data_mean, double* __restrict__ pca_mean, double* __restrict__ C, size_t zs,
+    double* __restrict__ host_data_mean, double* __restrict__ host_pca_mean) {
+  ZRUN(X); ZRUN(ranks); ZRUN(noise); ZRUN(data_mean); ZRUN(pca_mean); ZRUN(C);
+  __shared__ double s_m[256];
+  __shared__ double s_sw[16 * WC_ROWS];
+  __shared__ double s_p1[2][16][16];
+  __shared__ double s_p2[2][16][16];
+  __shared__ double s_acc[4][4][64];
+  const int ti = blockIdx.x, tj = blockIdx.y;
+  const int tid = threadIdx.x, w = tid >> 6, l = tid & 63;
+  const int cl = l & 15, g = 4 * w + (l >> 4);
+  const int ca = 16 * ti + cl, cb = 16 * tj + cl;
+  const bool two = ti != tj;
+  const int n4 = (n + 3) & ~3;
+  const unsigned cac = ca < d ? ca : d - 1, cbc = cb < d ? cb : d - 1;
+
+  long long rk[4];
+#pragma unroll
+  for (int k = 0; k < 4; ++k) { const int i = tid + 256 * k; rk[k] = ranks[i < n ? i : n - 1]; }
+  double xa[WC_ROWS], xb[WC_ROWS], na[WC_ROWS], nb[WC_ROWS];
+#pragma unroll
+  for (int u = 0; u < WC_ROWS; ++u) { xa[u] = 0.0; xb[u] = 0.0; na[u] = 0.0; nb[u] = 0.0; }
+#pragma unroll
+  for (int ug = 0; ug < WC_ROWS / 4; ++ug) {
+    if (64 * ug < n4) {
+      unsigned row[4];
+#pragma unroll
+      for (int v = 0; v < 4; ++v) { const int i = g + 16 * (4 * ug + v); row[v] = (unsigned)(i < n ? i : n - 1) * (unsigned)d; }
+#pragma unroll
+      for (int v = 0; v < 4; ++v) xa[4 * ug + v] = X[row[v] + cac];
+      if (two) {
+#pragma unroll
+        for (int v = 0; v < 4; ++v) xb[4 * ug + v] = X[row[v] + cbc];
+      }
+      if (noise) {
+#pragma unroll
+        for (int v = 0; v < 4; ++v) na[4 * ug + v] = noise[row[v] + cac];
+        if (two) {
+#pragma unroll
+          for (int v = 0; v < 4; ++v) nb[4 * ug + v] = noise[row[v] + cbc];
+        }
+      }
+    }
+  }
+
+  const double logn = log((double)n);
+  double pw[4];
+#pragma unroll
+  for (int k = 0; k < 4; ++k) pw[k] = tid + 256 * k < n ? wpca_preweight(logn, rk[k]) : 0.0;
+  s_m[tid] = ((0.0 + pw[0]) + (0.0 + pw[2])) + ((0.0 + pw[1]) + (0.0 + pw[3]));
+  double acc_a = 0.0, acc_b = 0.0;
+#pragma unroll
+  for (int u = 0; u < WC_ROWS; ++u) {
+    const bool in = g + 16 * u < n;
+    xa[u] = (ca < d && in) ? xa[u] : 0.0;
+    xb[u] = (cb < d && in) ? xb[u] : 0.0;
+    if (ca < d && in) acc_a += xa[u];
+    if (cb < d && in) acc_b += xb[u];
+  }
+  s_p1[0][g][cl] = acc_a;
+  s_p1[1][g][cl] = acc_b;
+  __syncthreads();
+  double tot;
+  {
+    double x = (s_m[l] + s_m[l + 128]) + (s_m[l + 64] + s_m[l + 192]);
+#pragma unroll
+    for (int off = 32; off > 0; off >>= 1) {
+      const double y = __shfl_down(x, off, 64);
+      if (l < off) x = x + y;
+    }
+    tot = read_lane(x, 0);
+  }
+#pragma unroll
+  for (int k = 0; k < 2; ++k) {
+    const int i = tid + 256 * k;
+    if (i < n) s_sw[i] = sqrt(pw[k] / tot);
+  }
+  double mu_a, mu_b;
+  {
+    double sa = 0.0, sb = 0.0;
+#pragma unroll
+    for (int gg = 0; gg < 16; ++gg) { sa += s_p1[0][gg][cl]; sb += s_p1[1][gg][cl]; }
+    mu_a = ca < d ? sa / (double)n : 0.0;
+    mu_b = cb < d ? sb / (double)n : 0.0;
+  }
+  __syncthreads();
+
+  acc_a = 0.0; acc_b = 0.0;
+#pragma unroll
+  for (int u = 0; u < WC_ROWS; ++u) {
+    const int i = g + 16 * u;
+    const double sw = s_sw[i];
+    double wa = 0.0, wb = 0.0;
+    if (ca < d && i < n) {
+      wa = wpca_weighted(xa[u], mu_a, sw);
+      if (noise) wa = wpca_noised(wa, na[u]);
+    }
+    if (two && cb < d && i < n) {
+      wb = wpca_weighted(xb[u], mu_b, sw);
+      if (noise) wb = wpca_noised(wb, nb[u]);
+    }
+    xa[u] = wa; xb[u] = wb;
+    if (i < n4) { acc_a += wa; acc_b += wb; }
+  }
+  s_p2[0][g][cl] = acc_a;
+  s_p2[1][g][cl] = acc_b;
+  __syncthreads();
+  double mw_a, mw_b;
+  {
+    double sa = 0.0, sb = 0.0;
+#pragma unroll
+    for (int gg = 0; gg < 16; ++gg) { sa += s_p2[0][gg][cl]; sb += s_p2[1][gg][cl]; }
+    mw_a = ca < d ? sa / (double)n : 0.0;
+    mw_b = cb < d ? sb / (double)n : 0.0;
+  }
+  if (tj == 0 && g == 0 && ca < d) {
+    data_mean[ca] = mu_a; pca_mean[ca] = mw_a;
+    if (host_data_mean) { host_data_mean[ca] = mu_a; host_pca_mean[ca] = mw_a; }
+  }
+
+  double4_t acc = {0.0, 0.0, 0.0, 0.0};
+  const int steps = n4 >> 2;
+#pragma unroll
+  for (int u = 0; u < WC_ROWS; ++u) {
+    if (w + 4 * u >= steps) break;
+    const bool in = g + 16 * u < n;
+    const double a = (ca < d && in) ? xa[u] - mw_a : 0.0;
+    const double b = two ? ((cb < d && in) ? xb[u] - mw_b : 0.0) : a;
+    acc = __builtin_amdgcn_mfma_f64_16x16x4f64(a, b, acc, 0, 0, 0);
+  }
+  for (int r = 0; r < 4; ++r) s_acc[w][r][l] = acc[r];
+  __syncthreads();
+  if (w == 0) {
+    for (int r = 0; r < 4; ++r) {
+      double s = ((s_acc[0][r][l] + s_acc[1][r][l]) + s_acc[2][r][l]) + s_acc[3][r][l];
+      C[(size_t)(ti * 16 + (l >> 4) + 4 * r) * DP + tj * 16 + (l & 15)] = s * inv_nm1;
+    }
+  }
+}
+
 #define JAC_THREADS 1024
 #ifdef PCABO_ACQ_TIMING
 __device__ unsigned long long g_jac_stamps[8];
@@ -179,6 +333,7 @@
 #endif
 struct PcaSelect {
   int n; double var_threshold; int n_components; double* comps; double* evr; int* k_dev; HostMirror* hm;
+  double *host_comps, *host_evr;
 };
 template <int NT>
 __device__ inline void jac_chain(const double* x, const double* y, double& a, double& b, double& g) {
@@ -417,6 +572,7 @@
     for (int r = 0; r < rcount; ++r) tot += s_lam[s_order[r]];
     const double e = s_lam[s_order[tid]] / tot;
     sel.evr[tid] = e;
+    if (sel.host_evr) sel.host_evr[tid] = e;
     s_evr[tid] = e;
     const double* v = s_g + s_order[tid] * LD;
     double best = -1.0, sgn = 1.0;
@@ -446,7 +602,9 @@
   }
   for (int idx = tid; idx < rcount * d; idx += (int)blockDim.x) {
     const int r = idx / d, j = idx % d;
-    sel.comps[idx] = s_sgn[r] * s_g[s_order[r] * LD + j];
+    const double cv = s_sgn[r] * s_g[s_order[r] * LD + j];
+    sel.comps[idx] = cv;
+    if (sel.host_comps) sel.host_comps[idx] = cv;
   }
 }
 
@@ -607,14 +765,23 @@
 void launch_rank(hipStream_t s, const double* f, int n, int maximize, long long* ranks) {
   hipLaunchKernelGGL(k_rank, dim3((n + 255) / 256), dim3(256), 0, s, f, n, maximize, ranks);
 }
-void launch_wpca_prep(hipStream_t s, const double* X, const long long* ranks, const double* noise, int n, int d,
-                      int DP, double* weights, double* data_mean, double* pca_mean, double* Wc, ZB zb) {
+static int g_wpca_form = -1;
+extern "C" int pcabo_debug_wpca_form(void) { return g_wpca_form; }
+int launch_wpca_cov(hipStream_t s, const double* X, const long long* ranks, const double* noise, int n, int d, int DP,
+                    double* weights, double* data_mean, double* pca_mean, double* Wc, double* C, bool allow_fused,
+                    double* host_means, size_t host_ld, ZB zb) {
+  const int n4 = (n + 3) & ~3;
+  const double inv_nm1 = 1.0 / (double)(n - 1);
+  double* host_pm = host_means ? host_means + host_ld : nullptr;
+  if (allow_fused && DP <= 64 && (n4 + 15) / 16 <= WC_ROWS) {
+    hipLaunchKernelGGL(k_wpca_cov, dim3(DP / 16, DP / 16, zb.B), dim3(256), 0, s, X, ranks, noise, n, d, DP, inv_nm1, data_mean,
+                       pca_mean, C, zb.zs, host_means, host_pm);
+    return g_wpca_form = 1;
+  }
   hipLaunchKernelGGL(k_wpca_prep, dim3(1, 1, zb.B), dim3(WP_THREADS), 0, s, X, ranks, noise, n, d, DP, weights, data_mean,
-                     pca_mean, Wc, zb.zs);
-}
-void launch_cov(hipStream_t s, const double* Wc, int n, int DP, double* C, ZB zb) {
-  int n4 = (n + 3) & ~3;
-  hipLaunchKernelGGL(k_cov, dim3(DP / 16, DP / 16, zb.B), dim3(256), 0, s, Wc, n4, DP, 1.0 / (double)(n - 1), C, zb.zs);
+                     pca_mean, Wc, zb.zs, host_means, host_pm);
+  hipLaunchKernelGGL(k_cov, dim3(DP / 16, DP / 16, zb.B), dim3(256), 0, s, Wc, n4, DP, inv_nm1, C, zb.zs);
+  return g_wpca_form = 0;
 }
 template <int NT>
 static void launch_jacobi_as(hipStream_t s, int threads, size_t lds, const double* C, int d, int DP, const double* V0, double* G,
@@ -628,7 +795,7 @@
 }
 void launch_jacobi(hipStream_t s, const double* C, int d, int DP, const double* V0, double* G, double* lam, int* sweeps,
                    int n, double var_threshold, int n_components, double* comps, double* evr, int* k_dev, HostMirror* hm,
-                   ZB zb) {
+                   ZB zb, double* host_comps, double* host_evr) {
   const int nt = d <= 16 ? 1 : d <= 32 ? 2 : d <= 48 ? 3 : d <= 64 ? 4 : d <= 96 ? 6 : 8;
   const size_t col = (size_t)(16 * nt | 1);
   size_t lds = (size_t)d * col * sizeof(double);
@@ -636,7 +803,7 @@
   const int npairs = ((d + 1) & ~1) / 2;
   int threads = (npairs * 16 + 63) & ~63;
   if (threads < d) threads = (d + 63) & ~63;
-  PcaSelect sel{n, var_threshold, n_components, comps, evr, k_dev, hm};
+  PcaSelect sel{n, var_threshold, n_components, comps, evr, k_dev, hm, host_comps, host_evr};
   switch (nt) {
     case 1: launch_jacobi_as<1>(s, threads, lds, C, d, DP, V0, G, lam, sweeps, sel, zb); break;
     case 2: launch_jacobi_as<2>(s, threads, lds, C, d, DP, V0, G, lam, sweeps, sel, zb); break;
diff --git a/para-ortho-pca-bo_amd/csrc/pcabo_api.hip b/para-ortho-pca-bo_amd/csrc/pcabo_api.hip
--- a/para-ortho-pca-bo_amd/csrc/pcabo_api.hip
+++ b/para-ortho-pca-bo_amd/csrc/pcabo_api.hip
@@ -79,7 +79,9 @@
   hipStream_t stream2 = nullptr;
   hipEvent_t evZn = nullptr, evKS = nullptr;
   bool zn_recorded = false;
+  int last_score_order = -1;
   bool opt_hidden_tail = true;
+  bool opt_fused_wpca = true;
   int max_n = 0, max_d = 0, max_q = 0;
   int NPcap = 0, ld = 0, DPcap = 0, KPcap = 0, Scap = 0;
   int ptr_mode = PCABO_PTR_HOST;
@@ -480,12 +482,14 @@
   if (launch_cholesky(s, ctx->dL, NP, ctx->ld, ctx->dInfo, ctx->dDiag, zb, fold ? ctx->dR : nullptr) != 0)
     return set_err(ctx, PCABO_ERR_HIP, "the Cholesky launches could not be set up (device or kernel attribute)%s", "");
   if (const int rc = phase(3)) return rc;
+  const bool direct = !ctx->in_batch && ctx->opt_hidden_tail && zb.zs == 0 && zb.B == 1;
   if (fold) launch_trinv_drain(s, ctx->dL, NP, ctx->ld, ctx->dR);
   else launch_trinv(s, ctx->dL, NP, ctx->ld, ctx->dR, zb);
-  launch_alpha(s, ctx->dR, ctx->dYs, n, NP, ctx->ld, ctx->dTmp, ctx->dAlpha, zb);
+  launch_alpha(s, ctx->dR, ctx->dYs, n, NP, ctx->ld, ctx->dTmp, ctx->dAlpha, zb, direct ? ctx->dInfo : nullptr,
+               direct ? (int*)&ctx->hm->chol_info : nullptr);
   if (const int rc = phase(4)) return rc;
   if (zb.zs) HIPCHK(hipMemcpy2DAsync((void*)&ctx->hm->chol_info, zb.hzs, ctx->dInfo, zb.zs, sizeof(int), zb.B, hipMemcpyDeviceToHost, s));
-  else HIPCHK(hipMemcpyAsync((void*)&ctx->hm->chol_info, ctx->dInfo, sizeof(int), hipMemcpyDeviceToHost, s));
+  else if (!direct) HIPCHK(hipMemcpyAsync((void*)&ctx->hm->chol_info, ctx->dInfo, sizeof(int), hipMemcpyDeviceToHost, s));
   return PCABO_OK;
 }
 template <class Phase>
@@ -584,6 +588,7 @@
     case PCABO_OPT_BESTF_F32: ctx->bestf_f32 = value != 0; return PCABO_OK;
     case PCABO_OPT_GROUP_ACQ: ctx->opt_group_acq = value != 0; return PCABO_OK;
     case PCABO_OPT_HIDDEN_TAIL: ctx->opt_hidden_tail = value != 0; return PCABO_OK;
+    case PCABO_OPT_FUSED_WPCA: ctx->opt_fused_wpca = value != 0; return PCABO_OK;
     default: return set_err(ctx, PCABO_ERR_ARG, "pcabo_set_option: unknown option %s%d", "", option);
   }
 }
@@ -640,18 +645,23 @@
 static int enqueue_wpca(pcabo_ctx* ctx, const WpcaInputs& in, int n, int d, double var_threshold, int n_components) {
   hipStream_t s = ctx->stream;
   const int DP = round_up(d, 16);
+  const bool direct = !ctx->in_batch && ctx->opt_hidden_tail;
+  const size_t D = ctx->max_d;
+  double* h = direct ? ctx->hSmall : nullptr;
   {
     ProfScope ps(ctx, 0, 8.0 * n * d * 2 + 8.0 * n * d, 2.0 * n * d * d + 9.0 * d * d * d + 2.0 * n * d * d);
-    launch_wpca_prep(s, in.X, in.ranks, in.noise, n, d, DP, ctx->dWeights, ctx->dDataMean, ctx->dPcaMean, ctx->dWc);
-    launch_cov(s, ctx->dWc, n, DP, ctx->dC);
+    launch_wpca_cov(s, in.X, in.ranks, in.noise, n, d, DP, ctx->dWeights, ctx->dDataMean, ctx->dPcaMean, ctx->dWc, ctx->dC,
+                    ctx->opt_fused_wpca, h, D);
     const double* v0 = (ctx->vprev_d == d) ? ctx->dGbuf[ctx->gcur] : nullptr;
     ctx->gcur ^= 1;
     ctx->dG = ctx->dGbuf[ctx->gcur];
     launch_jacobi(s, ctx->dC, d, DP, v0, ctx->dG, ctx->dLam, ctx->dSweeps, n, var_threshold, n_components, ctx->dComps,
-                  ctx->dEvr, ctx->dK, ctx->hm);
+                  ctx->dEvr, ctx->dK, ctx->hm, ZB(), h ? h + 3 * D : nullptr, h ? h + 2 * D : nullptr);
     ctx->vprev_d = d;
+    if (direct) HIPCHK(hipEventRecord(ctx->evPca, s));
     launch_project(s, in.X, ctx->dDataMean, ctx->dPcaMean, ctx->dComps, ctx->dK, n, d, ctx->dZ);
   }
+  if (direct) return PCABO_OK;
   const int rcount = n < d ? n : d;
   HIPCHK(hipMemcpyAsync(ctx->hSmall, ctx->dPcaOut, ((size_t)3 * ctx->max_d + (size_t)rcount * d) * sizeof(double),
                         hipMemcpyDeviceToHost, s));
@@ -1014,8 +1024,7 @@
 
 static int score_tail(pcabo_ctx* ctx, int nq, AcqParams& p) {
   hipStream_t s = ctx->stream;
-  launch_score_tail(s, nq, gp_model(ctx), p, ctx->dKS, ctx->dPartial, ctx->dVal);
-  HIPCHK(hipMemcpyAsync(ctx->hVal, ctx->dVal, (size_t)nq * sizeof(double), hipMemcpyDeviceToHost, s));
+  launch_score_tail(s, nq, gp_model(ctx), p, ctx->dKS, ctx->dPartial, ctx->dVal, ctx->hVal);
   HIPCHK(wait_stream(s));
   HIPCHK(hipGetLastError());
   return PCABO_OK;
@@ -1091,6 +1100,7 @@
   if (!ctx->gp_pending) return set_err(ctx, PCABO_ERR_ARG, "pcabo_gp_condition_end_eval: no conditioning in flight%s", "");
   if (ctx->wpca_uncollected) { int rc0 = pcabo_wpca_results(ctx, nullptr, nullptr, nullptr, nullptr, nullptr); if (rc0 != PCABO_OK) return rc0; }
   if (q <= PCABO_INLAUNCH_MAXQ || ctx->ptr_mode != PCABO_PTR_HOST) {
+    ctx->last_score_order = 0;
     int rc = pcabo_gp_condition_end(ctx);
     if (rc != PCABO_OK) return rc;
     return pcabo_acq_eval(ctx, Xq, q, best_f, maximize, acq, val, nullptr);
@@ -1101,6 +1111,7 @@
   const bool hidden = ctx->zn_recorded && ctx->opt_hidden_tail && !ctx->prof && score_gemm_possible(q);
   ctx->zn_recorded = false;
   int rc;
+  ctx->last_score_order = hidden ? 1 : 0;
   if (hidden) {
     HIPCHK(hipStreamWaitEvent(ctx->stream2, ctx->evZn, 0));
     HIPCHK(hipMemcpyAsync(ctx->dXq, ctx->hXq, (size_t)q * ctx->k * sizeof(double), hipMemcpyHostToDevice, ctx->stream2));
@@ -1124,6 +1135,8 @@
   memcpy(val, ctx->hVal, (size_t)q * sizeof(double));
   return PCABO_OK;
 }
+
+int pcabo_debug_score_order(pcabo_ctx* ctx) { return ctx ? ctx->last_score_order : -1; }
 
 int pcabo_logei(pcabo_ctx* ctx, const double* Xq, int q, double best_f, int maximize, double* val, double* grad) {
   return pcabo_acq_eval(ctx, Xq, q, best_f, maximize, PCABO_ACQ_LOG_EI, val, grad);
@@ -1451,6 +1464,7 @@
   bool score_enqueued = false;
   bool imap_enqueued = false;
   bool opt_enqueued = false; int opt_restarts = 0, opt_limit = 0; std::vector<int> opt_act;
+  bool fused_wpca = true;
   int dev_lbfgsb = 0;
   std::vector<unsigned> dbg_branches; std::vector<double> dbg_group_out; int dbg_groups = 0;
   unsigned *dOptTab = nullptr, *hOptTab = nullptr;
@@ -1604,6 +1618,7 @@
     batch->dev_lbfgsb = value;
     return PCABO_OK;
   }
+  if (option == PCABO_OPT_FUSED_WPCA) { batch->fused_wpca = value != 0; return PCABO_OK; }
   if (option != PCABO_OPT_GROUP_ACQ) return bset_err(batch, PCABO_ERR_ARG, "pcabo_batch_set_option: unknown option %s%d", "", option);
   batch->group_acq = value != 0;
   for (pcabo_ctx* c : batch->ctx) c->opt_group_acq = batch->group_acq;
@@ -1681,8 +1696,8 @@
   const ZB zb = batch_zb(batch);
   const int DP = round_up(d, 16);
   if (batch->prof) (void)hipEventRecord(batch->pev[0], s);
-  launch_wpca_prep(s, inX, inRanks, inNoise, n, d, DP, c0->dWeights, c0->dDataMean, c0->dPcaMean, c0->dWc, zb);
-  launch_cov(s, c0->dWc, n, DP, c0->dC, zb);
+  launch_wpca_cov(s, inX, inRanks, inNoise, n, d, DP, c0->dWeights, c0->dDataMean, c0->dPcaMean, c0->dWc, c0->dC, batch->fused_wpca,
+                  nullptr, 0, zb);
   const double* v0 = (batch->vprev_d == d) ? c0->dGbuf[batch->gcur] : nullptr;
   batch->gcur ^= 1;
   launch_jacobi(s, c0->dC, d, DP, v0, c0->dGbuf[batch->gcur], c0->dLam, c0->dSweeps, n, var_threshold, n_components,
diff --git a/para-ortho-pca-bo_amd/csrc/pcabo_internal.h b/para-ortho-pca-bo_amd/csrc/pcabo_internal.h
--- a/para-ortho-pca-bo_amd/csrc/pcabo_internal.h
+++ b/para-ortho-pca-bo_amd/csrc/pcabo_internal.h
@@ -238,12 +238,12 @@
 #define PCABO_HYP_MEAN_C 2
 #define PCABO_HYP_WORDS 4
 struct ZB { int B = 1; size_t zs = 0, hzs = 0; const double* hyp = nullptr; };
-void launch_wpca_prep(hipStream_t s, const double* X, const long long* ranks, const double* noise, int n, int d,
-                      int DP, double* weights, double* data_mean, double* pca_mean, double* Wc, ZB zb = ZB());
-void launch_cov(hipStream_t s, const double* Wc, int n, int DP, double* C, ZB zb = ZB());
+int launch_wpca_cov(hipStream_t s, const double* X, const long long* ranks, const double* noise, int n, int d, int DP,
+                    double* weights, double* data_mean, double* pca_mean, double* Wc, double* C, bool allow_fused,
+                    double* host_means = nullptr, size_t host_ld = 0, ZB zb = ZB());
 void launch_jacobi(hipStream_t s, const double* C, int d, int DP, const double* V0, double* G, double* lam, int* sweeps,
                    int n, double var_threshold, int n_components, double* comps, double* evr, int* k_dev, HostMirror* hm,
-                   ZB zb = ZB());
+                   ZB zb = ZB(), double* host_comps = nullptr, double* host_evr = nullptr);
 void launch_project(hipStream_t s, const double* X, const double* data_mean, const double* pca_mean,
                     const double* comps, const int* k_dev, int n, int d, double* Z, ZB zb = ZB());
 void launch_zstats(hipStream_t s, const double* Z, const double* y, int n, int k, const double* user_norm_bounds,
@@ -267,7 +267,7 @@
                       double* R = nullptr);
 void launch_trinv_diag_w(hipStream_t s, const double* L, int nblk, int ld, double* R, ZB zb = ZB());
 void launch_alpha(hipStream_t s, const double* R, const double* ys, int n, int NP, int ld, double* tmp, double* alpha,
-                  ZB zb = ZB());
+                  ZB zb = ZB(), const int* info = nullptr, int* host_info = nullptr);
 void launch_mll_grad(hipStream_t s, const double* R, const double* AT, const double* nrm, const double* alpha, const double* L,
                      const double* ys, int n, int NP, int KP, int ld, double* partial, double* out,
                      const int* k_dev = nullptr, ZB zb = ZB());
@@ -288,7 +288,8 @@
 void launch_score(hipStream_t st, const double* Xq, int q, const GpModel& m, AcqParams p, double* KS, double* partial, double* val,
                   AcqBatch ab = AcqBatch(), int B = 1);
 void launch_score_ks_only(hipStream_t st, const double* Xq, int q, const GpModel& m, AcqParams p, double* KS);
-void launch_score_tail(hipStream_t st, int q, const GpModel& m, AcqParams p, const double* KS, double* partial, double* val);
+void launch_score_tail(hipStream_t st, int q, const GpModel& m, AcqParams p, const double* KS, double* partial, double* val,
+                       double* host_val = nullptr);
 bool acq_server_possible(int q, int n, int k, int NP);
 int acq_slabs(int NP);
 void launch_inverse_map(hipStream_t s, const double* z, const double* comps, const double* data_mean,
diff --git a/para-ortho-pca-bo_amd/pcabo/_native.py b/para-ortho-pca-bo_amd/pcabo/_native.py
--- a/para-ortho-pca-bo_amd/pcabo/_native.py
+++ b/para-ortho-pca-bo_amd/pcabo/_native.py
@@ -13,6 +13,7 @@
 PTR_HOST, PTR_DEVICE = 0, 1
 OPT_RESIDENT, OPT_BESTF_F32, OPT_GROUP_ACQ, OPT_DEVICE_LBFGSB = 0, 1, 2, 3
 OPT_HIDDEN_TAIL = 5
+OPT_FUSED_WPCA = 6
 FIT_THETA0 = (0.006737946999085467, 0.0, 0.0)
 FIT_TASK_NOT_PD = -2
 PROFILE_GROUPS = ("wpca", "gram", "cholesky", "root_inverse_alpha", "acq_partial", "acq_large_batches")
@@ -179,6 +180,10 @@
     LIB.pcabo_debug_batch_lbfgsb_device_out.argtypes = [C.c_void_p, C.c_void_p, C.c_int]
 
 
+def wpca_form() -> int:
+    return int(LIB.pcabo_debug_wpca_form())
+
+
 def device_count() -> int:
     return int(LIB.pcabo_device_count())
 
@@ -425,6 +430,10 @@
         K = np.empty((self.n, self.n))
         self._chk(LIB.pcabo_get_gram(self._h, _ptr(K)))
         return K
+
+    def score_order(self) -> int:
+        LIB.pcabo_debug_score_order.argtypes = [C.c_void_p]
+        return int(LIB.pcabo_debug_score_order(self._h))
 
     def set_profiling(self, on: bool) -> None:
         self._chk(LIB.pcabo_set_profiling(self._h, int(bool(on))))
@@ -485,6 +494,9 @@
             import warnings
             warnings.warn(advice, RuntimeWarning, stacklevel=2)
 
+    def set_option(self, option: int, value: int) -> None:
+        self._chk(LIB.pcabo_batch_set_option(self._h, int(option), int(value)))
+
     def set_workers(self, workers: int) -> None:
         self._chk(LIB.pcabo_batch_set_workers(self._h, int(workers)))
 
```

Result: no change. 403.5 BO iterations/s (median of 3 runs) (-0.3%).
